# PJLab-ADG/DetZero

Measured on AMD Instinct MI355X. Metric: LiDAR frames/sec (160k pts, 0.1m voxels), higher is better.
Workload: dtype f32 as f16 pairs (hi+lo, 22-bit significand; 3 f16 MFMA per product, f32 accumulate)

## Files before the change

### detzero_amd/csrc/common.h

```cpp
#pragma once
#include <hip/hip_runtime.h>
#include <stdint.h>
#include <stdio.h>

#include "../../include/detzero_hip.h"

namespace dz {

void set_error(const char *fmt, ...);

#define DZ_CHECK_ARG(cond, ...)                 \
    do {                                        \
        if (!(cond)) {                          \
            dz::set_error(__VA_ARGS__);         \
            return DZ_ERR_INVALID;              \
        }                                       \
    } while (0)

#define DZ_HIP(expr)                                                                     \
    do {                                                                                 \
        hipError_t _e = (expr);                                                          \
        if (_e != hipSuccess) {                                                          \
            dz::set_error("%s failed: %s (%s:%d)", #expr, hipGetErrorString(_e), __FILE__, __LINE__); \
            return DZ_ERR_HIP;                                                           \
        }                                                                                \
    } while (0)

#define DZ_LAUNCH_CHECK()                                                                \
    do {                                                                                 \
        hipError_t _e = hipGetLastError();                                               \
        if (_e != hipSuccess) {                                                          \
            dz::set_error("kernel launch failed: %s (%s:%d)", hipGetErrorString(_e), __FILE__, __LINE__); \
            return DZ_ERR_HIP;                                                           \
        }                                                                                \
    } while (0)

static inline int ceil_div(long a, long b) { return (int)((a + b - 1) / b); }

static inline int tile_masks_words(int cap) { return (cap / 32 + 1 + 3) & ~3; }
static inline size_t align_up(size_t x, size_t a) { return (x + a - 1) / a * a; }

static inline int stream_grid(long work_items, int block) {
    long g = (work_items + block - 1) / block;
    if (g < 1) g = 1;
    if (g > 2048) g = 2048;
    return (int)g;
}

constexpr int DZ_MAX_DEVICES = 32;
struct PerDeviceFlags { bool v[DZ_MAX_DEVICES] = {}; };
static inline int reserve_lds(const void *kernel, int bytes, PerDeviceFlags &done, const char *who) {
    int dev = 0;
    if (hipGetDevice(&dev) != hipSuccess) { set_error("%s: hipGetDevice failed", who); return DZ_ERR_HIP; }
    if (dev >= 0 && dev < DZ_MAX_DEVICES && done.v[dev]) return DZ_OK;
    if (hipFuncSetAttribute(kernel, hipFuncAttributeMaxDynamicSharedMemorySize, bytes) != hipSuccess) {
        set_error("%s: cannot reserve %d bytes of LDS on device %d", who, bytes, dev);
        return DZ_ERR_HIP;
    }
    if (dev >= 0 && dev < DZ_MAX_DEVICES) done.v[dev] = true;
    return DZ_OK;
}
static inline int device_cus() {
    static int cus[DZ_MAX_DEVICES] = {};
    int dev = 0;
    if (hipGetDevice(&dev) != hipSuccess) return 256;
    if (dev >= 0 && dev < DZ_MAX_DEVICES && cus[dev]) return cus[dev];
    int n = 0;
    if (hipDeviceGetAttribute(&n, hipDeviceAttributeMultiprocessorCount, dev) != hipSuccess || n <= 0) n = 256;
    if (dev >= 0 && dev < DZ_MAX_DEVICES) cus[dev] = n;
    return n;
}

constexpr uint32_t KEY_INVALID = 0xFFFFFFFFu;

__device__ __forceinline__ int bitmap_rank(const uint32_t *__restrict__ bitmap,
                                           const uint32_t *__restrict__ prefix, uint32_t key) {
    const uint32_t w = key >> 5, bit = key & 31u;
    const uint32_t word = bitmap[w];
    return (int)(prefix[w] + __popc(word & ((1u << bit) - 1u)));
}
__device__ __forceinline__ int bitmap_find(const uint32_t *__restrict__ bitmap,
                                           const uint32_t *__restrict__ prefix, uint32_t key) {
    const uint32_t w = key >> 5, bit = key & 31u;
    const uint32_t word = bitmap[w];
    if (!((word >> bit) & 1u)) return -1;
    return (int)(prefix[w] + __popc(word & ((1u << bit) - 1u)));
}

struct LevelGeom {
    int b, d, h, w, layout, nby, nbx;
    __host__ __device__ __forceinline__ uint32_t key(int bi, int z, int y, int x) const {
        if (layout == 0) return (uint32_t)(((bi * d + z) * h + y) * w + x);
        const uint32_t brick = (uint32_t)((bi * nby + (y >> 3)) * nbx + (x >> 3));
        return ((brick * (uint32_t)d + (uint32_t)z) << 6) | (uint32_t)(((y & 7) << 3) | (x & 7));
    }
    __host__ __device__ __forceinline__ bool inside(int bi, int z, int y, int x) const {
        return (unsigned)bi < (unsigned)b && (unsigned)z < (unsigned)d && (unsigned)y < (unsigned)h && (unsigned)x < (unsigned)w;
    }
    __host__ __device__ __forceinline__ size_t cells() const {
        return layout == 0 ? (size_t)b * d * h * w : (size_t)b * nby * nbx * d * 64;
    }
    __host__ __device__ __forceinline__ uint32_t batch_key(int bi) const {
        return layout == 0 ? (uint32_t)bi * (uint32_t)(d * h * w) : (uint32_t)bi * (uint32_t)(nby * nbx * d * 64);
    }
};
static inline LevelGeom make_level(int b, int d, int h, int w, int layout) {
    LevelGeom g;
    g.b = b; g.d = d; g.h = h; g.w = w; g.layout = layout ? 1 : 0;
    g.nby = (h + 7) / 8; g.nbx = (w + 7) / 8;
    return g;
}

__device__ __forceinline__ uint32_t block_excl_scan_256(uint32_t v, uint32_t *lds, uint32_t &total) {
    const int lane = threadIdx.x & 63, wid = threadIdx.x >> 6;
    uint32_t incl = v;
#pragma unroll
    for (int off = 1; off < 64; off <<= 1) {
        uint32_t t = __shfl_up(incl, off, 64);
        if (lane >= off) incl += t;
    }
    if (lane == 63) lds[wid] = incl;
    __syncthreads();
    uint32_t woff = 0, tot = 0;
#pragma unroll
    for (int w = 0; w < 4; ++w) {
        uint32_t s = lds[w];
        if (w < wid) woff += s;
        tot += s;
    }
    __syncthreads();
    total = tot;
    return woff + incl - v;
}

struct ScanDims { int d0, d1, d2; };
int fill_u32(void *ptr, uint32_t value, size_t nwords, hipStream_t stream);
int nms_sweep(const unsigned long long *mask, const int *d_n, int batch, int n_cap, int col_blocks, int post_max, int *keep,
              int *d_num_keep, hipStream_t stream);
size_t bitmap_scan_workspace_bytes(size_t nwords);
int bitmap_scan(const uint32_t *bitmap, size_t nwords, uint32_t *prefix, int *d_total, int mode,
                ScanDims dims, int *coords_out, int cap_out, void *ws, size_t ws_bytes,
                hipStream_t stream, bool nonzero_only = false,
                const unsigned char *line_flags = nullptr);
int level_scan(const uint32_t *bitmap, const LevelGeom &lg, uint32_t *prefix, int *d_total, int *coords_out, int cap_out, void *ws,
               size_t ws_bytes, hipStream_t stream, bool nonzero_only, const unsigned char *line_flags = nullptr);

}
```

### detzero_amd/csrc/sparse_conv_h.hip

```cpp
#include "hgemm.h"
#include "sparse_conv_w.h"

namespace dz {

constexpr int KVOL_MAX_H = 27;

template <class T, class M, int NS, bool GN, int OCC>
__global__ __launch_bounds__(T::THREADS) __attribute__((amdgpu_waves_per_eu(OCC))) void k_spconv_h(SpConvHArgs a) {
    extern __shared__ __attribute__((aligned(16))) unsigned char smem_raw[];
    v4u *const smem = reinterpret_cast<v4u *>(smem_raw);
    int *const nbr_s = reinterpret_cast<int *>(smem + T::LDS_U4);
    __shared__ unsigned int mask_s;
    __shared__ __attribute__((aligned(16))) float sc_s[T::BC], sh_s[T::BC];
    constexpr int P = T::P_PER_THREAD;
    constexpr int NST = T::P_PER_THREAD + T::C_PER_THREAD;

    const int tid = threadIdx.x, lane = tid & 63, wid = tid >> 6;
    const int wp = wid / T::WC, wc = wid % T::WC;
    const int m = min(*a.d_m_out, a.cap);
    const int ntiles = (m + T::BP - 1) / T::BP;
    const int kchunks = a.cin / T::KC;
    const int n0 = blockIdx.y * T::BC;
    const srsrc_t prsrc = make_srsrc(a.in, a.in_bytes);
    const srsrc_t crsrc = make_srsrc(a.w, a.w_bytes);
    const srsrc_t nrsrc = make_srsrc(a.nbr, a.nbr_bytes);
    unsigned int cvoff[T::C_PER_THREAD];
#pragma unroll
    for (int i = 0; i < T::C_PER_THREAD; ++i) {
        const int idx = tid + i * T::THREADS;
        cvoff[i] = OOB_OFFSET;
        if (T::C_PIECES % T::THREADS == 0 || idx < T::C_PIECES) {
            const int n = idx / (T::KC / 4), q = idx % (T::KC / 4);
            cvoff[i] = (unsigned int)(((n0 + n) * a.cin + q * 4) * 4);
        }
    }
    const unsigned int tap_bytes = (unsigned int)(a.cout_pad * a.cin * 4);
    const unsigned int nbr_tap_bytes = (unsigned int)a.cap * 4u;
    for (int c = tid; c < T::BC; c += T::THREADS) {
        const bool in = n0 + c < a.cout;
        sc_s[c] = (in && a.scale) ? a.scale[n0 + c] : 1.f;
        sh_s[c] = (in && a.shift) ? a.shift[n0 + c] : 0.f;
    }
    __syncthreads();

    constexpr int XRUN = 16;
    const int xcd = blockIdx.x & 7;
    for (int t = blockIdx.x >> 3;; t += gridDim.x >> 3) {
        const int tile = ((t / XRUN) * 8 + xcd) * XRUN + t % XRUN;
        if ((t / XRUN) * 8 * XRUN >= ntiles) break;
        if (tile >= ntiles) continue;
        const int row0 = tile * T::BP;
        unsigned int taps;
        if constexpr (GN) {
            taps = 0u;
#pragma unroll
            for (int i = 0; i < T::BP / 32; ++i) taps |= a.tile_masks[tile * (T::BP / 32) + i];
            taps = __builtin_amdgcn_readfirstlane(taps);
        } else {
            if (tid == 0) mask_s = 0u;
            __syncthreads();
            unsigned int local = 0u;
            for (int idx = tid; idx < a.kvol * T::BP; idx += T::THREADS) {
                const int k = idx / T::BP, r = idx % T::BP;
                const int row = row0 + r;
                const int v = (row < m) ? a.nbr[(size_t)k * a.cap + row] : -1;
                nbr_s[idx] = v;
                if (v >= 0) local |= 1u << k;
            }
            if (local) atomicOr(&mask_s, local);
            __syncthreads();
            taps = mask_s;
        }

        f32x16 acc[T::CT][T::PT];
#pragma unroll
        for (int i = 0; i < T::CT; ++i)
#pragma unroll
            for (int j = 0; j < T::PT; ++j)
#pragma unroll
                for (int e = 0; e < 16; ++e) acc[i][j][e] = 0.f;

        const int nchunks = __popc(taps) * kchunks;
        if (nchunks > 0) {
            unsigned int rem = taps;
            int tap = __ffs((int)rem) - 1, kc = 0;
            auto advance = [&]() {
                rem &= rem - 1;
                if (rem == 0u) { rem = taps; ++kc; }
                tap = __ffs((int)rem) - 1;
            };
            if constexpr (GN) {
                int nb[NS][P];
                unsigned int nvoff[P];
#pragma unroll
                for (int i = 0; i < P; ++i) {
                    const int idx = tid + i * T::THREADS;
                    const int row = row0 + idx / (T::KC / 4);
                    nvoff[i] = ((T::P_PIECES % T::THREADS == 0 || idx < T::P_PIECES) && row < m) ? (unsigned int)row * 4u : OOB_OFFSET;
                }
                unsigned int rem_a = taps;
                int tap_a = __ffs((int)rem_a) - 1;
                auto fetch_nbr = [&](int (&dst)[P]) {
                    const unsigned int toff = (unsigned int)tap_a * nbr_tap_bytes;
#pragma unroll
                    for (int i = 0; i < P; ++i)
                        asm volatile("buffer_load_dword %0, %1, %2, 0 offen" : "=v"(dst[i]) : "v"(nvoff[i] == OOB_OFFSET ? OOB_OFFSET : nvoff[i] + toff), "s"(nrsrc));
                    rem_a &= rem_a - 1;
                    if (rem_a == 0u) rem_a = taps;
                    tap_a = __ffs((int)rem_a) - 1;
                };
#pragma unroll
                for (int s = 0; s < NS; ++s) fetch_nbr(nb[s]);
                asm volatile("s_waitcnt vmcnt(0)");
#pragma unroll
                for (int s = 0; s < NS; ++s)
#pragma unroll
                    for (int i = 0; i < P; ++i) asm volatile("" : "+v"(nb[s][i]));
                auto issue = [&](HStage<T> &st, auto s_t) {
                    constexpr int S = decltype(s_t)::value;
                    asm volatile("s_waitcnt vmcnt(%0)" ::"n"((NS - 1) * (NST + P)));
                    unsigned int pvoff[P];
#pragma unroll
                    for (int i = 0; i < P; ++i) {
                        asm volatile("" : "+v"(nb[S][i]));
                        const int q = (tid + i * T::THREADS) % (T::KC / 4);
                        const int rb = nb[S][i];
                        pvoff[i] = (nvoff[i] != OOB_OFFSET && rb >= 0) ? (unsigned int)rb * (unsigned int)(a.cin * 4) + (unsigned int)(q * 16) : OOB_OFFSET;
                    }
                    load_hstage<T>(st, prsrc, pvoff, (unsigned int)(kc * T::KC * 4), crsrc, cvoff,
                                   (unsigned int)tap * tap_bytes + (unsigned int)(kc * T::KC * 4));
                    fetch_nbr(nb[S]);
                };
                hgemm_pipeline<T, M, NS, P, (T::THREADS == 512)>(nchunks, smem, issue, advance, acc, wp, wc, lane, tid);
            } else {
                auto issue = [&](HStage<T> &st, auto) {
                    unsigned int pvoff[P];
#pragma unroll
                    for (int i = 0; i < P; ++i) {
                        const int idx = tid + i * T::THREADS;
                        pvoff[i] = OOB_OFFSET;
                        if (T::P_PIECES % T::THREADS == 0 || idx < T::P_PIECES) {
                            const int rr = idx / (T::KC / 4), q = idx % (T::KC / 4);
                            const int rb = nbr_s[tap * T::BP + rr];
                            pvoff[i] = rb >= 0 ? (unsigned int)rb * (unsigned int)(a.cin * 4) + (unsigned int)(q * 16) : OOB_OFFSET;
                        }
                    }
                    load_hstage<T>(st, prsrc, pvoff, (unsigned int)(kc * T::KC * 4), crsrc, cvoff,
                                   (unsigned int)tap * tap_bytes + (unsigned int)(kc * T::KC * 4));
                };
                hgemm_pipeline<T, M, NS>(nchunks, smem, issue, advance, acc, wp, wc, lane, tid);
            }
        }

        store_tile_pair16<T, M>(acc, smem_raw, sc_s, sh_s, n0, a.cout, a.relu != 0, reinterpret_cast<const unsigned char *>(a.residual),
                                reinterpret_cast<unsigned char *>(a.out), wp, wc, lane, wid, [&](int lr) {
                                    const int row = row0 + lr;
                                    return row < m ? (size_t)row * a.cout * 4 : ~size_t(0);
                                });
        __syncthreads();
    }
}


template <class M, class T, int NS, bool GN, int OCC>
static int launch_spconv_h(const SpConvHArgs &a, hipStream_t stream) {
    constexpr int LDS = T::LDS_BYTES + (GN ? 0 : KVOL_MAX_H * T::BP * 4);
    static PerDeviceFlags lds_done;
    if (int rc_ = reserve_lds(reinterpret_cast<const void *>(&k_spconv_h<T, M, NS, GN, OCC>), LDS, lds_done, "dz_spconv_forward_split")) return rc_;
    int grid = ceil_div(a.cap, T::BP);
    if (grid > 2048) grid = 2048;
    grid = (grid + 7) & ~7;
    if (grid < 8) grid = 8;
    hipLaunchKernelGGL((k_spconv_h<T, M, NS, GN, OCC>), dim3(grid, a.cout_pad / T::BC), dim3(T::THREADS), LDS, stream, a);
    DZ_LAUNCH_CHECK();
    return DZ_OK;
}

enum SpHVariant { SH_NONE = 0, SH_W_16_16, SH_W_16_32, SH_W_32_32, SH_WP_16_16, SH_WP_16_32, SH_WP_32_32, SH_128_32_16_LDS, SH_128_32_32_LDS,
                  SH_256_64_RING, SH_256_64_LDS, SH_256_128_RING, SH_256_128_LDS };

using SpHLaunch = int (*)(const SpConvHArgs &, hipStream_t);
struct SpHEntry { const char *name, *arm; SpHLaunch launch[3]; };
#define DZ_BY_MATH(fn, ...) {fn<MathF16, __VA_ARGS__>, fn<MathBF16, __VA_ARGS__>, fn<MathF16H, __VA_ARGS__>}
static const SpHEntry kSpH[] = {
    {"none", "none", {nullptr, nullptr, nullptr}},
    {"k_spconv_w<16x16>", "k_spconv_w<16x16>", DZ_BY_MATH(launch_spconv_w, 16, 16, 4, 4, 3, false)},
    {"k_spconv_w<16x32>", "k_spconv_w<16x32>", DZ_BY_MATH(launch_spconv_w, 16, 32, 3, 6, 3, false)},
    {"k_spconv_w<32x32>", "k_spconv_w<32x32>", DZ_BY_MATH(launch_spconv_w, 32, 32, 2, 12, 3, false)},
    {"k_spconv_w<16x16>", "k_spconv_w<16x16>", DZ_BY_MATH(launch_spconv_w, 16, 16, 4, 6, 3, true)},
    {"k_spconv_w<16x32>", "k_spconv_w<16x32>", DZ_BY_MATH(launch_spconv_w, 16, 32, 3, 6, 3, true)},
    {"k_spconv_w<32x32>", "k_spconv_w<32x32>", DZ_BY_MATH(launch_spconv_w, 32, 32, 2, 12, 3, true)},
    {"k_spconv_h<128x32x16>", "k_spconv_h<128x32x16> lds", DZ_BY_MATH(launch_spconv_h, HTile<128, 32, 16, 4, 1>, 4, false, 4)},
    {"k_spconv_h<128x32x32>", "k_spconv_h<128x32x32> lds", DZ_BY_MATH(launch_spconv_h, HTile<128, 32, 32, 4, 1>, 3, false, 1)},
    {"k_spconv_h<256x64x32>", "k_spconv_h<256x64x32> ring", DZ_BY_MATH(launch_spconv_h, HTile<256, 64, 32, 4, 2>, 3, true, 2)},
    {"k_spconv_h<256x64x32>", "k_spconv_h<256x64x32> lds", DZ_BY_MATH(launch_spconv_h, HTile<256, 64, 32, 4, 2>, 3, false, 2)},
    {"k_spconv_h<256x128x32>", "k_spconv_h<256x128x32> ring", DZ_BY_MATH(launch_spconv_h, HTile<256, 128, 32, 4, 2>, 2, true, 2)},
    {"k_spconv_h<256x128x32>", "k_spconv_h<256x128x32> lds", DZ_BY_MATH(launch_spconv_h, HTile<256, 128, 32, 4, 2>, 2, false, 2)},
};
#undef DZ_BY_MATH
static_assert(sizeof(kSpH) / sizeof(kSpH[0]) == SH_256_128_LDS + 1, "one entry per variant");

static SpHVariant spconv_h_select(int cin, int cout, bool packed, bool masks) {
    if (packed || (masks && cout <= 32)) {
        if (cin == 16 && cout == 16) return packed ? SH_WP_16_16 : SH_W_16_16;
        if (cin == 16 && cout == 32) return packed ? SH_WP_16_32 : SH_W_16_32;
        if (cin == 32 && cout == 32) return packed ? SH_WP_32_32 : SH_W_32_32;
        if (packed) return SH_NONE;
    }
    if (cin == 16 && cout <= 32) return SH_128_32_16_LDS;
    if (cin == 32 && cout <= 32) return SH_128_32_32_LDS;
    if ((cin == 32 || cin == 64) && cout == 64) return masks ? SH_256_64_RING : SH_256_64_LDS;
    if ((cin == 64 || cin == 128) && cout == 128) return masks ? SH_256_128_RING : SH_256_128_LDS;
    return SH_NONE;
}

}

using namespace dz;

extern "C" {

int dz_spconv_forward_split(const float *in, int in_rows, int cin, const int *nbr, const uint32_t *tile_masks, int kvol, int cap_out,
                            const int *d_m_out, const float *w, const float *scale, const float *shift, const float *residual,
                            int relu, float *out, int cout, int math, void *stream_) {
    hipStream_t stream = (hipStream_t)stream_;
    DZ_CHECK_ARG(in && nbr && d_m_out && w && out, "dz_spconv_forward_split: null pointer");
    DZ_CHECK_ARG(kvol >= 1 && kvol <= KVOL_MAX_H, "dz_spconv_forward_split: kvol %d not in [1,27]", kvol);
    DZ_CHECK_ARG(math == DZ_MATH_F16X2 || math == DZ_MATH_BF16X2 || math == DZ_MATH_F16, "dz_spconv_forward_split: math %d is not a split mode", math);
    DZ_CHECK_ARG(cout % 8 == 0 && cin % 8 == 0, "dz_spconv_forward_split: channels must be multiples of the 8-channel pair16 group");
    if (cap_out == 0) return DZ_OK;
    const int cout_pad = cout < 32 ? 32 : cout;
    const size_t in_bytes = (size_t)in_rows * cin * sizeof(float);
    const size_t w_bytes = (size_t)kvol * cout_pad * cin * sizeof(float);
    if (in_rows < 0 || in_bytes >= 0x80000000ull) {
        set_error("dz_spconv_forward_split: input of %zu bytes exceeds the 2 GiB buffer-addressing limit", in_bytes);
        return DZ_ERR_UNSUPPORTED;
    }
    const size_t nbr_bytes = (size_t)kvol * cap_out * sizeof(int);
    SpConvHArgs a{in, nbr, tile_masks, d_m_out, w, scale, shift, residual, out, cin, cout, cout_pad, kvol, cap_out, relu,
                  (unsigned int)in_bytes, (unsigned int)w_bytes, nbr_bytes < 0x80000000ull ? (unsigned int)nbr_bytes : 0u,
                  tile_masks ? (unsigned int)tile_masks_words(cap_out) * 4u : 0u};
    const SpHVariant v = spconv_h_select(cin, cout, false, a.tile_masks && a.nbr_bytes);
    if (v == SH_NONE) {
        set_error("dz_spconv_forward_split: unsupported channels cin=%d cout=%d", cin, cout);
        return DZ_ERR_UNSUPPORTED;
    }
    return kSpH[v].launch[math - 1](a, stream);
}

int dz_spconv_forward_split_packed(const float *in, int in_rows, int cin, const int *nbr_packed, const uint32_t *tile_masks, int cap_out,
                                   const int *d_m_out, const float *w, const float *scale, const float *shift, const float *residual,
                                   int relu, float *out, int cout, int math, void *stream_) {
    hipStream_t stream = (hipStream_t)stream_;
    DZ_CHECK_ARG(in && nbr_packed && tile_masks && d_m_out && w && out, "dz_spconv_forward_split_packed: null pointer");
    DZ_CHECK_ARG(math == DZ_MATH_F16X2 || math == DZ_MATH_BF16X2 || math == DZ_MATH_F16, "dz_spconv_forward_split_packed: math %d is not a split mode", math);
    if (cap_out == 0) return DZ_OK;
    const int kvol = 27, cout_pad = 32;
    const size_t in_bytes = (size_t)in_rows * cin * sizeof(float);
    const size_t w_bytes = (size_t)kvol * cout_pad * cin * sizeof(float);
    const size_t nbr_bytes = (size_t)9 * cap_out * sizeof(int);
    if (in_rows < 0 || in_bytes >= 0x80000000ull || nbr_bytes >= 0x80000000ull) {
        set_error("dz_spconv_forward_split_packed: input of %zu / table of %zu bytes exceeds the 2 GiB buffer-addressing limit", in_bytes, nbr_bytes);
        return DZ_ERR_UNSUPPORTED;
    }
    SpConvHArgs a{in, nbr_packed, tile_masks, d_m_out, w, scale, shift, residual, out, cin, cout, cout_pad, kvol, cap_out, relu,
                  (unsigned int)in_bytes, (unsigned int)w_bytes, (unsigned int)nbr_bytes, (unsigned int)tile_masks_words(cap_out) * 4u};
    const SpHVariant v = spconv_h_select(cin, cout, true, true);
    if (v == SH_NONE) {
        set_error("dz_spconv_forward_split_packed: %d -> %d channels (the packed table feeds the 16 -> 16, 16 -> 32 and 32 -> 32 kernels)", cin, cout);
        return DZ_ERR_UNSUPPORTED;
    }
    return kSpH[v].launch[math - 1](a, stream);
}

const char *dz_spconv_variant_split(int cin, int cout) {
    return kSpH[spconv_h_select(cin, cout, false, true)].name;
}

const char *dz_spconv_variant_split_packed(int cin, int cout) {
    return kSpH[spconv_h_select(cin, cout, true, true)].name;
}

const char *dz_spconv_variant_split_arm(int cin, int cout, int kvol, int has_tile_masks, size_t nbr_bytes) {
    (void)kvol;
    return kSpH[spconv_h_select(cin, cout, false, has_tile_masks && nbr_bytes > 0 && nbr_bytes < 0x80000000ull)].arm;
}

}
```

### detzero_amd/csrc/sparse_index.hip

```cpp
#include <algorithm>
#include <stdarg.h>
#include <string.h>

#include "common.h"

namespace dz {

static thread_local char g_err[512] = "";
void set_error(const char *fmt, ...) {
    va_list ap;
    va_start(ap, fmt);
    vsnprintf(g_err, sizeof(g_err), fmt, ap);
    va_end(ap);
}
const char *last_error() { return g_err; }

__global__ void k_fill_u32(uint32_t *__restrict__ p, uint32_t v, size_t n) {
    const size_t n4 = n / 4;
    uint4 *p4 = reinterpret_cast<uint4 *>(p);
    const uint4 v4 = make_uint4(v, v, v, v);
    for (size_t i = (size_t)blockIdx.x * blockDim.x + threadIdx.x; i < n4; i += (size_t)gridDim.x * blockDim.x) p4[i] = v4;
    for (size_t i = n4 * 4 + (size_t)blockIdx.x * blockDim.x + threadIdx.x; i < n; i += (size_t)gridDim.x * blockDim.x) p[i] = v;
}

int fill_u32(void *ptr, uint32_t value, size_t nwords, hipStream_t stream) {
    if (nwords == 0) return DZ_OK;
    if (((uintptr_t)ptr & 15u) != 0) { set_error("fill_u32: pointer not 16-byte aligned"); return DZ_ERR_INVALID; }
    hipLaunchKernelGGL(k_fill_u32, dim3(stream_grid((long)(nwords / 4 + 1), 256)), dim3(256), 0, stream,
                       reinterpret_cast<uint32_t *>(ptr), value, nwords);
    DZ_LAUNCH_CHECK();
    return DZ_OK;
}

template <int WPT>
__global__ __launch_bounds__(256) void k_scan_reduce(const uint32_t *__restrict__ bitmap, size_t nwords,
                                                     uint32_t *__restrict__ partial, const unsigned char *__restrict__ line_flags) {
    __shared__ uint32_t lds[4];
    const size_t base = (size_t)blockIdx.x * (256 * WPT) + (size_t)threadIdx.x * WPT;
    uint32_t s = 0;
    if (!line_flags || (base < nwords && line_flags[base >> 5])) {
#pragma unroll
        for (int j = 0; j < WPT; ++j)
            if (base + j < nwords) s += __popc(bitmap[base + j]);
    }
    uint32_t total;
    block_excl_scan_256(s, lds, total);
    if (threadIdx.x == 0) partial[blockIdx.x] = total;
}

__global__ __launch_bounds__(1024) void k_scan_partials(uint32_t *__restrict__ partial, int nblocks, int *__restrict__ d_total) {
    constexpr int PPT = 8, TRIP = 1024 * PPT;
    __shared__ uint32_t buf[TRIP + TRIP / 32];
    __shared__ uint32_t wsum[16];
    const int t = threadIdx.x, lane = t & 63, wid = t >> 6;
    auto slot = [](int i) { return i + (i >> 5); };
    uint32_t carry = 0, nxt[PPT];
#pragma unroll
    for (int j = 0; j < PPT; ++j) nxt[j] = (j * 1024 + t < nblocks) ? partial[j * 1024 + t] : 0u;
    for (int base = 0; base < nblocks; base += TRIP) {
#pragma unroll
        for (int j = 0; j < PPT; ++j) buf[slot(j * 1024 + t)] = nxt[j];
        if (base + TRIP < nblocks) {
#pragma unroll
            for (int j = 0; j < PPT; ++j) { const int i = base + TRIP + j * 1024 + t; nxt[j] = i < nblocks ? partial[i] : 0u; }
        }
        __syncthreads();
        uint32_t v[PPT], s = 0;
#pragma unroll
        for (int j = 0; j < PPT; ++j) { v[j] = buf[slot(t * PPT + j)]; s += v[j]; }
        uint32_t incl = s;
#pragma unroll
        for (int off = 1; off < 64; off <<= 1) {
            const uint32_t u = __shfl_up(incl, off, 64);
            if (lane >= off) incl += u;
        }
        if (lane == 63) wsum[wid] = incl;
        __syncthreads();
        uint32_t woff = 0, tot = 0;
#pragma unroll
        for (int w = 0; w < 16; ++w) { const uint32_t x = wsum[w]; if (w < wid) woff += x; tot += x; }
        uint32_t run = carry + woff + incl - s;
#pragma unroll
        for (int j = 0; j < PPT; ++j) { buf[slot(t * PPT + j)] = run; run += v[j]; }
        carry += tot;
        __syncthreads();
#pragma unroll
        for (int j = 0; j < PPT; ++j) { const int i = base + j * 1024 + t; if (i < nblocks) partial[i] = buf[slot(j * 1024 + t)]; }
        __syncthreads();
    }
    if (t == 0) *d_total = (int)carry;
}

struct FastDiv { uint32_t d; double inv; };
__device__ __forceinline__ uint32_t fast_divmod(uint32_t n, const FastDiv f, uint32_t &rem) {
    uint32_t q = (uint32_t)__double2uint_rz((double)n * f.inv);
    uint32_t r = n - q * f.d;
    if ((int32_t)r < 0) { --q; r += f.d; }
    else if (r >= f.d) { ++q; r -= f.d; }
    rem = r;
    return q;
}
struct ScanDecode { FastDiv d0, d1, d2; };

template <int MODE, int WPT, bool NZ = false>
__global__ __launch_bounds__(256) void k_scan_down(const uint32_t *__restrict__ bitmap, size_t nwords,
                                                   const uint32_t *__restrict__ partial,
                                                   uint32_t *__restrict__ prefix, ScanDecode dec,
                                                   int *__restrict__ coords_out, int cap_out,
                                                   const unsigned char *__restrict__ line_flags, const int *__restrict__ d_total) {
    constexpr int CHUNK = 256 * WPT;
    if (NZ) {
        const uint32_t p0 = partial[blockIdx.x], p1 = blockIdx.x + 1 < gridDim.x ? partial[blockIdx.x + 1] : (uint32_t)*d_total;
        if (p0 == p1) return;
    }
    __shared__ uint32_t lds[4];
    __shared__ __attribute__((aligned(16))) uint32_t w_s[CHUNK];
    __shared__ __attribute__((aligned(16))) uint32_t p_s[CHUNK];
    const size_t base = (size_t)blockIdx.x * CHUNK + (size_t)threadIdx.x * WPT;
    uint32_t wv[WPT];
    const bool live = !line_flags || (base < nwords && line_flags[base >> 5]);
#pragma unroll
    for (int j = 0; j < WPT; ++j) wv[j] = (live && base + j < nwords) ? bitmap[base + j] : 0u;
    uint32_t s = 0;
#pragma unroll
    for (int j = 0; j < WPT; ++j) s += __popc(wv[j]);
    uint32_t total;
    uint32_t run = block_excl_scan_256(s, lds, total) + partial[blockIdx.x];
    uint32_t pv[WPT];
#pragma unroll
    for (int j = 0; j < WPT; ++j) { pv[j] = run; run += __popc(wv[j]); }
#pragma unroll
    for (int j = 0; j < WPT; ++j)
        if (base + j < nwords && (!NZ || wv[j])) prefix[base + j] = pv[j];
    if (MODE < 0 || total == 0) return;
#pragma unroll
    for (int j = 0; j < WPT; ++j) { w_s[threadIdx.x * WPT + j] = wv[j]; p_s[threadIdx.x * WPT + j] = pv[j]; }
    __syncthreads();
#pragma unroll 1
    for (int j = 0; j < WPT; ++j) {
        const int idx = threadIdx.x + 256 * j;
        uint32_t word = w_s[idx];
        if (!word) continue;
        uint32_t r = p_s[idx];
        const uint32_t key0 = (uint32_t)(((size_t)blockIdx.x * CHUNK + idx) << 5);
        if (MODE == 2) {
            uint32_t z, by, bx;
            const uint32_t brick = fast_divmod(key0 >> 6, dec.d0, z);
            const uint32_t t = fast_divmod(brick, dec.d2, bx);
            const uint32_t bb = fast_divmod(t, dec.d1, by);
            const int y0 = (int)(by * 8u + ((key0 >> 3) & 7u)), x0 = (int)(bx * 8u);
            while (word) {
                const int bit = __ffs((int)word) - 1;
                word &= word - 1;
                if ((int)r < cap_out) reinterpret_cast<int4 *>(coords_out)[r] = make_int4((int)bb, (int)z, y0 + (bit >> 3), x0 + (bit & 7));
                ++r;
            }
            continue;
        }
        uint32_t c2, c1, c0;
        const uint32_t t1 = fast_divmod(key0, dec.d2, c2);
        const uint32_t t0 = fast_divmod(t1, dec.d1, c1);
        uint32_t bb = fast_divmod(t0, dec.d0, c0);
        int last = 0;
        while (word) {
            const int bit = __ffs((int)word) - 1;
            word &= word - 1;
            c2 += (uint32_t)(bit - last);
            last = bit;
            while (c2 >= dec.d2.d) {
                c2 -= dec.d2.d;
                if (++c1 == dec.d1.d) { c1 = 0; if (++c0 == dec.d0.d) { c0 = 0; ++bb; } }
            }
            if ((int)r < cap_out) {
                int4 o;
                if (MODE == 0) o = make_int4((int)bb, (int)c0, (int)c1, (int)c2);
                else o = make_int4((int)bb, (int)c2, (int)c1, (int)c0);
                reinterpret_cast<int4 *>(coords_out)[r] = o;
            }
            ++r;
        }
    }
}

size_t bitmap_scan_workspace_bytes(size_t nwords) {
    const size_t nblocks = (nwords + 255) / 256;
    return align_up(nblocks * sizeof(uint32_t), 256);
}

template <int WPT>
static void launch_scan(const uint32_t *bitmap, size_t nwords, uint32_t *prefix, int *d_total, int mode, const ScanDecode &dec,
                        int *coords_out, int cap_out, uint32_t *partial, hipStream_t stream, bool nonzero_only,
                        const unsigned char *lf) {
    const int nblocks = (int)((nwords + 256 * WPT - 1) / (256 * WPT));
    hipLaunchKernelGGL(k_scan_reduce<WPT>, dim3(nblocks), dim3(256), 0, stream, bitmap, nwords, partial, lf);
    hipLaunchKernelGGL(k_scan_partials, dim3(1), dim3(1024), 0, stream, partial, nblocks, d_total);
    if (mode == 0 && nonzero_only)
        hipLaunchKernelGGL((k_scan_down<0, WPT, true>), dim3(nblocks), dim3(256), 0, stream, bitmap, nwords, partial, prefix, dec,
                           coords_out, cap_out, lf, d_total);
    else if (mode == 0)
        hipLaunchKernelGGL((k_scan_down<0, WPT>), dim3(nblocks), dim3(256), 0, stream, bitmap, nwords, partial, prefix, dec,
                           coords_out, cap_out, lf, d_total);
    else if (mode == 1)
        hipLaunchKernelGGL((k_scan_down<1, WPT>), dim3(nblocks), dim3(256), 0, stream, bitmap, nwords, partial, prefix, dec,
                           coords_out, cap_out, lf, d_total);
    else if (mode == 2 && nonzero_only)
        hipLaunchKernelGGL((k_scan_down<2, WPT, true>), dim3(nblocks), dim3(256), 0, stream, bitmap, nwords, partial, prefix, dec,
                           coords_out, cap_out, lf, d_total);
    else if (mode == 2)
        hipLaunchKernelGGL((k_scan_down<2, WPT>), dim3(nblocks), dim3(256), 0, stream, bitmap, nwords, partial, prefix, dec,
                           coords_out, cap_out, lf, d_total);
    else
        hipLaunchKernelGGL((k_scan_down<-1, WPT>), dim3(nblocks), dim3(256), 0, stream, bitmap, nwords, partial, prefix, dec,
                           coords_out, cap_out, lf, d_total);
}

int bitmap_scan(const uint32_t *bitmap, size_t nwords, uint32_t *prefix, int *d_total, int mode,
                ScanDims dims, int *coords_out, int cap_out, void *ws, size_t ws_bytes,
                hipStream_t stream, bool nonzero_only, const unsigned char *line_flags) {
    if (ws_bytes < bitmap_scan_workspace_bytes(nwords)) {
        set_error("bitmap_scan: workspace %zu < %zu", ws_bytes, bitmap_scan_workspace_bytes(nwords));
        return DZ_ERR_WORKSPACE;
    }
    uint32_t *partial = reinterpret_cast<uint32_t *>(ws);
    ScanDecode dec;
    dec.d0 = FastDiv{(uint32_t)(dims.d0 > 0 ? dims.d0 : 1), 1.0 / (double)(dims.d0 > 0 ? dims.d0 : 1)};
    dec.d1 = FastDiv{(uint32_t)(dims.d1 > 0 ? dims.d1 : 1), 1.0 / (double)(dims.d1 > 0 ? dims.d1 : 1)};
    dec.d2 = FastDiv{(uint32_t)(dims.d2 > 0 ? dims.d2 : 1), 1.0 / (double)(dims.d2 > 0 ? dims.d2 : 1)};
    if (nwords <= ((size_t)1 << 21))
        launch_scan<1>(bitmap, nwords, prefix, d_total, mode, dec, coords_out, cap_out, partial, stream, nonzero_only, line_flags);
    else
        launch_scan<4>(bitmap, nwords, prefix, d_total, mode, dec, coords_out, cap_out, partial, stream, nonzero_only, line_flags);
    DZ_LAUNCH_CHECK();
    return DZ_OK;
}

__global__ void k_set_bits_from_coords(const int *__restrict__ coords, const int *__restrict__ d_n, int n_cap,
                                       LevelGeom lg, uint32_t *__restrict__ bitmap) {
    const int n = d_n ? min(*d_n, n_cap) : n_cap;
    for (int i = blockIdx.x * blockDim.x + threadIdx.x; i < n; i += gridDim.x * blockDim.x) {
        const int4 c = reinterpret_cast<const int4 *>(coords)[i];
        if (!lg.inside(c.x, c.y, c.z, c.w)) continue;
        const uint32_t key = lg.key(c.x, c.y, c.z, c.w);
        atomicOr(&bitmap[key >> 5], 1u << (key & 31u));
    }
}

__global__ void k_rank_of_coords(const int *__restrict__ coords, const int *__restrict__ d_n, int n_cap, LevelGeom lg,
                                 const uint32_t *__restrict__ bitmap, const uint32_t *__restrict__ prefix, int *__restrict__ rank) {
    const int n = d_n ? min(*d_n, n_cap) : n_cap;
    for (int i = blockIdx.x * blockDim.x + threadIdx.x; i < n_cap; i += gridDim.x * blockDim.x) {
        int r = -1;
        if (i < n) {
            const int4 c = reinterpret_cast<const int4 *>(coords)[i];
            if (lg.inside(c.x, c.y, c.z, c.w)) r = bitmap_rank(bitmap, prefix, lg.key(c.x, c.y, c.z, c.w));
        }
        rank[i] = r;
    }
}

struct ConvGeom {
    int k[3], s[3], p[3];
    int od, oh, ow;
};

__device__ __forceinline__ int outs_of(int c, int k, int s, int p, int od, int (&w)[3]) {
    int n = 0;
    const int cp = c + p;
    for (int t = cp % s; t < k && t <= cp; t += s) {
        const int o = (cp - t) / s;
        if (o < od && n < 3) w[n++] = o;
    }
    return n;
}

__global__ void k_mark_outputs(const int *__restrict__ coords_in, const int *__restrict__ d_m_in, int cap_in,
                               ConvGeom g, LevelGeom lo, uint32_t *__restrict__ bitmap_out) {
    const int m = min(*d_m_in, cap_in);
    for (int i = blockIdx.x * blockDim.x + threadIdx.x; i < m; i += gridDim.x * blockDim.x) {
        const int4 c = reinterpret_cast<const int4 *>(coords_in)[i];
        int wz[3], wy[3], wx[3];
        const int nz = outs_of(c.y, g.k[0], g.s[0], g.p[0], g.od, wz);
        const int ny = outs_of(c.z, g.k[1], g.s[1], g.p[1], g.oh, wy);
        const int nx = outs_of(c.w, g.k[2], g.s[2], g.p[2], g.ow, wx);
        for (int a = 0; a < nz; ++a)
            for (int b = 0; b < ny; ++b) {
                uint32_t word_idx = 0xFFFFFFFFu, bits = 0u;
                for (int e = 0; e < nx; ++e) {
                    const uint32_t key = lo.key(c.x, wz[a], wy[b], wx[e]);
                    if ((key >> 5) != word_idx) {
                        if (bits && (__builtin_nontemporal_load(&bitmap_out[word_idx]) & bits) != bits) atomicOr(&bitmap_out[word_idx], bits);
                        word_idx = key >> 5;
                        bits = 0u;
                    }
                    bits |= 1u << (key & 31u);
                }
                if (bits && (__builtin_nontemporal_load(&bitmap_out[word_idx]) & bits) != bits) atomicOr(&bitmap_out[word_idx], bits);
            }
    }
}

__global__ __launch_bounds__(256) void k_mark_outputs_w(const int *__restrict__ coords_in, const int *__restrict__ d_m_in, int cap_in,
                                                        ConvGeom g, LevelGeom lo, uint32_t *__restrict__ bitmap_out) {
    const int m = min(*d_m_in, cap_in);
    const int m_pad = (m + 63) & ~63;
    const int lane = threadIdx.x & 63;
    for (int i = blockIdx.x * blockDim.x + threadIdx.x; i < m_pad; i += gridDim.x * blockDim.x) {
        uint32_t widx[4] = {0xFFFFFFFFu, 0xFFFFFFFFu, 0xFFFFFFFFu, 0xFFFFFFFFu}, wbits[4] = {0u, 0u, 0u, 0u};
        if (i < m) {
            const int4 c = reinterpret_cast<const int4 *>(coords_in)[i];
            int wz[3], wy[3], wx[3];
            const int nz = outs_of(c.y, g.k[0], g.s[0], g.p[0], g.od, wz);
            const int ny = outs_of(c.z, g.k[1], g.s[1], g.p[1], g.oh, wy);
            const int nx = outs_of(c.w, g.k[2], g.s[2], g.p[2], g.ow, wx);
#pragma unroll
            for (int a = 0; a < 2; ++a)
#pragma unroll
                for (int b = 0; b < 2; ++b) {
                    if (a >= nz || b >= ny || nx < 1) continue;
                    const uint32_t k0 = lo.key(c.x, wz[a], wy[b], wx[0]);
                    uint32_t w = k0 >> 5, bits = 1u << (k0 & 31u);
                    if (nx > 1) {
                        const uint32_t k1 = lo.key(c.x, wz[a], wy[b], wx[1]);
                        if ((k1 >> 5) == w) bits |= 1u << (k1 & 31u);
                        else atomicOr(&bitmap_out[k1 >> 5], 1u << (k1 & 31u));
                    }
                    widx[a * 2 + b] = w;
                    wbits[a * 2 + b] = bits;
                }
        }
        bool last[4];
#pragma unroll
        for (int sl = 0; sl < 4; ++sl) {
            const uint32_t w = widx[sl];
            uint32_t bits = wbits[sl];
#pragma unroll
            for (int d = 1; d < 64; d <<= 1) {
                const uint32_t wp = (uint32_t)__shfl_up((int)w, d, 64), bp = (uint32_t)__shfl_up((int)bits, d, 64);
                if (lane >= d && wp == w) bits |= bp;
            }
            const uint32_t wn = (uint32_t)__shfl_down((int)w, 1, 64);
            last[sl] = bits && (lane == 63 || wn != w);
            wbits[sl] = bits;
        }
        uint32_t seen[4];
#pragma unroll
        for (int sl = 0; sl < 4; ++sl) seen[sl] = last[sl] ? __builtin_nontemporal_load(&bitmap_out[widx[sl]]) : 0xFFFFFFFFu;
#pragma unroll
        for (int sl = 0; sl < 4; ++sl)
            if (last[sl] && (seen[sl] & wbits[sl]) != wbits[sl]) atomicOr(&bitmap_out[widx[sl]], wbits[sl]);
    }
}

#ifndef DZ_NBR_DIAG
#define DZ_NBR_DIAG 0
#endif
typedef unsigned int nbr_u3 __attribute__((ext_vector_type(3)));

template <bool EDGE>
__device__ __forceinline__ void nbr_row3(nbr_u3 w, nbr_u3 p, int ci, uint32_t bc, bool ok, bool lv, bool rv, int &vl, int &vc, int &vr) {
    uint32_t wc_ = w.y, pc_ = p.y, lw = w.x, lp = p.x, rw = w.z, rp = p.z;
    if (EDGE) {
        wc_ = ci == 1 ? w.y : (ci == 0 ? w.x : w.z);
        pc_ = ci == 1 ? p.y : (ci == 0 ? p.x : p.z);
        lw = ci == 1 ? w.x : (ci == 2 ? w.y : 0u); lp = ci == 1 ? p.x : p.y;
        rw = ci == 1 ? w.z : (ci == 0 ? w.y : 0u); rp = ci == 1 ? p.z : p.y;
    }
    if (!ok) wc_ = lw = rw = 0u;
    const int rank = (int)(pc_ + __popc(wc_ & ((1u << bc) - 1u)));
    const uint32_t cbit = (wc_ >> bc) & 1u;
    vc = cbit ? rank : -1;
    const bool lbit = bc != 0u ? ((wc_ >> (bc - 1u)) & 1u) != 0u : (lw >> 31) != 0u;
    const bool rbit = bc != 31u ? ((wc_ >> (bc + 1u)) & 1u) != 0u : (rw & 1u) != 0u;
    const int lrank = bc != 0u ? rank - 1 : (int)(lp + __popc(lw)) - 1;
    const int rrank = bc != 31u ? rank + (int)cbit : (int)rp;
    vl = lbit && lv ? lrank : -1;
    vr = rbit && rv ? rrank : -1;
}

template <int K0, int K1, int KW, bool XCD, bool PACK = false>
__global__ __launch_bounds__(256) void k_build_neighbors_rows(const int *__restrict__ coords_out, const int *__restrict__ d_m_out,
                                                              int cap_out, const uint32_t *__restrict__ bitmap_in,
                                                              const uint32_t *__restrict__ prefix_in, LevelGeom li, ConvGeom g,
                                                              int *__restrict__ nbr, uint32_t *__restrict__ tile_masks, int mask_rows,
                                                              uint32_t last_base, uint32_t index_bytes, uint32_t nbr_bytes) {
// ... 149 lines not shown
            if (tz + 1 < 3) fetch(tz + 1, sl[tz + 1]);
            const Slab &q = sl[tz];
            const bool any_edge = __any(q.edge);
#pragma unroll
            for (int ty = 0; ty < 3; ++ty) {
                const int r = tz * 3 + ty;
                const uint32_t bc = q.kc[ty] & 31u;
                int vl, vc, vr;
                if (any_edge) nbr_row3<true>(q.word[ty], q.pref[ty], (int)((q.kc[ty] >> 5) - q.base[ty]), bc, q.ok[ty], lv, rv, vl, vc, vr);
                else nbr_row3<false>(q.word[ty], q.pref[ty], 1, bc, q.ok[ty], lv, rv, vl, vc, vr);
                const uint32_t rr = vl >= 0 ? (uint32_t)vl + 1u : (vc >= 0 ? (uint32_t)vc : (vr >= 0 ? (uint32_t)vr : 0u));
                const uint32_t e = rr | (vl >= 0 ? 1u << 29 : 0u) | (vc >= 0 ? 1u << 30 : 0u) | (vr >= 0 ? 1u << 31 : 0u);
                words[r] = mine ? e : 0u;
                if (mine) __builtin_amdgcn_raw_buffer_store_b32((int)e, tab, voff, (uint32_t)r * row_bytes, 0);
                bits |= ((vl >= 0 ? 1u : 0u) | (vc >= 0 ? 2u : 0u) | (vr >= 0 ? 4u : 0u)) << (r * 3);
            }
        }
        {
            uint32_t gb = bits;
#pragma unroll
            for (int d = 16; d >= 1; d >>= 1) gb |= (uint32_t)__shfl_xor((int)gb, d, 64);
            if ((tid & 31) == 0 && o < mask_rows) tile_masks[o >> 5] = gb;
        }
        __syncthreads();
#pragma unroll
        for (int tz = 0; tz < 3; ++tz) {
            int lo = 0x7FFFFFFF, hi = -1;
#pragma unroll
            for (int ty = 0; ty < 3; ++ty) {
                const uint32_t e = words[tz * 3 + ty];
                if (!(e >> 29)) continue;
                const int r = (int)(e & 0x1FFFFFFFu), l = (int)((e >> 29) & 1u), cc = (int)((e >> 30) & 1u), rt = (int)(e >> 31);
                lo = min(lo, r - l);
                hi = max(hi, rt ? r + cc : (cc ? r : r - 1));
            }
#pragma unroll
            for (int d = 32; d >= 1; d >>= 1) {
                lo = min(lo, __shfl_xor(lo, d, 64));
                hi = max(hi, __shfl_xor(hi, d, 64));
            }
            if ((tid & 63) == 0 && hi >= 0) { atomicMin(&lo_s[su][tz], lo); atomicMax(&hi_s[su][tz], hi); }
        }
        const int unit = blk * upb + su, row0 = unit * tile_rows;
        unsigned int key = 0x8000000u;
        if (perm) {
            const unsigned int k27 = (unit & 1) ? (0x7FFFFFFu - (bits & 0x7FFFFFFu)) : (bits & 0x7FFFFFFu);
            key = mine ? k27 : 0x8000000u;
            key_s[tid] = key;
        }
        __syncthreads();
        if (ui < 3 && unit < nunits) {
            const int tz = ui;
            int lo = lo_s[su][tz], n = hi_s[su][tz] >= 0 ? hi_s[su][tz] - lo + 1 : 0;
            if (n == 0) lo = 0;
            if (tz == 1 && n == 0 && row0 < m) n = 1;
            win[(size_t)unit * 6 + 2 * tz] = lo;
            win[(size_t)unit * 6 + 2 * tz + 1] = n;
        }
        if (perm) {
            int rank = 0;
            const unsigned int *ks = key_s + su * tile_rows;
            for (int j = 0; j < tile_rows; j += 4) {
                const uint4 v = *reinterpret_cast<const uint4 *>(&ks[j]);
                rank += (v.x < key || (v.x == key && j < ui)) + (v.y < key || (v.y == key && j + 1 < ui)) + (v.z < key || (v.z == key && j + 2 < ui)) +
                        (v.w < key || (v.w == key && j + 3 < ui));
            }
            const int pos = row0 + rank;
            if (pos < cap_out) {
                perm[pos] = o;
#pragma unroll
                for (int g = 0; g < 9; ++g) nbr_sorted[(size_t)g * cap_out + pos] = (int)words[g];
            }
        }
        __syncthreads();
    }
}

__global__ __launch_bounds__(256) void k_build_neighbors(const int *__restrict__ coords_out,
                                                         const int *__restrict__ d_m_out, int cap_out,
                                                         const uint32_t *__restrict__ bitmap_in,
                                                         const uint32_t *__restrict__ prefix_in, LevelGeom li,
                                                         ConvGeom g, int *__restrict__ nbr,
                                                         uint32_t *__restrict__ tile_masks) {
    const int m = min(*d_m_out, cap_out);
    const int rows = g.k[0] * g.k[1];
    const int m_pad = (m + 63) & ~63;
    const long total = (long)m_pad * rows;
    for (long idx = (long)blockIdx.x * blockDim.x + threadIdx.x; idx < total;
         idx += (long)gridDim.x * blockDim.x) {
        const int o = (int)(idx % m_pad);
        const int zy = (int)(idx / m_pad);
        const int tz = zy / g.k[1], ty = zy % g.k[1];
        uint32_t bits = 0u;
        if (o < m) {
            const int4 c = reinterpret_cast<const int4 *>(coords_out)[o];
            const int uz = c.y * g.s[0] - g.p[0] + tz;
            const int uy = c.z * g.s[1] - g.p[1] + ty;
            const bool row_ok = (unsigned)uz < (unsigned)li.d && (unsigned)uy < (unsigned)li.h;
            const int base_x = c.w * g.s[2] - g.p[2];
            for (int tx = 0; tx < g.k[2]; ++tx) {
                const int ux = base_x + tx;
                int v = -1;
                if (row_ok && (unsigned)ux < (unsigned)li.w) v = bitmap_find(bitmap_in, prefix_in, li.key(c.x, uz, uy, ux));
                const int tap = (tz * g.k[1] + ty) * g.k[2] + tx;
                nbr[(size_t)tap * cap_out + o] = v;
                if (v >= 0) bits |= 1u << tap;
            }
        }
        if (tile_masks) {
#pragma unroll
            for (int d = 16; d >= 1; d >>= 1) bits |= (uint32_t)__shfl_xor((int)bits, d, 64);
            if ((threadIdx.x & 31) == 0 && bits) atomicOr(&tile_masks[o >> 5], bits);
        }
    }
}

__global__ void k_scatter_rows(const float *__restrict__ src, const int *__restrict__ rank,
                               const int *__restrict__ d_n, int n_cap, int c_src, float *__restrict__ dst,
                               int c_dst) {
    const int n = d_n ? min(*d_n, n_cap) : n_cap;
    const long total = (long)n * c_dst;
    for (long idx = (long)blockIdx.x * blockDim.x + threadIdx.x; idx < total;
         idx += (long)gridDim.x * blockDim.x) {
        const int i = (int)(idx / c_dst), ch = (int)(idx % c_dst);
        const int r = rank[i];
        if (r < 0) continue;
        dst[(size_t)r * c_dst + ch] = (ch < c_src) ? src[(size_t)i * c_src + ch] : 0.f;
    }
}

__global__ void k_gather_rows(const float *__restrict__ src, const int *__restrict__ idx_,
                              const int *__restrict__ d_n, int n_cap, int c, float *__restrict__ out) {
    const int n = d_n ? min(*d_n, n_cap) : n_cap;
    const long total = (long)n * c;
    for (long idx = (long)blockIdx.x * blockDim.x + threadIdx.x; idx < total;
         idx += (long)gridDim.x * blockDim.x) {
        const int i = (int)(idx / c), ch = (int)(idx % c);
        out[idx] = src[(size_t)idx_[i] * c + ch];
    }
}

static bool geom_from(const int *k3, const int *s3, const int *p3, int d, int h, int w, ConvGeom &g) {
    for (int i = 0; i < 3; ++i) {
        g.k[i] = k3[i]; g.s[i] = s3[i]; g.p[i] = p3[i];
        if (g.k[i] < 1 || g.s[i] < 1 || g.p[i] < 0) return false;
    }
    g.od = (d + 2 * g.p[0] - g.k[0]) / g.s[0] + 1;
    g.oh = (h + 2 * g.p[1] - g.k[1]) / g.s[1] + 1;
    g.ow = (w + 2 * g.p[2] - g.k[2]) / g.s[2] + 1;
    return g.od > 0 && g.oh > 0 && g.ow > 0;
}

int level_scan(const uint32_t *bitmap, const LevelGeom &lg, uint32_t *prefix, int *d_total, int *coords_out, int cap_out, void *ws,
               size_t ws_bytes, hipStream_t stream, bool nonzero_only, const unsigned char *line_flags) {
    const size_t nwords = align_up((lg.cells() + 31) / 32, 8);
    if (lg.layout == 0)
        return bitmap_scan(bitmap, nwords, prefix, d_total, 0, ScanDims{lg.d, lg.h, lg.w}, coords_out, cap_out, ws, ws_bytes, stream,
                           nonzero_only, line_flags);
    return bitmap_scan(bitmap, nwords, prefix, d_total, 2, ScanDims{lg.d, lg.nby, lg.nbx}, coords_out, cap_out, ws, ws_bytes, stream,
                       nonzero_only, line_flags);
}

}

using namespace dz;

extern "C" {

const char *dz_version(void) { return "detzero_hip 0.1 (gfx950)"; }
const char *dz_last_error(void) { return dz::last_error(); }

int dz_device_cu_count(void) {
    int dev = 0, n = 0;
    if (hipGetDevice(&dev) != hipSuccess) return -1;
    if (hipDeviceGetAttribute(&n, hipDeviceAttributeMultiprocessorCount, dev) != hipSuccess) return -1;
    return n;
}

size_t dz_index_words(int b, int d, int h, int w, int layout) {
    const size_t cells = make_level(b, d, h, w, layout).cells();
    return align_up((cells + 31) / 32, 8);
}

size_t dz_index_workspace_bytes(int b, int d, int h, int w, int layout) {
    return bitmap_scan_workspace_bytes(dz_index_words(b, d, h, w, layout));
}

static int check_cells(int b, int d, int h, int w, int layout) {
    if (b < 1 || d < 1 || h < 1 || w < 1 || (layout != DZ_LAYOUT_LINEAR && layout != DZ_LAYOUT_BRICK) ||
        make_level(b, d, h, w, layout).cells() >= 0xFFFFFFFFull) {
        set_error("grid %d x %d x %d x %d (layout %d) does not fit 32-bit cell keys", b, d, h, w, layout);
        return DZ_ERR_UNSUPPORTED;
    }
    return DZ_OK;
}


int dz_index_from_coords(const int *coords, const int *d_n, int n_cap, int b, int d, int h, int w, int layout,
                         uint32_t *bitmap, uint32_t *prefix, int *coords_out, int *d_m, int cap_out,
                         int *rank_of_input, void *ws, size_t ws_bytes, void *stream_) {
    hipStream_t stream = (hipStream_t)stream_;
    DZ_CHECK_ARG((coords || n_cap == 0) && bitmap && prefix && coords_out && d_m && n_cap >= 0 && cap_out >= 0,
                 "dz_index_from_coords: null/negative argument");
    int rc = check_cells(b, d, h, w, layout);
    if (rc) return rc;
    const LevelGeom lg = make_level(b, d, h, w, layout);
    const size_t nwords = dz_index_words(b, d, h, w, layout);
    rc = fill_u32(bitmap, 0u, nwords, stream);
    if (rc) return rc;
    if (n_cap > 0)
        hipLaunchKernelGGL(k_set_bits_from_coords, dim3(stream_grid(n_cap, 256)), dim3(256), 0, stream, coords,
                           d_n, n_cap, lg, bitmap);
    rc = level_scan(bitmap, lg, prefix, d_m, coords_out, cap_out, ws, ws_bytes, stream, false);
    if (rc) return rc;
    if (rank_of_input && n_cap > 0)
        hipLaunchKernelGGL(k_rank_of_coords, dim3(stream_grid(n_cap, 256)), dim3(256), 0, stream, coords, d_n,
                           n_cap, lg, bitmap, prefix, rank_of_input);
    DZ_LAUNCH_CHECK();
    return DZ_OK;
}

int dz_index_downsample(const int *coords_in, const int *d_m_in, int cap_in, int b, int d, int h, int w, int layout,
                        const int *h_k3, const int *h_s3, const int *h_p3, uint32_t *bitmap_out,
                        uint32_t *prefix_out, int *coords_out, int *d_m_out, int cap_out, void *ws,
                        size_t ws_bytes, void *stream_) {
    hipStream_t stream = (hipStream_t)stream_;
    DZ_CHECK_ARG(coords_in && d_m_in && bitmap_out && prefix_out && coords_out && d_m_out,
                 "dz_index_downsample: null argument");
    ConvGeom g;
    DZ_CHECK_ARG(geom_from(h_k3, h_s3, h_p3, d, h, w, g), "dz_index_downsample: bad kernel/stride/padding");
    int rc = check_cells(b, g.od, g.oh, g.ow, layout);
    if (rc) return rc;
    const LevelGeom lo = make_level(b, g.od, g.oh, g.ow, layout);
    const size_t nwords = dz_index_words(b, g.od, g.oh, g.ow, layout);
    rc = fill_u32(bitmap_out, 0u, nwords, stream);
    if (rc) return rc;
    static const int plain = getenv("DZ_TUNE_MARK_PLAIN") ? atoi(getenv("DZ_TUNE_MARK_PLAIN")) : 0;
    const bool two = (g.k[0] + g.s[0] - 1) / g.s[0] <= 2 && (g.k[1] + g.s[1] - 1) / g.s[1] <= 2 && (g.k[2] + g.s[2] - 1) / g.s[2] <= 2;
    if (cap_in > 0 && two && !plain)
        hipLaunchKernelGGL(k_mark_outputs_w, dim3(stream_grid(cap_in, 256)), dim3(256), 0, stream, coords_in, d_m_in,
                           cap_in, g, lo, bitmap_out);
    else if (cap_in > 0)
        hipLaunchKernelGGL(k_mark_outputs, dim3(stream_grid(cap_in, 256)), dim3(256), 0, stream, coords_in, d_m_in,
                           cap_in, g, lo, bitmap_out);
    rc = level_scan(bitmap_out, lo, prefix_out, d_m_out, coords_out, cap_out, ws, ws_bytes, stream, false);
    if (rc) return rc;
    DZ_LAUNCH_CHECK();
    return DZ_OK;
}

int dz_tile_masks_words(int cap_out) { return cap_out < 0 ? 0 : tile_masks_words(cap_out); }

int dz_build_neighbors(const int *coords_out, const int *d_m_out, int cap_out, const uint32_t *bitmap_in,
                       const uint32_t *prefix_in, int b, int d, int h, int w, int layout, const int *h_k3, const int *h_s3,
                       const int *h_p3, int *nbr, uint32_t *tile_masks, void *stream_) {
    hipStream_t stream = (hipStream_t)stream_;
    DZ_CHECK_ARG(coords_out && d_m_out && bitmap_in && prefix_in && nbr, "dz_build_neighbors: null argument");
    ConvGeom g;
    DZ_CHECK_ARG(geom_from(h_k3, h_s3, h_p3, d, h, w, g), "dz_build_neighbors: bad kernel/stride/padding");
    DZ_CHECK_ARG(layout == DZ_LAYOUT_LINEAR || layout == DZ_LAYOUT_BRICK, "dz_build_neighbors: bad layout %d", layout);
    if (cap_out == 0) return DZ_OK;
    const LevelGeom li = make_level(b, d, h, w, layout);
    static const int generic = getenv("DZ_TUNE_NBR_GENERIC") ? atoi(getenv("DZ_TUNE_NBR_GENERIC")) : 0;
    const bool kw3 = g.k[2] == 3 && g.p[2] == 1 && (long)(g.ow - 1) * g.s[2] <= w - 1;
    const bool kw1 = g.k[2] == 1 && g.p[2] == 0 && (long)(g.ow - 1) * g.s[2] <= w - 1;
    const size_t table_bytes = (size_t)g.k[0] * g.k[1] * g.k[2] * cap_out * sizeof(int);
    if (!generic && layout == DZ_LAYOUT_LINEAR && g.k[0] == 3 && ((g.k[1] == 3 && kw3) || (g.k[1] == 1 && kw1)) &&
        table_bytes < 0xFFFFFFFFull) {
        const int mask_rows = tile_masks_words(cap_out) * 32;
        const size_t index_words = dz_index_words(b, d, h, w, layout);
        const uint32_t last_base = (uint32_t)(index_words - 3);
        static const int gmax = getenv("DZ_TUNE_NBR_GRID") ? atoi(getenv("DZ_TUNE_NBR_GRID")) : 2048;
        const dim3 grid((std::min(stream_grid(tile_masks ? mask_rows : cap_out, 256), gmax) + 7) & ~7);
        static const int flat = getenv("DZ_TUNE_NBR_FLAT") ? atoi(getenv("DZ_TUNE_NBR_FLAT")) : 0;
#define DZ_NBR_ROWS(K1_, KW_, X_)                                                                                                   \
    hipLaunchKernelGGL((k_build_neighbors_rows<3, K1_, KW_, X_>), grid, dim3(256), 0, stream, coords_out, d_m_out, cap_out, bitmap_in, \
                       prefix_in, li, g, nbr, tile_masks, mask_rows, last_base, (uint32_t)(index_words * 4), (uint32_t)table_bytes)
        if (g.k[1] == 3) { if (flat) DZ_NBR_ROWS(3, 3, false); else DZ_NBR_ROWS(3, 3, true); }
        else { if (flat) DZ_NBR_ROWS(1, 1, false); else DZ_NBR_ROWS(1, 1, true); }
#undef DZ_NBR_ROWS
        DZ_LAUNCH_CHECK();
        return DZ_OK;
    }
    if (tile_masks) {
        const int rc = fill_u32(tile_masks, 0u, (size_t)tile_masks_words(cap_out), stream);
        if (rc) return rc;
    }
    const long work = (long)cap_out * g.k[0] * g.k[1];
    hipLaunchKernelGGL(k_build_neighbors, dim3(stream_grid(work, 256)), dim3(256), 0, stream, coords_out, d_m_out,
                       cap_out, bitmap_in, prefix_in, li, g, nbr, tile_masks);
    DZ_LAUNCH_CHECK();
    return DZ_OK;
}

int dz_build_neighbors_packed(const int *coords_out, const int *d_m_out, int cap_out, const uint32_t *bitmap_in,
                              const uint32_t *prefix_in, int b, int d, int h, int w, int layout, const int *h_k3, const int *h_s3,
                              const int *h_p3, int *nbr, uint32_t *tile_masks, void *stream_) {
    hipStream_t stream = (hipStream_t)stream_;
    DZ_CHECK_ARG(coords_out && d_m_out && bitmap_in && prefix_in && nbr && tile_masks, "dz_build_neighbors_packed: null argument");
    ConvGeom g;
    DZ_CHECK_ARG(geom_from(h_k3, h_s3, h_p3, d, h, w, g), "dz_build_neighbors_packed: bad kernel/stride/padding");
    const bool kw3 = g.k[2] == 3 && g.p[2] == 1 && (long)(g.ow - 1) * g.s[2] <= w - 1;
    const size_t table_bytes = (size_t)9 * cap_out * sizeof(int);
    if (layout != DZ_LAYOUT_LINEAR || g.k[0] != 3 || g.k[1] != 3 || !kw3 || table_bytes >= 0xFFFFFFFFull || cap_out >= (1 << 29)) {
        set_error("dz_build_neighbors_packed: needs linear keys, a 3 x 3 x 3 window with x padding 1 and fewer than 2^29 rows");
        return DZ_ERR_UNSUPPORTED;
    }
    if (cap_out == 0) return DZ_OK;
    const LevelGeom li = make_level(b, d, h, w, layout);
    const int mask_rows = tile_masks_words(cap_out) * 32;
    const size_t index_words = dz_index_words(b, d, h, w, layout);
    const dim3 grid((stream_grid(mask_rows, 256) + 7) & ~7);
    hipLaunchKernelGGL((k_build_neighbors_rows<3, 3, 3, true, true>), grid, dim3(256), 0, stream, coords_out, d_m_out, cap_out, bitmap_in,
                       prefix_in, li, g, nbr, tile_masks, mask_rows, (uint32_t)(index_words - 3), (uint32_t)(index_words * 4),
                       (uint32_t)table_bytes);
    DZ_LAUNCH_CHECK();
    return DZ_OK;
}

int dz_build_neighbors_packed_x(const int *coords, const int *d_m, int cap, const uint32_t *bitmap, const uint32_t *prefix, int b, int d, int h,
                                int w, int *nbr, uint32_t *tile_masks, int tile_rows, int *windows, int *nbr_sorted, int *perm, void *stream_) {
    hipStream_t stream = (hipStream_t)stream_;
    DZ_CHECK_ARG(coords && d_m && bitmap && prefix && nbr && tile_masks && windows, "dz_build_neighbors_packed_x: null argument");
    DZ_CHECK_ARG(b >= 1 && d >= 1 && h >= 1 && w >= 1 && cap >= 0, "dz_build_neighbors_packed_x: bad grid");
    DZ_CHECK_ARG(tile_rows == 128 || tile_rows == 256, "dz_build_neighbors_packed_x: tile_rows %d (128 or 256: dz_spconv_x_tile_rows)", tile_rows);
    DZ_CHECK_ARG((nbr_sorted == nullptr) == (perm == nullptr), "dz_build_neighbors_packed_x: nbr_sorted and perm come together");
    const size_t table_bytes = (size_t)9 * cap * sizeof(int);
    if (table_bytes >= 0xFFFFFFFFull || cap >= (1 << 29)) {
        set_error("dz_build_neighbors_packed_x: needs fewer than 2^29 rows");
        return DZ_ERR_UNSUPPORTED;
    }
    if (cap == 0) return DZ_OK;
    const LevelGeom li = make_level(b, d, h, w, DZ_LAYOUT_LINEAR);
    const int mask_rows = tile_masks_words(cap) * 32;
    const size_t index_words = dz_index_words(b, d, h, w, DZ_LAYOUT_LINEAR);
    const dim3 grid((std::min(ceil_div(cap, 256), 2048) + 7) & ~7);
    hipLaunchKernelGGL(k_build_neighbors_xwin, grid, dim3(256), 0, stream, coords, d_m, cap, bitmap, prefix, li, nbr, tile_masks, mask_rows,
                       (uint32_t)(index_words - 3), (uint32_t)(index_words * 4), (uint32_t)table_bytes, tile_rows, windows, nbr_sorted, perm);
    DZ_LAUNCH_CHECK();
    return DZ_OK;
}

int dz_scatter_rows(const float *src, const int *rank, const int *d_n, int n_cap, int c_src, float *dst, int c_dst,
                    void *stream_) {
    hipStream_t stream = (hipStream_t)stream_;
    DZ_CHECK_ARG(src && rank && dst && c_src > 0 && c_dst >= c_src, "dz_scatter_rows: bad argument");
    if (n_cap == 0) return DZ_OK;
    hipLaunchKernelGGL(k_scatter_rows, dim3(stream_grid((long)n_cap * c_dst, 256)), dim3(256), 0, stream, src, rank,
                       d_n, n_cap, c_src, dst, c_dst);
    DZ_LAUNCH_CHECK();
    return DZ_OK;
}

int dz_gather_rows(const float *src, const int *idx, const int *d_n, int n_cap, int c, float *out, void *stream_) {
    hipStream_t stream = (hipStream_t)stream_;
    DZ_CHECK_ARG(src && idx && out && c > 0, "dz_gather_rows: bad argument");
    if (n_cap == 0) return DZ_OK;
    hipLaunchKernelGGL(k_gather_rows, dim3(stream_grid((long)n_cap * c, 256)), dim3(256), 0, stream, src, idx, d_n,
                       n_cap, c, out);
    DZ_LAUNCH_CHECK();
    return DZ_OK;
}

}
```

### detzero_amd/csrc/voxelize.hip

```cpp
#include "hgemm.h"

namespace dz {

struct VoxGeom {
    float lo[3], vs[3], hi[3];
    int g[3];
    int xy_mask;
};

__device__ __forceinline__ bool voxel_coord(const float *p, const VoxGeom &g, int &cx, int &cy, int &cz) {
    if (g.xy_mask && !(p[0] >= g.lo[0] && p[0] <= g.hi[0] && p[1] >= g.lo[1] && p[1] <= g.hi[1])) return false;
    const float fx = floorf(__fdiv_rn(__fsub_rn(p[0], g.lo[0]), g.vs[0]));
    const float fy = floorf(__fdiv_rn(__fsub_rn(p[1], g.lo[1]), g.vs[1]));
    const float fz = floorf(__fdiv_rn(__fsub_rn(p[2], g.lo[2]), g.vs[2]));
    if (!(fx >= 0.f && fx < (float)g.g[0] && fy >= 0.f && fy < (float)g.g[1] && fz >= 0.f && fz < (float)g.g[2]))
        return false;
    cx = (int)fx; cy = (int)fy; cz = (int)fz;
    return true;
}

__global__ void k_hard_keys(const float *__restrict__ pts, int n, int c, VoxGeom g, int n_per, uint32_t cells,
                            uint32_t *__restrict__ keys, uint32_t *__restrict__ bitmap) {
    for (int i = blockIdx.x * blockDim.x + threadIdx.x; i < n; i += gridDim.x * blockDim.x) {
        const float *p = pts + (size_t)i * c;
// ... 180 lines not shown
                           const int *__restrict__ d_m, int cap, int max_points, int c, float *__restrict__ out,
                           int c_out) {
    const int m = d_m ? min(*d_m, cap) : cap;
    const long total = (long)m * c_out;
    for (long idx = (long)blockIdx.x * blockDim.x + threadIdx.x; idx < total;
         idx += (long)gridDim.x * blockDim.x) {
        const int v = (int)(idx / c_out), ch = (int)(idx % c_out);
        float r = 0.f;
        if (ch < c) {
            float s = 0.f;
            for (int q = 0; q < max_points; ++q) s = __fadd_rn(s, voxels[((size_t)v * max_points + q) * c + ch]);
            const float nrm = fmaxf((float)num_points[v], 1.0f);
            r = __fdiv_rn(s, nrm);
        }
        out[idx] = r;
    }
}

__global__ void k_dyn_keys(const float *__restrict__ pts, int n, int stride, VoxGeom g, int batch,
                           uint32_t *__restrict__ keys, uint32_t *__restrict__ bitmap) {
    const int lane = threadIdx.x & 63;
    const int n_pad = (n + 63) & ~63;
    for (int i = blockIdx.x * blockDim.x + threadIdx.x; i < n_pad; i += gridDim.x * blockDim.x) {
        uint32_t key = KEY_INVALID;
        if (i < n) {
            const float *p = pts + (size_t)i * stride;
            const float xyz[3] = {p[1], p[2], p[3]};
            int cx, cy, cz;
            const int b = (int)p[0];
            if ((unsigned)b < (unsigned)batch && voxel_coord(xyz, g, cx, cy, cz))
                key = (uint32_t)(((b * g.g[0] + cx) * g.g[1] + cy) * g.g[2] + cz);
            keys[i] = key;
        }
        const uint32_t w = key == KEY_INVALID ? KEY_INVALID : key >> 5;
        uint32_t bits = key == KEY_INVALID ? 0u : 1u << (key & 31u);
#pragma unroll
        for (int d = 1; d < 64; d <<= 1) {
            const uint32_t wp = (uint32_t)__shfl_up((int)w, d, 64), bp = (uint32_t)__shfl_up((int)bits, d, 64);
            if (lane >= d && wp == w) bits |= bp;
        }
        const uint32_t wn = (uint32_t)__shfl_down((int)w, 1, 64);
        if (bits && (lane == 63 || wn != w)) atomicOr(&bitmap[w], bits);
    }
}

constexpr float DYN_FIX = 268435456.f;

__global__ void k_dyn_accumulate(const float *__restrict__ pts, int n, int c, const uint32_t *__restrict__ keys,
                                 const uint32_t *__restrict__ bitmap, const uint32_t *__restrict__ prefix, int cap,
                                 unsigned long long *__restrict__ acc, int *__restrict__ counts) {
    const int lane = threadIdx.x & 63;
    const int n_pad = (n + 63) & ~63;
    for (int i = blockIdx.x * blockDim.x + threadIdx.x; i < n_pad; i += gridDim.x * blockDim.x) {
        const uint32_t key = i < n ? keys[i] : KEY_INVALID;
        const uint32_t prev = (uint32_t)__shfl_up((int)key, 1, 64), next = (uint32_t)__shfl_down((int)key, 1, 64);
        const unsigned long long heads = __ballot(lane == 0 || prev != key);
        const int first = 63 - __clzll(heads & (~0ull >> (63 - lane)));
        const int run = lane - first + 1;
        const bool last = key != KEY_INVALID && (lane == 63 || next != key);
        int v = cap;
        if (last) v = bitmap_rank(bitmap, prefix, key);
        int steps = 0;
        while (steps < 6 && __ballot(lane - (1 << steps) >= first) != 0ull) ++steps;
        for (int ch = 0; ch < c; ++ch) {
            long long q = key != KEY_INVALID ? __float2ll_rn(pts[(size_t)i * (c + 1) + 1 + ch] * DYN_FIX) : 0ll;
#pragma unroll
            for (int j = 0; j < 6; ++j) {
                if (j >= steps) break;
                const int lo = __shfl_up((int)(unsigned int)q, 1 << j, 64), hi = __shfl_up((int)(q >> 32), 1 << j, 64);
                if (lane - (1 << j) >= first) q += (long long)(((unsigned long long)(unsigned int)hi << 32) | (unsigned int)lo);
            }
            if (v < cap) atomicAdd(&acc[(size_t)v * c + ch], (unsigned long long)q);
        }
        if (v < cap) atomicAdd(&counts[v], run);
    }
}

__global__ void k_dyn_divide(const unsigned long long *__restrict__ acc, float *__restrict__ feats, const int *__restrict__ counts,
                             const int *__restrict__ d_m, int cap, int c) {
    const int m = min(*d_m, cap);
    const long total = (long)m * c;
    for (long idx = (long)blockIdx.x * blockDim.x + threadIdx.x; idx < total;
         idx += (long)gridDim.x * blockDim.x) {
        const int v = (int)(idx / c);
        const double sum = (double)(long long)acc[idx] * (1.0 / (double)DYN_FIX);
        feats[idx] = __fdiv_rn((float)sum, (float)counts[v]);
    }
}

static bool make_geom(const float *r6, const float *vs3, const int *g3, int xy_mask, VoxGeom &g) {
    g.xy_mask = xy_mask;
    for (int i = 0; i < 3; ++i) {
        g.lo[i] = r6[i]; g.hi[i] = r6[3 + i]; g.vs[i] = vs3[i]; g.g[i] = g3[i];
        if (!(g.vs[i] > 0.f) || g.g[i] < 1) return false;
    }
    return true;
}

struct HardWs {
    uint32_t *keys, *bitmap, *prefix, *pt_bitmap, *pt_prefix;
    int *mins, *canon_coords, *d_m;
    void *scan_ws;
    size_t scan_ws_bytes, total;
};
static HardWs carve_hard(void *ws, int n, size_t nwords, int max_points) {
    HardWs w{};
    size_t off = 0;
    auto take = [&](size_t bytes) { size_t o = off; off += align_up(bytes, 256); return o; };
    char *base = (char *)ws;
    const size_t pt_words = align_up(((size_t)n + 31) / 32, 8);
    size_t o_keys = take((size_t)n * 4), o_bm = take(nwords * 4), o_pf = take(nwords * 4);
    size_t o_pb = take(pt_words * 4), o_pp = take(pt_words * 4);
    size_t o_min = take((size_t)max_points * n * 4), o_cc = take((size_t)n * 16), o_dm = take(256);
    w.scan_ws_bytes = bitmap_scan_workspace_bytes(nwords > pt_words ? nwords : pt_words);
    size_t o_sw = take(w.scan_ws_bytes);
    w.total = off;
    if (base) {
        w.keys = (uint32_t *)(base + o_keys); w.bitmap = (uint32_t *)(base + o_bm); w.prefix = (uint32_t *)(base + o_pf);
        w.pt_bitmap = (uint32_t *)(base + o_pb); w.pt_prefix = (uint32_t *)(base + o_pp);
        w.mins = (int *)(base + o_min); w.canon_coords = (int *)(base + o_cc); w.d_m = (int *)(base + o_dm);
        w.scan_ws = base + o_sw;
    }
    return w;
}

}

using namespace dz;

extern "C" {

size_t dz_voxelize_hard_workspace_bytes(int n, int gx, int gy, int gz, int max_points) {
    if (n < 1) n = 1;
    return carve_hard(nullptr, n, dz_index_words(1, gz, gy, gx, DZ_LAYOUT_LINEAR), max_points).total;
}

static int voxelize_hard_impl(const float *points, int n, int c, const float *h_range6, const float *h_vsize3,
                              const int *h_grid3, int xy_range_mask, int max_points, int max_voxels, float *voxels,
                              int *coords_zyx, int *num_points, int batch_index, int batch, int cap_frame, float *feats,
                              int c_stride, int *coords_bzyx, int *d_num_voxels, void *ws, size_t ws_bytes, hipStream_t stream) {
    VoxGeom g;
    DZ_CHECK_ARG(make_geom(h_range6, h_vsize3, h_grid3, xy_range_mask, g), "dz_voxelize_hard: bad geometry");
    const size_t cells = (size_t)g.g[0] * g.g[1] * g.g[2];
    if (cells * (size_t)batch >= 0xFFFFFFFFull) { set_error("dz_voxelize_hard: grid x batch too large for 32-bit keys"); return DZ_ERR_UNSUPPORTED; }
    if (n == 0) return fill_u32(d_num_voxels, 0u, (size_t)batch, stream);
    DZ_CHECK_ARG(points, "dz_voxelize_hard: null points");
    const int n_per = n / batch;
    const size_t nwords = dz_index_words(batch, g.g[2], g.g[1], g.g[0], DZ_LAYOUT_LINEAR);
    HardWs w = carve_hard(ws, n, nwords, max_points);
    if (ws_bytes < w.total) { set_error("dz_voxelize_hard: workspace %zu < %zu", ws_bytes, w.total); return DZ_ERR_WORKSPACE; }
    const size_t pt_words = align_up(((size_t)n + 31) / 32, 8);
    const int cap = n;

    int rc = fill_u32(w.bitmap, 0u, nwords, stream);
    if (!rc) rc = fill_u32(w.pt_bitmap, 0u, pt_words, stream);
    if (!rc) rc = fill_u32(w.mins, 0x7f7f7f7fu, (size_t)max_points * cap, stream);
    if (rc) return rc;
    const int grid_n = stream_grid(n, 256);
    hipLaunchKernelGGL(k_hard_keys, dim3(grid_n), dim3(256), 0, stream, points, n, c, g, n_per, (uint32_t)cells, w.keys, w.bitmap);
    rc = bitmap_scan(w.bitmap, nwords, w.prefix, w.d_m, 0, ScanDims{g.g[2], g.g[1], g.g[0]}, w.canon_coords, cap,
                         w.scan_ws, w.scan_ws_bytes, stream);
    if (rc) return rc;
    hipLaunchKernelGGL(k_hard_insert, dim3(grid_n), dim3(256), 0, stream, w.keys, n, w.bitmap, w.prefix, w.mins, cap, max_points);
    hipLaunchKernelGGL(k_hard_mark_first, dim3(grid_n), dim3(256), 0, stream, w.mins, w.d_m, cap, w.pt_bitmap);
    rc = bitmap_scan(w.pt_bitmap, pt_words, w.pt_prefix, d_num_voxels, -1, ScanDims{1, 1, 1}, nullptr, 0, w.scan_ws,
                     w.scan_ws_bytes, stream);
    if (rc) return rc;
    if (feats)
        hipLaunchKernelGGL(k_hard_emit_mean, dim3(stream_grid((long)cap * c_stride, 256)), dim3(256), 0, stream, points, c, w.mins,
                           cap, max_points, max_voxels, w.d_m, w.canon_coords, w.pt_bitmap, w.pt_prefix, batch_index, batch, n_per,
                           cap_frame, feats, c_stride, coords_bzyx, d_num_voxels);
    else
        hipLaunchKernelGGL(k_hard_emit, dim3(stream_grid((long)cap * max_points, 256)), dim3(256), 0, stream, points, c,
                           w.mins, cap, max_points, max_voxels, w.d_m, w.canon_coords, w.pt_bitmap, w.pt_prefix, voxels,
                           coords_zyx, num_points, d_num_voxels);
    DZ_LAUNCH_CHECK();
    return DZ_OK;
}

int dz_voxelize_hard(const float *points, int n, int c, const float *h_range6, const float *h_vsize3,
                     const int *h_grid3, int xy_range_mask, int max_points, int max_voxels, float *voxels, int *coords_zyx,
                     int *num_points, int *d_num_voxels, void *ws, size_t ws_bytes, void *stream_) {
    DZ_CHECK_ARG(n >= 0 && c >= 3 && max_points >= 1 && max_voxels >= 1, "dz_voxelize_hard: bad sizes");
    DZ_CHECK_ARG(voxels && coords_zyx && num_points && d_num_voxels && ws, "dz_voxelize_hard: null pointer");
    return voxelize_hard_impl(points, n, c, h_range6, h_vsize3, h_grid3, xy_range_mask, max_points, max_voxels, voxels, coords_zyx,
                              num_points, 0, 1, 0, nullptr, 0, nullptr, d_num_voxels, ws, ws_bytes, (hipStream_t)stream_);
}

int dz_voxelize_hard_mean(const float *points, int n, int c, const float *h_range6, const float *h_vsize3,
                          const int *h_grid3, int xy_range_mask, int max_points, int max_voxels, int batch_index, float *feats,
                          int c_stride, int *coords_bzyx, int *d_num_voxels, void *ws, size_t ws_bytes, void *stream_) {
    DZ_CHECK_ARG(n >= 0 && c >= 3 && max_points >= 1 && max_voxels >= 1 && c_stride >= c, "dz_voxelize_hard_mean: bad sizes");
    DZ_CHECK_ARG(feats && coords_bzyx && d_num_voxels && ws, "dz_voxelize_hard_mean: null pointer");
    return voxelize_hard_impl(points, n, c, h_range6, h_vsize3, h_grid3, xy_range_mask, max_points, max_voxels, nullptr, nullptr,
                              nullptr, batch_index, 1, 0, feats, c_stride, coords_bzyx, d_num_voxels, ws, ws_bytes, (hipStream_t)stream_);
}

size_t dz_voxelize_hard_batched_workspace_bytes(int n_per_frame, int batch, int gx, int gy, int gz, int max_points) {
    const long n = (long)(n_per_frame < 1 ? 1 : n_per_frame) * (batch < 1 ? 1 : batch);
    return carve_hard(nullptr, (int)n, dz_index_words(batch < 1 ? 1 : batch, gz, gy, gx, DZ_LAYOUT_LINEAR), max_points).total;
}

int dz_voxelize_hard_mean_batched(const float *points, int n_per_frame, int batch, int c, const float *h_range6,
                                  const float *h_vsize3, const int *h_grid3, int xy_range_mask, int max_points, int max_voxels,
                                  float *feats, int c_stride, int *coords_bzyx, int cap_per_frame, int *d_num_voxels, void *ws,
                                  size_t ws_bytes, void *stream_) {
    DZ_CHECK_ARG(n_per_frame >= 0 && batch >= 1 && batch <= 256 && c >= 3 && max_points >= 1 && max_voxels >= 1 && c_stride >= c,
                 "dz_voxelize_hard_mean_batched: bad sizes");
    DZ_CHECK_ARG((long)n_per_frame * batch < 0x7FFFFFFFl, "dz_voxelize_hard_mean_batched: too many points");
    DZ_CHECK_ARG(cap_per_frame >= (max_voxels < n_per_frame ? max_voxels : n_per_frame),
                 "dz_voxelize_hard_mean_batched: cap_per_frame below min(max_voxels, points per frame)");
    DZ_CHECK_ARG(feats && coords_bzyx && d_num_voxels && ws, "dz_voxelize_hard_mean_batched: null pointer");
    return voxelize_hard_impl(points, n_per_frame * batch, c, h_range6, h_vsize3, h_grid3, xy_range_mask, max_points, max_voxels,
                              nullptr, nullptr, nullptr, 0, batch, cap_per_frame, feats, c_stride, coords_bzyx, d_num_voxels, ws,
                              ws_bytes, (hipStream_t)stream_);
}

static size_t level_ws_layout(long n, int max_points, int cap, size_t nwords, size_t *o_min, size_t *o_sw, size_t *sw_bytes, size_t *o_lf,
                              size_t *lf_words) {
    size_t off = align_up((size_t)(n < 1 ? 1 : n) * 4, 256);
    *o_min = off;
    off += align_up((size_t)max_points * (cap < 1 ? 1 : cap) * 4, 256);
    *sw_bytes = bitmap_scan_workspace_bytes(nwords);
    *o_sw = off;
    off += align_up(*sw_bytes, 256);
    *lf_words = align_up((nwords + 31) / 32, 16) / 4;
    *o_lf = off;
    off += align_up(*lf_words * 4, 256);
    return off;
}

size_t dz_voxelize_to_level_workspace_bytes(int n_per_frame, int batch, int max_points, int cap, int d, int h, int w, int layout) {
    size_t a, b, c, e, f;
    return level_ws_layout((long)n_per_frame * batch, max_points, cap, dz_index_words(batch, d, h, w, layout), &a, &b, &c, &e, &f);
}

int dz_voxelize_to_level(const float *points, int n_per_frame, int batch, int c, const float *h_range6, const float *h_vsize3,
                         const int *h_grid3, int xy_range_mask, int max_points, int max_voxels, int level_d, int layout, uint32_t *bitmap,
                         uint32_t *prefix, int *coords_out, int *d_m, int cap, float *feats, int c_dst, int math, void *ws,
                         size_t ws_bytes, void *stream_) {
    hipStream_t stream = (hipStream_t)stream_;
    DZ_CHECK_ARG(n_per_frame >= 0 && batch >= 1 && c >= 3 && max_points >= 1 && c_dst >= c && c_dst % 8 == 0,
                 "dz_voxelize_to_level: bad sizes");
    DZ_CHECK_ARG(math >= 0 && math <= 2, "dz_voxelize_to_level: bad math mode %d", math);
    DZ_CHECK_ARG(bitmap && prefix && coords_out && d_m && feats && ws, "dz_voxelize_to_level: null pointer");
    VoxGeom g;
    DZ_CHECK_ARG(make_geom(h_range6, h_vsize3, h_grid3, xy_range_mask, g), "dz_voxelize_to_level: bad geometry");
    DZ_CHECK_ARG(level_d >= g.g[2], "dz_voxelize_to_level: level depth %d below the voxel grid's %d", level_d, g.g[2]);
    if (n_per_frame > max_voxels) {
        set_error("dz_voxelize_to_level: %d points per frame could exceed max_voxels %d - use dz_voxelize_hard_mean_batched",
                  n_per_frame, max_voxels);
        return DZ_ERR_UNSUPPORTED;
    }
    const long n = (long)n_per_frame * batch;
    DZ_CHECK_ARG(n < 0x7FFFFFFFl && cap >= (n < 1 ? 1 : 0), "dz_voxelize_to_level: too many points");
    DZ_CHECK_ARG(layout == DZ_LAYOUT_LINEAR || layout == DZ_LAYOUT_BRICK, "dz_voxelize_to_level: bad layout %d", layout);
    const LevelGeom lg = make_level(batch, level_d, g.g[1], g.g[0], layout);
    if (lg.cells() >= 0xFFFFFFFFull) { set_error("dz_voxelize_to_level: grid x batch too large for 32-bit keys"); return DZ_ERR_UNSUPPORTED; }
    const size_t nwords = dz_index_words(batch, level_d, g.g[1], g.g[0], layout);
    size_t o_min, o_sw, sw_bytes, o_lf, lf_words;
    const size_t need = level_ws_layout(n, max_points, cap, nwords, &o_min, &o_sw, &sw_bytes, &o_lf, &lf_words);
    if (ws_bytes < need) { set_error("dz_voxelize_to_level: workspace %zu < %zu", ws_bytes, need); return DZ_ERR_WORKSPACE; }
    uint32_t *keys = (uint32_t *)ws;
    int *mins = (int *)((char *)ws + o_min);
    static const int use_flags = getenv("DZ_TUNE_LINE_FLAGS") ? atoi(getenv("DZ_TUNE_LINE_FLAGS")) : 1;
    unsigned char *line_flags = use_flags ? (unsigned char *)ws + o_lf : nullptr;
    int rc = fill_u32(bitmap, 0u, nwords, stream);
    if (!rc) rc = fill_u32(mins, 0x7f7f7f7fu, (size_t)max_points * cap, stream);
    if (!rc && line_flags) rc = fill_u32(line_flags, 0u, lf_words, stream);
    if (rc) return rc;
    if (n == 0) return level_scan(bitmap, lg, prefix, d_m, coords_out, cap, (char *)ws + o_sw, sw_bytes, stream, true, line_flags);
    DZ_CHECK_ARG(points, "dz_voxelize_to_level: null points");
    const int grid_n = stream_grid(n, 256);
    hipLaunchKernelGGL(k_level_keys, dim3(grid_n), dim3(256), 0, stream, points, (int)n, c, g, n_per_frame, lg, keys, bitmap,
                       line_flags);
    rc = level_scan(bitmap, lg, prefix, d_m, coords_out, cap, (char *)ws + o_sw, sw_bytes, stream, true, line_flags);
    if (rc) return rc;
    hipLaunchKernelGGL(k_hard_insert, dim3(grid_n), dim3(256), 0, stream, keys, (int)n, bitmap, prefix, mins, cap, max_points);
    const dim3 ge(stream_grid((long)cap * (c_dst / 8), 256));
    if (math == 0)
        hipLaunchKernelGGL(k_level_emit_mean<0>, ge, dim3(256), 0, stream, points, c, mins, cap, max_points, d_m, feats, c_dst);
    else if (math == 1)
        hipLaunchKernelGGL(k_level_emit_mean<1>, ge, dim3(256), 0, stream, points, c, mins, cap, max_points, d_m, feats, c_dst);
    else
        hipLaunchKernelGGL(k_level_emit_mean<2>, ge, dim3(256), 0, stream, points, c, mins, cap, max_points, d_m, feats, c_dst);
    DZ_LAUNCH_CHECK();
    return DZ_OK;
}

int dz_mean_vfe(const float *voxels, const int *num_points, const int *d_m, int cap, int max_points, int c, float *out,
                int c_out_stride, void *stream_) {
    hipStream_t stream = (hipStream_t)stream_;
    DZ_CHECK_ARG(voxels && num_points && out && c >= 1 && c_out_stride >= c && max_points >= 1, "dz_mean_vfe: bad argument");
    if (cap == 0) return DZ_OK;
    hipLaunchKernelGGL(k_mean_vfe, dim3(stream_grid((long)cap * c_out_stride, 256)), dim3(256), 0, stream, voxels,
                       num_points, d_m, cap, max_points, c, out, c_out_stride);
    DZ_LAUNCH_CHECK();
    return DZ_OK;
}

static size_t dyn_layout(int n, size_t nwords, int cap, int c, size_t *o_keys, size_t *o_bm, size_t *o_pf, size_t *o_cnt,
                         size_t *o_acc, size_t *o_sw, size_t *sw_bytes) {
    size_t off = 0;
    auto take = [&](size_t bytes) { size_t o = off; off += align_up(bytes, 256); return o; };
    *o_keys = take((size_t)(n < 1 ? 1 : n) * 4);
    *o_bm = take(nwords * 4);
    *o_pf = take(nwords * 4);
    *o_cnt = take((size_t)(cap < 1 ? 1 : cap) * 4);
    *o_acc = take((size_t)(cap < 1 ? 1 : cap) * (c < 1 ? 1 : c) * 8);
    *sw_bytes = bitmap_scan_workspace_bytes(nwords);
    *o_sw = take(*sw_bytes);
    return off;
}

size_t dz_voxelize_dynamic_workspace_bytes(int n, int batch, int gx, int gy, int gz, int c, int cap) {
    size_t a, b, d, e, f, g, h;
    return dyn_layout(n, dz_index_words(batch, gx, gy, gz, DZ_LAYOUT_LINEAR), cap, c, &a, &b, &d, &e, &h, &f, &g);
}

int dz_voxelize_dynamic_mean(const float *points_b, int n, int c, const float *h_range6, const float *h_vsize3,
                             const int *h_grid3, int xy_range_mask, int batch, float *feats, int *coords_bzyx,
                             int *d_num_voxels, int cap,
                             void *ws, size_t ws_bytes, void *stream_) {
    hipStream_t stream = (hipStream_t)stream_;
    DZ_CHECK_ARG(n >= 0 && c >= 3 && batch >= 1 && cap >= 0, "dz_voxelize_dynamic_mean: bad sizes");
    DZ_CHECK_ARG(feats && coords_bzyx && d_num_voxels && ws, "dz_voxelize_dynamic_mean: null pointer");
    VoxGeom g;
    DZ_CHECK_ARG(make_geom(h_range6, h_vsize3, h_grid3, xy_range_mask, g), "dz_voxelize_dynamic_mean: bad geometry");
    const size_t cells = (size_t)batch * g.g[0] * g.g[1] * g.g[2];
    if (cells >= 0x7FFFFFFFull) { set_error("dz_voxelize_dynamic_mean: batch*grid exceeds int32 merge keys"); return DZ_ERR_UNSUPPORTED; }
    const size_t nwords = dz_index_words(batch, g.g[0], g.g[1], g.g[2], DZ_LAYOUT_LINEAR);
    size_t o_keys, o_bm, o_pf, o_cnt, o_acc, o_sw, sw_bytes;
    const size_t need = dyn_layout(n, nwords, cap, c, &o_keys, &o_bm, &o_pf, &o_cnt, &o_acc, &o_sw, &sw_bytes);
    if (ws_bytes < need) { set_error("dz_voxelize_dynamic_mean: workspace %zu < %zu", ws_bytes, need); return DZ_ERR_WORKSPACE; }
    char *base = (char *)ws;
    uint32_t *keys = (uint32_t *)(base + o_keys), *bitmap = (uint32_t *)(base + o_bm), *prefix = (uint32_t *)(base + o_pf);
    int *counts = (int *)(base + o_cnt);
    unsigned long long *acc = (unsigned long long *)(base + o_acc);

    int rc = fill_u32(bitmap, 0u, nwords, stream);
    if (!rc && cap > 0) rc = fill_u32(feats, 0u, (size_t)cap * c, stream);
    if (!rc && cap > 0) rc = fill_u32(acc, 0u, (size_t)cap * c * 2, stream);
    if (!rc && cap > 0) rc = fill_u32(counts, 0u, (size_t)cap, stream);
    if (rc) return rc;
    if (n > 0) {
        DZ_CHECK_ARG(points_b, "dz_voxelize_dynamic_mean: null points");
        hipLaunchKernelGGL(k_dyn_keys, dim3(stream_grid(n, 256)), dim3(256), 0, stream, points_b, n, c + 1, g, batch, keys,
                           bitmap);
    }
    rc = bitmap_scan(bitmap, nwords, prefix, d_num_voxels, 1, ScanDims{g.g[0], g.g[1], g.g[2]}, coords_bzyx, cap,
                         base + o_sw, sw_bytes, stream);
    if (rc) return rc;
    if (n > 0 && cap > 0) {
        hipLaunchKernelGGL(k_dyn_accumulate, dim3(stream_grid((long)n, 256)), dim3(256), 0, stream, points_b, n, c,
                           keys, bitmap, prefix, cap, acc, counts);
        hipLaunchKernelGGL(k_dyn_divide, dim3(stream_grid((long)cap * c, 256)), dim3(256), 0, stream, acc, feats, counts,
                           d_num_voxels, cap, c);
    }
    DZ_LAUNCH_CHECK();
    return DZ_OK;
}

}
```

### detzero_amd/det_modules.py

```python
import contextlib
import os
from functools import partial

import numpy as np
import torch
import torch.nn as nn

from . import ops, range_audit
from .lib import DetZeroHipError
from .range_audit import RangeAudit

PACKED_TABLES = bool(os.environ.get('DZ_TUNE_PACKED_TABLES'))

K3, S1, P1 = (3, 3, 3), (1, 1, 1), (1, 1, 1)


def _inference_only(module):
    if module.training:
        raise DetZeroHipError('%s: only the inference path is implemented on the HIP backend '
                              '(call .eval()); training is out of scope' % type(module).__name__)


def fold_bn(bn, conv_bias=None):
    w = bn.weight.detach().double()
    b = bn.bias.detach().double()
    mean = bn.running_mean.detach().double()
    var = bn.running_var.detach().double()
    scale = w / torch.sqrt(var + bn.eps)
    shift = b - mean * scale
    if conv_bias is not None:
        shift = shift + conv_bias.detach().double() * scale
    return scale.float().contiguous(), shift.float().contiguous()


_FROM_ENTRY = object()
CACHE_GEN = [0]


class _Cached(nn.Module):

    def __init__(self):
        super().__init__()
        self._plan = None
        self.act_exp = None
        self.math = 0
        self.register_load_state_dict_post_hook(lambda module, incompatible: module.invalidate())

    def invalidate(self):
        self._plan = None
        CACHE_GEN[0] += 1

    def set_math(self, mode):
        if ops.math_id(mode) != self.math:
            CACHE_GEN[0] += 1
        self.math = ops.math_id(mode)
        return self

    def set_prescale(self, exps):
        self.act_exp = {k: int(v) for k, v in exps.items()} if exps else None
        CACHE_GEN[0] += 1
        return self

    def _e(self, name):
        if getattr(self, 'act_exp', None) is None or ops.storage_math(self.math) != 1:
            return 0
        return int(self.act_exp.get(name, 0))

    def _p(self, entry, e_in=0, e_out=0, key='w', scale=_FROM_ENTRY, shift=_FROM_ENTRY):
        scale = entry.get('scale') if scale is _FROM_ENTRY else scale
        shift = entry.get('shift') if shift is _FROM_ENTRY else shift
        if not self.math:
            return entry[key], scale, shift
        sm = ops.storage_math(self.math)
        if sm != 1:
            return self._w(entry, key), scale, shift
        cache = entry.setdefault('_pre', {})
        ck = (key, int(e_in), int(e_out), None if scale is None else scale.data_ptr(), None if shift is None else shift.data_ptr())
        if ck not in cache:
            wk = (key, 'w')
            if wk not in cache:
                ws, inv = ops.weight_prescale(entry[key])
                cache[wk] = (ops.pack_weight_split(ws, sm), inv)
            wp, inv = cache[wk]
            k = inv * (2.0 ** (int(e_out) - int(e_in)))
            ref = scale if scale is not None else shift
            if ref is not None and k.numel() != ref.numel():
                g = k.shape[0] if k.dim() > 1 else 1
                kk = k.reshape(g, -1)
                pad = ref.numel() // g - kk.shape[1]
                if pad < 0:
                    raise DetZeroHipError('_p: %d weight columns per group but %d scale / shift entries' % (kk.shape[1], ref.numel() // g))
                k = torch.cat([kk, kk.new_ones(g, pad)], dim=1)
            k = k.reshape(-1).contiguous()
            sc = (scale * k if scale is not None else k).contiguous()
            sh = None if shift is None else ((shift * (2.0 ** int(e_out))).contiguous() if e_out else shift)
            cache[ck] = (wp, sc, sh)
        return cache[ck]

    def _w(self, entry, key='w'):
        if not self.math:
            return entry[key]
        ck = '%s_split%d' % (key, ops.storage_math(self.math))
        if ck not in entry:
            entry[ck] = ops.pack_weight_split(entry[key], ops.storage_math(self.math))
        return entry[ck]

    def _apply(self, fn, *a, **kw):
        self._plan = None
        CACHE_GEN[0] += 1
        return super()._apply(fn, *a, **kw)


class SparseConvTensor:

    def __init__(self, features, indices, spatial_shape, batch_size, level=None, padded=None, math=0):
        self._features = features
        self.indices = indices
        self.spatial_shape = list(spatial_shape)
        self.batch_size = batch_size
        self._level = level
        self._padded = padded
        self._math = math

    @property
    def features(self):
        if self._features is None:
            rows = self._padded[0][:self.indices.shape[0]]
            self._features = ops.level_rows_f32(rows, self._padded[1], self._math)
        return self._features

    @features.setter
    def features(self, value):
        self._features = value

    def feature_rows(self, rows):
        if self._features is not None or self._padded is None or not self._math:
            return self.features[rows]
        return ops.level_rows_f32(self._padded[0][rows].contiguous(), self._padded[1], self._math)

    def replace_feature(self, new_features):
        return SparseConvTensor(new_features, self.indices, self.spatial_shape, self.batch_size, self._level)

    def dense(self):
        c = self.features.shape[1]
        d, h, w = self.spatial_shape
        bev = ops.sparse_to_bev(self.features, self._level, c, pad=0)
        return bev.view(self.batch_size, h, w, c, d).permute(0, 3, 4, 1, 2)


class _SparseConvBase(nn.Module):
    def __init__(self, in_channels, out_channels, kernel_size, stride=1, padding=0, bias=True, indice_key=None,
                 subm=False):
        super().__init__()
        k = (kernel_size,) * 3 if isinstance(kernel_size, int) else tuple(kernel_size)
        s = (stride,) * 3 if isinstance(stride, int) else tuple(stride)
        p = (padding,) * 3 if isinstance(padding, int) else tuple(padding)
        self.in_channels, self.out_channels = in_channels, out_channels
        self.kernel_size, self.stride, self.padding = k, s, p
        self.indice_key, self.subm = indice_key, subm
        self.weight = nn.Parameter(torch.empty(out_channels, *k, in_channels))
        nn.init.kaiming_uniform_(self.weight, a=5 ** 0.5)
        if bias:
            self.bias = nn.Parameter(torch.zeros(out_channels))
        else:
            self.register_parameter('bias', None)
# ... 42 lines not shown
    elif conv_type == 'spconv':
        conv = SparseConv3d(in_channels, out_channels, kernel_size, stride=stride, padding=padding, bias=False,
                            indice_key=indice_key)
    else:
        raise NotImplementedError(conv_type)
    return SparseSequential(conv, norm_fn(out_channels), nn.ReLU())


class MeanVFE(nn.Module):

    def __init__(self, model_cfg, num_point_features, **kwargs):
        super().__init__()
        self.num_point_features = num_point_features

    def get_output_feature_dim(self):
        return self.num_point_features

    def forward(self, batch_dict, **kwargs):
        voxels, num_points = batch_dict['voxels'], batch_dict['voxel_num_points']
        batch_dict['voxel_features'] = ops.mean_vfe(voxels.float().contiguous(), num_points.int().contiguous())
        return batch_dict


class DynamicMeanVFE(nn.Module):

    def __init__(self, model_cfg, num_point_features, voxel_size, grid_size, point_cloud_range, **kwargs):
        super().__init__()
        self.num_point_features = num_point_features
        self.voxel_size = [float(v) for v in voxel_size]
        self.point_cloud_range = [float(v) for v in point_cloud_range]
        self.grid_size = [int(g) for g in grid_size]

    def get_output_feature_dim(self):
        return self.num_point_features

    @torch.no_grad()
    def forward(self, batch_dict, **kwargs):
        points = batch_dict['points'].float().contiguous()
        feats, coords = ops.voxelize_dynamic(points, self.point_cloud_range, self.voxel_size,
                                             batch_dict['batch_size'])
        batch_dict['voxel_features'] = feats
        batch_dict['voxel_coords'] = coords
        return batch_dict


class VoxelResBackBone8x(_Cached):

    CIN_PAD = 16

    def __init__(self, model_cfg, input_channels, grid_size, **kwargs):
        super().__init__()
        self.model_cfg = model_cfg
        channels = list(model_cfg.get('CHANNELS', [16, 32, 64, 128])) if hasattr(model_cfg, 'get') else [16, 32, 64, 128]
        norm_fn = partial(nn.BatchNorm1d, eps=1e-3, momentum=0.01)
        grid_size = [int(g) for g in grid_size]
        self.sparse_shape = [grid_size[2] + 1, grid_size[1], grid_size[0]]
        self.input_channels = input_channels

        self.conv_input = SparseSequential(
            SubMConv3d(input_channels, channels[0], 3, padding=1, bias=False, indice_key='subm1'),
            norm_fn(channels[0]), nn.ReLU())
        block = post_act_block
        self.conv1 = SparseSequential(
            SparseBasicBlock(channels[0], channels[0], norm_fn=norm_fn, indice_key='res1'),
            SparseBasicBlock(channels[0], channels[0], norm_fn=norm_fn, indice_key='res1'))
        self.conv2 = SparseSequential(
            block(channels[0], channels[1], 3, norm_fn=norm_fn, stride=2, padding=1, indice_key='spconv2', conv_type='spconv'),
            SparseBasicBlock(channels[1], channels[1], norm_fn=norm_fn, indice_key='res2'),
            SparseBasicBlock(channels[1], channels[1], norm_fn=norm_fn, indice_key='res2'))
        self.conv3 = SparseSequential(
            block(channels[1], channels[2], 3, norm_fn=norm_fn, stride=2, padding=1, indice_key='spconv3', conv_type='spconv'),
            SparseBasicBlock(channels[2], channels[2], norm_fn=norm_fn, indice_key='res3'),
            SparseBasicBlock(channels[2], channels[2], norm_fn=norm_fn, indice_key='res3'))
        self.conv4 = SparseSequential(
            block(channels[2], channels[3], 3, norm_fn=norm_fn, stride=2, padding=(0, 1, 1), indice_key='spconv4', conv_type='spconv'),
            SparseBasicBlock(channels[3], channels[3], norm_fn=norm_fn, indice_key='res4'),
            SparseBasicBlock(channels[3], channels[3], norm_fn=norm_fn, indice_key='res4'))
        last_pad = model_cfg.get('last_pad', 0) if hasattr(model_cfg, 'get') else 0
        self.conv_out = SparseSequential(
            SparseConv3d(channels[3], channels[3], (3, 1, 1), stride=(2, 1, 1), padding=last_pad, bias=False,
                         indice_key='spconv_down2'),
            norm_fn(channels[3]), nn.ReLU())
        self.num_point_features = channels[3]
        self.layout = int(os.environ.get('DZ_TUNE_LAYOUT', ops.LAYOUT_LINEAR))
        self.engine = os.environ.get('DZ_TUNE_SPCONV_ENGINE', 'xrun')
        self.f32_engine = os.environ.get('DZ_TUNE_SPCONV_F32_ENGINE', 'gather')
        self.tile_couts = tuple(int(c) for c in os.environ.get('DZ_TUNE_SPCONV_TILE_COUTS', '16,32,64,128').split(',') if c)
        self.backbone_channels = {'x_conv1': channels[0], 'x_conv2': channels[1], 'x_conv3': channels[2],
                                  'x_conv4': channels[3]}
        self.channels = channels

    def set_engine(self, engine, f32_engine=None):
        if engine not in ('gather', 'tiles', 'xrun'):
            raise DetZeroHipError('unknown sparse engine %r (gather | xrun | tiles)' % (engine,))
        if f32_engine is not None and f32_engine not in ('gather', 'xrun'):
            raise DetZeroHipError('unknown fp32 sparse engine %r (gather | xrun)' % (f32_engine,))
        if engine == 'tiles' and ops.L.load().dz_spconv_tile_rows() == 0:
            raise DetZeroHipError("sparse engine 'tiles' is an experimental build option (measured slower, DESIGN.md 2d): rebuild the library "
                                  'with DZ_BUILD_EXPERIMENTAL=1 (python -m detzero_amd.build --force)')
        self.engine = engine
        if f32_engine is not None:
            self.f32_engine = f32_engine
        self.layout = ops.LAYOUT_BRICK if engine == 'tiles' else ops.LAYOUT_LINEAR

    def plan(self):
        if self._plan is not None:
            return self._plan

        def conv_bn(conv, bn, cin_pad=None):
            scale, shift = fold_bn(bn, conv.bias)
            return {'w': conv.taps(cin_pad), 'scale': scale, 'shift': shift, 'k': conv.kernel_size,
                    's': conv.stride, 'p': conv.padding}

        def blk(b):
            return (conv_bn(b.conv1, b.bn1), conv_bn(b.conv2, b.bn2))

        p = {'conv_input': conv_bn(self.conv_input[0], self.conv_input[1], self.CIN_PAD)}
        p['conv1'] = [blk(self.conv1[0]), blk(self.conv1[1])]
        for name in ('conv2', 'conv3', 'conv4'):
            seq = getattr(self, name)
            p[name] = {'down': conv_bn(seq[0][0], seq[0][1]), 'blocks': [blk(seq[1]), blk(seq[2])]}
        p['conv_out'] = conv_bn(self.conv_out[0], self.conv_out[1])
        self._plan = p
        return p

    def _audit(self, name, stage, y, level, e):
        audit = range_audit.active()
        if audit is not None:
            audit.probe('backbone3d.' + name, y, math=self.math, stage=stage, exp=e, d_rows=level.d_m)
        return y

    def _res_block(self, x, nbr, level, params, e=0, name=None, stage=None):
        c1, c2 = params
        y = self._audit('%s.conv1' % name, stage, ops.spconv_forward(x, nbr, level, *self._p(c1, e, e), None, True, math=self.math), level, e)
        return self._audit('%s.conv2' % name, stage, ops.spconv_forward(y, nbr, level, *self._p(c2, e, e), x, True, math=self.math), level, e)

    def build_pyramid(self, voxel_features, voxel_coords, batch_size, d_n=None, overlap=True, side_key=0, caps=None, level1=None,
                      staggered=False, exact=False):
        p = self.plan()
        dev = voxel_features.device
        if level1 is None:
            n = voxel_features.shape[0]
            lvl1 = ops.SparseLevel(batch_size, self.sparse_shape, max(n, 1), dev, layout=self.layout)
            rank = lvl1.build_from_coords(voxel_coords, d_n)
        else:
            lvl1, rank = level1, None
        main = torch.cuda.current_stream(dev)
        side = self._side_stream(dev, side_key) if overlap else main
        if overlap:
            side.wait_stream(main)
        steps = []
        tiled = self.engine == 'tiles' and self.math != 0

        pack = PACKED_TABLES and self.math != 0 and not tiled and self.layout == 0

        xrun = (self.engine if self.math != 0 else self.f32_engine) == 'xrun' and self.layout == 0
        xrun_couts = tuple(int(c) for c in os.environ.get('DZ_TUNE_XRUN_COUTS', '32,64,128').split(',') if c)

        def table(src, dst, k, s, p, cout):
            if (xrun and src is dst and cout in xrun_couts and tuple(k) == (3, 3, 3) and dst.cap < (1 << 29)
                    and ops.L.load().dz_spconv_x_tile_rows(int(cout), int(cout)) != 0
                    and (self.math != 0 or ops.L.load().dz_spconv_x_f32_window_rows(int(cout), int(cout)) != 0)):
                nbr = ops.neighbors_xrun(dst, cout)
                if getattr(nbr, 'xwin', None) is not None:
                    return nbr
            nbr = src.neighbors_to(dst, k, s, p, packed=pack and cout <= 32)
            return ops.build_tiles(nbr, dst) if tiled and cout in self.tile_couts and k[0] * k[1] * k[2] >= 3 else nbr

        def hand_over(step):
            nbr_d, nbr_s, lvl, _ = step
            for t in (nbr_d, nbr_s, lvl.coords, lvl.d_m, lvl.bitmap, lvl.prefix, lvl.ws):
                if t is not None:
                    t.record_stream(main)
                    if getattr(t, 'tile_masks', None) is not None:
                        t.tile_masks.record_stream(main)
                    for tt in getattr(t, 'tiles', None) or ():
                        tt.record_stream(main)
                    if getattr(t, 'xwin', None) is not None:
                        for tt in t.xwin:
                            if torch.is_tensor(tt):
                                tt.record_stream(main)
        ch = self.channels
        with torch.cuda.stream(side):
            nbr1 = table(lvl1, lvl1, K3, S1, P1, ch[0])
            steps.append((None, nbr1, lvl1, side.record_event() if overlap else None))
        x = voxel_features if level1 is not None else ops.scatter_rows(voxel_features, rank, self.CIN_PAD, lvl1.cap, d_n, math=self.math)
        pyr = {'x': x, 'steps': steps}
        names = ('conv2', 'conv3', 'conv4', 'conv_out')

        def build_stage(li, gate=None):
            name = names[li]
            level = steps[li][2]
            with torch.cuda.stream(side):
                if gate is not None:
                    side.wait_event(gate)
                dp = p[name]['down'] if name != 'conv_out' else p[name]
                nxt = level.downsample(dp['k'], dp['s'], dp['p'], cap=None if caps is None else int(caps[li]))
                if exact and caps is None:
                    m = nxt.num_active()
                    nxt.cap = max(int(m), 1)
                    nxt.coords = nxt.coords[:nxt.cap]
                co = ch[min(li + 1, 3)]
                nbr_d = table(level, nxt, dp['k'], dp['s'], dp['p'], co)
                nbr_s = table(nxt, nxt, K3, S1, P1, co) if name != 'conv_out' else None
                if name == 'conv_out' and caps is not None:
                    lv = [st[2] for st in steps[1:]] + [nxt]
                    key = (tuple(l.cap for l in lv), str(dev))
                    cache = self.__dict__.setdefault('_cap_limits', {})
                    if key not in cache:
                        cache[key] = torch.tensor(key[0], dtype=torch.int32, device=dev)
                    pyr['overflow'] = (torch.cat([l.d_m for l in lv]) > cache[key]).any()
                steps.append((nbr_d, nbr_s, nxt, side.record_event() if overlap else None))
            if overlap:
                hand_over(steps[-1])
                if 'overflow' in pyr and name == 'conv_out':
                    pyr['overflow'].record_stream(main)
        if overlap:
            hand_over(steps[0])
        if staggered and overlap:
            pyr['build_stage'] = build_stage
        else:
            for li in range(4):
                build_stage(li)
        return pyr

    def run_pyramid(self, pyr):
        p = self.plan()
        mm = self.math
        steps = pyr['steps']
        x = pyr['x']
        main = torch.cuda.current_stream(x.device)
        build_stage = pyr.pop('build_stage', None)

        def ready(ev):
            if ev is not None:
                main.wait_event(ev)
        if build_stage is not None:
            build_stage(0)
        _, nbr, lvl1, ev = steps[0]
        ready(ev)
        ci = p['conv_input']
        e = self._e('x_conv1')
        x = self._audit('conv_input', 'x_conv1', ops.spconv_forward(x, nbr, lvl1, *self._p(ci, 0, e), None, True, math=mm), lvl1, e)
        for bi, bp in enumerate(p['conv1']):
            x = self._res_block(x, nbr, lvl1, bp, e, 'conv1.%d' % bi, 'x_conv1')
        lvl1.act_exp = e
        out = {'x_conv1': (x, lvl1)}
        level = lvl1
        for i, name in enumerate(('conv2', 'conv3', 'conv4')):
            if build_stage is not None:
                build_stage(i + 1, gate=main.record_event())
            dp = p[name]['down']
            nbr_d, nbr, nxt, ev = steps[i + 1]
            ready(ev)
            e_prev, e = e, self._e('x_conv%d' % (i + 2))
            stage = 'x_conv%d' % (i + 2)
            x = self._audit('%s.0' % name, stage, ops.spconv_forward(x, nbr_d, nxt, *self._p(dp, e_prev, e), None, True, in_level=level, math=mm), nxt, e)
            for bi, bp in enumerate(p[name]['blocks']):
                x = self._res_block(x, nbr, nxt, bp, e, '%s.%d' % (name, bi + 1), stage)
            nxt.act_exp = e
            out['x_conv%d' % (i + 2)] = (x, nxt)
            level = nxt
        dp = p['conv_out']
        nbr_d, _, nxt, ev = steps[4]
        ready(ev)
        e_prev, e = e, self._e('encoded')
        x = self._audit('conv_out', 'encoded', ops.spconv_forward(x, nbr_d, nxt, *self._p(dp, e_prev, e), None, True, in_level=level, math=mm), nxt, e)
        nxt.act_exp = e
        out['encoded'] = (x, nxt)
        return out

    def run(self, voxel_features, voxel_coords, batch_size, d_n=None, side_key=0, exact=False):
        return self.run_pyramid(self.build_pyramid(voxel_features, voxel_coords, batch_size, d_n, True, side_key, exact=exact))

    def _side_stream(self, dev, key=0):
        pool = self.__dict__.setdefault('_side_streams', {})
        k = (str(dev), key)
        if k not in pool:
            pool[k] = torch.cuda.Stream(device=dev, priority=int(os.environ.get('DZ_TUNE_SIDE_PRIORITY', '0')))
        return pool[k]

    def forward(self, batch_dict):
        _inference_only(self)
        vf = batch_dict['voxel_features'].float().contiguous()
        vc = batch_dict['voxel_coords'].int().contiguous()
        batch_size = batch_dict['batch_size']
        with torch.no_grad():
            res = self.run(vf, vc, batch_size, exact=True)

        def as_tensor(item):
            feats, level = item
            m = level.num_active()
            return SparseConvTensor(None, level.coords[:m], level.shape, batch_size, level=level, padded=(feats, level), math=self.math)
        batch_dict.update({'encoded_spconv_tensor': as_tensor(res['encoded']), 'encoded_spconv_tensor_stride': 8})
        batch_dict.update({'multi_scale_3d_features': {k: as_tensor(res[k]) for k in ('x_conv1', 'x_conv2', 'x_conv3', 'x_conv4')}})
        batch_dict.update({'multi_scale_3d_strides': {'x_conv1': 1, 'x_conv2': 2, 'x_conv3': 4, 'x_conv4': 8}})
        return batch_dict


class HeightCompression(nn.Module):

    def __init__(self, model_cfg, **kwargs):
        super().__init__()
        self.model_cfg = model_cfg
        self.num_bev_features = self.model_cfg.NUM_BEV_FEATURES

    def forward(self, batch_dict):
        t = batch_dict['encoded_spconv_tensor']
        feats, level = t._padded if t._padded is not None else (t.features, t._level)
        math = t._math if t._padded is not None else 0
        c = feats.shape[1]
        bev = ops.sparse_to_bev(feats, level, c, pad=1, math=math)
        e = int(getattr(level, 'act_exp', 0) or 0) if t._padded is not None else 0
        batch_dict['_nhwc_spatial_features'] = bev
        batch_dict['_nhwc_math'] = math
        batch_dict['_nhwc_exp'] = e
        plain = ops.pair16_to_f32(bev, math) if math else bev
        if e:
            plain = plain * (2.0 ** -e)
# ... 653 lines not shown
```

### detzero_amd/lib.py

```python
import ctypes
import os

import torch

_HERE = os.path.dirname(os.path.abspath(__file__))
LIB_PATH = os.path.join(_HERE, 'libdetzero_hip.so')


ERR_INVALID, ERR_WORKSPACE, ERR_HIP, ERR_UNSUPPORTED = -1, -2, -3, -4


class DetZeroHipError(RuntimeError):
    pass


c_int, c_float, c_size_t, c_void_p, c_double = ctypes.c_int, ctypes.c_float, ctypes.c_size_t, ctypes.c_void_p, ctypes.c_double
_I3 = c_int * 3
_F3 = c_float * 3
_F6 = c_float * 6
_I8 = c_int * 8


class Conv2dDesc(ctypes.Structure):
    _fields_ = [
        ('inp', c_void_p), ('out', c_void_p), ('w', c_void_p), ('scale', c_void_p), ('shift', c_void_p),
        ('batch', c_int), ('ho', c_int), ('wo', c_int),
        ('in_hp', c_int), ('in_wp', c_int), ('in_cstride', c_int), ('in_coff', c_int), ('cin', c_int),
        ('kh', c_int), ('kw', c_int), ('stride', c_int), ('in_off', c_int),
        ('out_hp', c_int), ('out_wp', c_int), ('out_cstride', c_int), ('out_coff', c_int),
        ('out_sy', c_int), ('out_sx', c_int), ('out_dy', c_int), ('out_dx', c_int),
        ('groups', c_int), ('cout_pad', c_int),
        ('g_cout', _I8), ('g_ooff', _I8),
        ('relu', c_int),
        ('group_shift', c_void_p), ('group_rows', c_int), ('group_max', c_int), ('phase_groups', c_int),
        ('in_rowidx', c_void_p), ('in_row_channels', c_int), ('in_rows', c_int), ('in_tiles', c_void_p),
    ]


_SIGS = {
    'dz_version': (ctypes.c_char_p, []),
    'dz_last_error': (ctypes.c_char_p, []),
    'dz_device_cu_count': (c_int, []),
    'dz_voxelize_hard_workspace_bytes': (c_size_t, [c_int] * 5),
    'dz_voxelize_hard': (c_int, [c_void_p, c_int, c_int, c_void_p, c_void_p, c_void_p, c_int, c_int, c_int, c_void_p,
                                 c_void_p, c_void_p, c_void_p, c_void_p, c_size_t, c_void_p]),
    'dz_voxelize_hard_mean': (c_int, [c_void_p, c_int, c_int, c_void_p, c_void_p, c_void_p, c_int, c_int, c_int, c_int, c_void_p,
                                      c_int, c_void_p, c_void_p, c_void_p, c_size_t, c_void_p]),
    'dz_voxelize_hard_batched_workspace_bytes': (c_size_t, [c_int] * 6),
    'dz_voxelize_hard_mean_batched': (c_int, [c_void_p, c_int, c_int, c_int, c_void_p, c_void_p, c_void_p, c_int, c_int, c_int, c_void_p,
                                              c_int, c_void_p, c_int, c_void_p, c_void_p, c_size_t, c_void_p]),
    'dz_voxelize_to_level_workspace_bytes': (c_size_t, [c_int] * 8),
    'dz_voxelize_to_level': (c_int, [c_void_p, c_int, c_int, c_int, c_void_p, c_void_p, c_void_p, c_int, c_int, c_int, c_int, c_int, c_void_p,
                                     c_void_p, c_void_p, c_void_p, c_int, c_void_p, c_int, c_int, c_void_p, c_size_t, c_void_p]),
    'dz_mean_vfe': (c_int, [c_void_p, c_void_p, c_void_p, c_int, c_int, c_int, c_void_p, c_int, c_void_p]),
    'dz_voxelize_dynamic_workspace_bytes': (c_size_t, [c_int] * 7),
    'dz_voxelize_dynamic_mean': (c_int, [c_void_p, c_int, c_int, c_void_p, c_void_p, c_void_p, c_int, c_int, c_void_p,
                                         c_void_p, c_void_p, c_int, c_void_p, c_size_t, c_void_p]),
    'dz_index_words': (c_size_t, [c_int] * 5),
    'dz_index_workspace_bytes': (c_size_t, [c_int] * 5),
    'dz_index_from_coords': (c_int, [c_void_p, c_void_p, c_int, c_int, c_int, c_int, c_int, c_int, c_void_p, c_void_p,
                                     c_void_p, c_void_p, c_int, c_void_p, c_void_p, c_size_t, c_void_p]),
    'dz_index_downsample': (c_int, [c_void_p, c_void_p, c_int, c_int, c_int, c_int, c_int, c_int, c_void_p, c_void_p,
                                    c_void_p, c_void_p, c_void_p, c_void_p, c_void_p, c_int, c_void_p, c_size_t,
                                    c_void_p]),
    'dz_draw_subsets': (c_int, [c_void_p, c_int, c_int, ctypes.c_ulonglong, c_int, c_void_p, c_void_p]),
    'dz_grm_feature_channels': (c_int, [c_int]),
    'dz_grm_encode_points': (c_int, [c_void_p, c_void_p, c_void_p, c_void_p, c_void_p, c_void_p, c_int, c_void_p, c_void_p,
                                     c_int, c_int, c_int, c_int, c_void_p, c_void_p, c_void_p]),
    'dz_prm_feature_channels': (c_int, [c_void_p, c_int]),
    'dz_prm_encode_points': (c_int, [c_void_p, c_void_p, c_void_p, c_void_p, c_void_p, c_void_p, c_void_p, c_void_p, c_int, c_int,
                                     c_int, c_int, c_void_p, c_int, c_void_p, c_void_p, c_void_p, c_void_p, c_void_p, c_void_p,
                                     c_void_p]),
    'dz_tta_augment_points': (c_int, [c_void_p, c_int, c_int, c_void_p, c_void_p, c_int, c_void_p, c_void_p]),
    'dz_tta_restore_boxes': (c_int, [c_void_p, c_int, c_int, c_int, c_int, c_void_p, c_void_p, c_void_p]),
    'dz_wbf_workspace_bytes': (c_size_t, [c_int, c_int]),
    'dz_wbf_fuse_3d': (c_int, [c_void_p, c_void_p, c_void_p, c_void_p, c_int, c_int, c_int, c_void_p, c_int, c_void_p, c_void_p, c_double,
                               c_int, c_int, c_void_p, c_void_p, c_void_p, c_void_p, c_void_p, c_void_p, c_size_t, c_void_p]),
    'dz_merge_sweeps_workspace_bytes': (c_size_t, [c_int]),
    'dz_merge_sweeps': (c_int, [c_void_p, c_int, c_void_p, c_void_p, c_void_p, c_int, c_void_p, c_void_p, c_void_p, c_size_t, c_void_p]),
    'dz_linear_forward_split': (c_int, [c_void_p, ctypes.c_long, c_int, c_int, c_void_p, c_int, c_int, c_void_p, c_void_p, c_void_p, c_int,
                                        c_int, c_void_p, c_int, c_int, c_int, c_int, c_void_p]),
    'dz_tile_masks_words': (c_int, [c_int]),
    'dz_build_neighbors': (c_int, [c_void_p, c_void_p, c_int, c_void_p, c_void_p, c_int, c_int, c_int, c_int, c_int,
                                   c_void_p, c_void_p, c_void_p, c_void_p, c_void_p, c_void_p]),
    'dz_build_neighbors_packed': (c_int, [c_void_p, c_void_p, c_int, c_void_p, c_void_p, c_int, c_int, c_int, c_int, c_int,
                                          c_void_p, c_void_p, c_void_p, c_void_p, c_void_p, c_void_p]),
    'dz_scatter_rows': (c_int, [c_void_p, c_void_p, c_void_p, c_int, c_int, c_void_p, c_int, c_void_p]),
    'dz_spconv_forward': (c_int, [c_void_p, c_int, c_int, c_void_p, c_int, c_int, c_void_p, c_void_p, c_void_p, c_void_p,
                                  c_void_p, c_int, c_void_p, c_int, c_void_p]),
    'dz_sparse_to_bev': (c_int, [c_void_p, c_void_p, c_void_p, c_int, c_int, c_int, c_int, c_int, c_int, c_void_p,
                                 c_void_p]),
    'dz_conv2d_forward': (c_int, [ctypes.POINTER(Conv2dDesc), c_void_p]),
    'dz_conv2d_variant': (ctypes.c_char_p, [ctypes.POINTER(Conv2dDesc)]),
    'dz_spconv_variant': (ctypes.c_char_p, [c_int, c_int]),
    'dz_pair16_from_f32': (c_int, [c_void_p, ctypes.c_long, c_int, c_int, c_int, c_void_p, c_void_p]),
    'dz_pair16_to_f32': (c_int, [c_void_p, ctypes.c_long, c_int, c_int, c_void_p, c_void_p]),
    'dz_range_probe': (c_int, [c_void_p, ctypes.c_long, c_void_p, c_int, c_int, c_int, c_int, c_void_p, c_void_p]),
    'dz_range_reset': (c_int, [c_void_p, c_int, c_void_p]),
    'dz_scatter_rows_split': (c_int, [c_void_p, c_void_p, c_void_p, c_int, c_int, c_void_p, c_int, c_int, c_void_p]),
    'dz_spconv_forward_split': (c_int, [c_void_p, c_int, c_int, c_void_p, c_void_p, c_int, c_int, c_void_p, c_void_p, c_void_p,
                                        c_void_p, c_void_p, c_int, c_void_p, c_int, c_int, c_void_p]),
    'dz_spconv_forward_split_packed': (c_int, [c_void_p, c_int, c_int, c_void_p, c_void_p, c_int, c_void_p, c_void_p, c_void_p,
                                               c_void_p, c_void_p, c_int, c_void_p, c_int, c_int, c_void_p]),
    'dz_spconv_tile_rows': (c_int, []),
    'dz_spconv_tile_info_words': (c_int, []),
    'dz_spconv_tile_table_entries': (c_int, []),
    'dz_build_tiles_halo_stride': (c_size_t, [c_int]),
    'dz_build_tiles': (c_int, [c_void_p, c_int, c_int, c_void_p, c_void_p, c_void_p, c_void_p, c_void_p, c_void_p]),
    'dz_spconv_tiles_forward': (c_int, [c_void_p, c_int, c_int, c_void_p, c_void_p, c_void_p, c_void_p, c_int, c_int, c_void_p, c_void_p,
                                        c_void_p, c_void_p, c_void_p, c_int, c_void_p, c_int, c_int, c_void_p]),
    'dz_spconv_tiles_variant': (ctypes.c_char_p, [c_int, c_int]),
    'dz_spconv_x_tile_rows': (c_int, [c_int, c_int]),
    'dz_spconv_x_window_rows': (c_int, [c_int, c_int]),
    'dz_spconv_x_windows_words': (c_size_t, [c_int, c_int]),
    'dz_spconv_x_windows': (c_int, [c_void_p, c_int, c_void_p, c_int, c_void_p, c_void_p, c_void_p, c_void_p]),
    'dz_build_neighbors_packed_x': (c_int, [c_void_p, c_void_p, c_int, c_void_p, c_void_p, c_int, c_int, c_int, c_int, c_void_p, c_void_p, c_int,
                                            c_void_p, c_void_p, c_void_p, c_void_p]),
    'dz_spconv_forward_split_x': (c_int, [c_void_p, c_int, c_int, c_void_p, c_void_p, c_void_p, c_int, c_int, c_void_p, c_void_p, c_void_p, c_void_p,
                                          c_void_p, c_int, c_void_p, c_int, c_int, c_void_p]),
    'dz_spconv_x_variant': (ctypes.c_char_p, [c_int, c_int]),
    'dz_spconv_forward_x_f32': (c_int, [c_void_p, c_int, c_int, c_void_p, c_void_p, c_void_p, c_int, c_int, c_void_p, c_void_p, c_void_p, c_void_p,
                                        c_void_p, c_int, c_void_p, c_int, c_void_p]),
    'dz_spconv_x_f32_window_rows': (c_int, [c_int, c_int]),
    'dz_spconv_x_f32_variant': (ctypes.c_char_p, [c_int, c_int]),
    'dz_bev_tile_list_words': (c_size_t, [c_int, c_int, c_int]),
    'dz_bev_tile_list': (c_int, [c_void_p, c_int, c_int, c_int, c_int, c_int, c_int, c_void_p, c_void_p, c_void_p]),
    'dz_bev_fill_empty_tiles': (c_int, [c_void_p, c_int, c_int, c_int, c_void_p, c_int, c_int, c_void_p, c_int, c_int, c_int, c_int, c_void_p, c_int, c_void_p]),
    'dz_bev_row_index': (c_int, [c_void_p, c_void_p, c_int, c_int, c_int, c_int, c_int, c_int, c_int, c_void_p, c_void_p]),
    'dz_sparse_to_bev_split': (c_int, [c_void_p, c_void_p, c_void_p, c_int, c_int, c_int, c_int, c_int, c_int, c_void_p,
                                       c_void_p]),
    'dz_sparse_to_bev_split_dense': (c_int, [c_void_p, c_int, c_void_p, c_void_p, c_int, c_int, c_int, c_int, c_int, c_int, c_int, c_void_p,
                                             c_void_p]),
    'dz_conv2d_forward_split': (c_int, [ctypes.POINTER(Conv2dDesc), c_int, c_int, c_void_p]),
    'dz_conv2d_variant_split': (ctypes.c_char_p, [ctypes.POINTER(Conv2dDesc), c_int]),
    'dz_spconv_variant_split': (ctypes.c_char_p, [c_int, c_int]),
    'dz_spconv_variant_split_arm': (ctypes.c_char_p, [c_int, c_int, c_int, c_int, c_size_t]),
    'dz_spconv_variant_split_packed': (ctypes.c_char_p, [c_int, c_int]),
    'dz_xattn_folded_supported': (c_int, [c_int, c_int, c_int]),
    'dz_xattn_folded_workspace_bytes': (ctypes.c_size_t, [c_int, c_int]),
    'dz_xattn_folded': (c_int, [c_void_p] * 6 + [c_int] * 5 + [ctypes.c_float, c_void_p, ctypes.c_size_t, c_void_p, c_void_p]),
    'dz_roi_bev_features': (c_int, [c_void_p, c_int, c_void_p, ctypes.c_long, ctypes.c_long, c_int, c_int, c_int] + [ctypes.c_float] * 4 + [c_int, c_void_p, c_void_p]),
    'dz_linear_splitk_workspace_bytes': (ctypes.c_size_t, [c_int, c_int, c_int]),
    'dz_linear_forward_splitk': (c_int, [c_void_p, c_int, c_int, c_int, c_void_p, c_int, c_int, c_void_p, c_void_p, c_int, c_void_p, c_int, c_int, c_void_p,
                                         ctypes.c_size_t, c_void_p]),
    'dz_mha_core_split': (c_int, [c_void_p, c_void_p, c_void_p, c_void_p, c_int, c_int, c_int, c_int, ctypes.c_float, c_void_p, c_int, c_void_p]),
    'dz_pdv_sa_pool_supported': (c_int, [c_int] * 7),
    'dz_pdv_sa_pool': (c_int, [c_void_p, c_int, c_int, c_void_p, c_void_p, c_int, c_void_p, c_void_p, c_int, c_void_p, c_void_p, c_int,
                               c_void_p, c_int, c_void_p, c_void_p, c_int, c_void_p, c_int, c_void_p, c_void_p, c_int, c_int, c_void_p, c_void_p]),
    'dz_pdv_encoder_front': (c_int, [c_void_p, c_int, c_void_p, c_void_p, ctypes.c_long] + [c_void_p] * 9 + [c_int, c_void_p]),
    'dz_pdv_encoder_back': (c_int, [c_void_p, c_void_p, c_void_p, c_void_p, ctypes.c_long, c_void_p, c_void_p, c_void_p, c_void_p, c_float, c_void_p, c_void_p,
                                    c_void_p, c_void_p, c_void_p, c_void_p, c_float, c_void_p, c_int, c_int, c_void_p]),
    'dz_self_attention_split_supported': (c_int, [c_int, c_int]),
    'dz_self_attention_split': (c_int, [c_void_p, c_void_p, c_void_p, c_int, c_int, c_int, c_void_p, c_int, c_void_p]),
    'dz_pdv_sa_pool_split_supported': (c_int, [c_int] * 7),
    'dz_pdv_sa_pool_split': (c_int, [c_void_p, c_int, c_int, c_void_p, c_void_p, ctypes.c_long, c_int, c_void_p, c_void_p, c_int, c_void_p, c_void_p, c_int,
                                     c_void_p, c_int, c_void_p, c_void_p, c_int, c_void_p, c_int, c_void_p, c_void_p, c_int, c_int, c_int, c_void_p, c_int, c_void_p]),
    'dz_mlp_chain_forward': (c_int, [c_void_p, ctypes.c_long, c_void_p, c_void_p, c_void_p, c_void_p, c_int, c_int] + [c_void_p] * 10 + [c_int, c_void_p]),
    'dz_pointnet3_forward': (c_int, [c_void_p, ctypes.c_long] + [c_void_p] * 9 + [c_int, c_int, c_void_p, c_void_p, c_int, c_int, c_void_p]),
    'dz_centerhead_decode_workspace_bytes': (c_size_t, [c_int] * 4),
    'dz_centerhead_decode': (c_int, [c_void_p, c_int, c_int, c_int, c_int, c_int, c_float, c_void_p, c_void_p,
                                     c_void_p, c_int, c_int, c_void_p, c_void_p, c_void_p, c_void_p, c_void_p,
                                     c_size_t, c_void_p]),
    'dz_centerhead_candidates_offset': (c_size_t, [c_int] * 5),
    'dz_centerhead_select': (c_int, [c_void_p, c_int, c_int, c_int, c_int, c_int, c_int, c_void_p, c_size_t, c_void_p]),
    'dz_centerhead_decode_selected': (c_int, [c_void_p, c_int, c_int, c_int, c_int, c_int, c_float, c_void_p, c_void_p,
                                              c_void_p, c_int, c_void_p, c_void_p, c_void_p, c_void_p, c_void_p,
                                              c_size_t, c_void_p]),
    'dz_head_at_candidates_supported': (c_int, [c_int, c_int]),
    'dz_head_at_candidates': (c_int, [c_void_p, c_int, c_int, c_int, c_void_p, c_void_p, c_int, c_int, c_void_p, c_int, c_void_p, c_void_p,
                                      c_void_p, c_void_p, c_void_p, c_int, c_void_p, c_void_p, c_void_p, c_int, c_void_p]),
    'dz_nms_workspace_bytes': (c_size_t, [c_int]),
    'dz_nms_rotated': (c_int, [c_void_p, c_void_p, c_int, c_float, c_int, c_void_p, c_void_p, c_void_p, c_size_t,
                               c_void_p]),
    'dz_nms_rotated_batched': (c_int, [c_void_p, c_void_p, c_int, c_int, c_float, c_int, c_void_p, c_void_p, c_void_p, c_size_t,
                                       c_void_p]),
    'dz_pack_detections': (c_int, [c_void_p, c_void_p, c_void_p, c_void_p, c_void_p, c_int, c_int, c_int, c_void_p, c_void_p]),
    'dz_boxes_overlap_bev': (c_int, [c_void_p, c_int, c_void_p, c_int, c_void_p, c_void_p]),
    'dz_boxes_iou_bev': (c_int, [c_void_p, c_int, c_void_p, c_int, c_void_p, c_void_p]),
    'dz_boxes_pairwise_metric': (c_int, [c_void_p, c_int, c_void_p, c_int, c_int, c_void_p, c_void_p]),
    'dz_nms_normal': (c_int, [c_void_p, c_void_p, c_int, c_float, c_int, c_void_p, c_void_p, c_void_p, c_size_t,
                              c_void_p]),
    'dz_nms_normal_batched': (c_int, [c_void_p, c_void_p, c_int, c_int, c_float, c_int, c_void_p, c_void_p, c_void_p, c_size_t,
                                      c_void_p]),
    'dz_gather_rows': (c_int, [c_void_p, c_void_p, c_void_p, c_int, c_int, c_void_p, c_void_p]),
    'dz_pdv_centroids_workspace_bytes': (c_size_t, [c_int] * 7),
    'dz_pdv_voxel_centroids': (c_int, [c_void_p, c_int, c_int, c_void_p, c_void_p, c_void_p, c_int, c_int, c_void_p, c_void_p, c_void_p, c_void_p,
                                       c_int, c_void_p, c_void_p, c_void_p, c_void_p, c_int, c_void_p, c_size_t, c_void_p]),
    'dz_index_lookup': (c_int, [c_void_p, c_void_p, c_int, c_void_p, c_void_p, c_int, c_int, c_int, c_int, c_int, c_void_p, c_void_p]),
    'dz_pdv_ball_query': (c_int, [c_void_p, c_int, c_int, c_void_p, c_void_p, c_void_p, c_int, c_int, c_int, c_int, c_void_p, c_void_p, c_float,
                                  c_int, c_void_p, c_void_p, c_void_p]),
    'dz_pdv_group_features': (c_int, [c_void_p, c_int, c_int, c_void_p, c_void_p, c_int, c_void_p, c_void_p, c_int, c_void_p, c_void_p, c_int,
                                      c_void_p, c_int, c_void_p]),
    'dz_pdv_part_counts': (c_int, [c_void_p, c_int, c_int, c_void_p, c_int, c_int, c_int, c_int, c_void_p, c_void_p]),
    'dz_pdv_part_counts_ws_bytes': (ctypes.c_size_t, [c_int, c_int]),
    'dz_pdv_part_counts_binned': (c_int, [c_void_p, c_int, c_int, c_void_p, c_int, c_int, c_int, c_int, c_void_p, c_void_p, ctypes.c_size_t, c_void_p]),
    'dz_attention_single_head': (c_int, [c_void_p, c_void_p, c_void_p, c_void_p, c_int, c_int, c_int, c_float, c_void_p, c_void_p]),
    'dz_points_in_boxes_count': (c_int, [c_void_p, c_void_p, c_int, c_int, c_void_p, c_void_p]),
    'dz_points_in_boxes_v2': (c_int, [c_void_p, c_void_p, c_int, c_int, c_int, c_void_p, c_void_p]),
    'dz_crop_points_workspace_bytes': (c_size_t, [c_int] * 3),
    'dz_crop_points_in_boxes': (c_int, [c_void_p, c_int, c_void_p, c_int, c_void_p, c_int, c_void_p, c_void_p, c_void_p, c_void_p,
                                        c_int, c_void_p, c_size_t, c_void_p]),
    'dz_mha_core': (c_int, [c_void_p, c_void_p, c_void_p, c_void_p, c_int, c_int, c_int, c_int, c_float, c_void_p,
                            c_void_p]),
    'dz_linear_forward': (c_int, [c_void_p, c_int, c_int, c_int, c_void_p, c_int, c_int, c_void_p, c_void_p, c_void_p,
                                  c_int, c_int, c_void_p, c_int, c_void_p]),
    'dz_group_max': (c_int, [c_void_p, c_int, c_int, c_int, c_void_p, c_void_p]),
    'dz_rows_all_zero': (c_int, [c_void_p, c_void_p, c_int, c_int, c_void_p, c_void_p]),
    'dz_add_layernorm_combine': (c_int, [c_void_p, c_void_p, c_void_p, c_void_p, c_int, c_int, c_float, c_void_p, c_void_p, c_int, c_void_p, c_void_p]),
    'dz_add_layernorm': (c_int, [c_void_p, c_void_p, c_void_p, c_void_p, c_int, c_int, c_float, c_int, c_void_p, c_void_p]),
}

_lib = None


def load():
    global _lib
    if _lib is not None:
        return _lib
    if not os.path.exists(LIB_PATH):
        raise DetZeroHipError(
            'libdetzero_hip.so not found at %s - build it with `python -m detzero_amd.build` '
            '(hipcc --offload-arch=gfx950); there is no CPU fallback' % LIB_PATH)
    lib = ctypes.CDLL(LIB_PATH)
    for name, (res, args) in _SIGS.items():
        fn = getattr(lib, name)
        fn.restype = res
        fn.argtypes = args
    variant_split = lib.dz_conv2d_variant_split
    lib.dz_conv2d_variant_split = lambda desc, out_f32=0: variant_split(desc, out_f32)
    _lib = lib
    return lib


def exported_symbols():
    return sorted(_SIGS)
# ... 37 lines not shown
```

### include/detzero_hip.h

```cpp
#ifndef DETZERO_HIP_H
#define DETZERO_HIP_H

#include <stddef.h>
#include <stdint.h>

#ifdef __cplusplus
extern "C" {
#endif

#define DZ_OK 0
#define DZ_ERR_INVALID (-1)
#define DZ_ERR_WORKSPACE (-2)
#define DZ_ERR_HIP (-3)
#define DZ_ERR_UNSUPPORTED (-4)

const char *dz_version(void);
const char *dz_last_error(void);
int dz_device_cu_count(void);


size_t dz_voxelize_hard_workspace_bytes(int n, int gx, int gy, int gz, int max_points);
int dz_voxelize_hard(const float *points, int n, int c, const float *h_range6, const float *h_vsize3,
                     const int *h_grid3, int xy_range_mask, int max_points, int max_voxels, float *voxels,
                     int *coords_zyx, int *num_points, int *d_num_voxels, void *ws, size_t ws_bytes,
                     void *stream);
int dz_voxelize_hard_mean(const float *points, int n, int c, const float *h_range6, const float *h_vsize3,
                          const int *h_grid3, int xy_range_mask, int max_points, int max_voxels, int batch_index,
                          float *feats, int c_stride, int *coords_bzyx, int *d_num_voxels, void *ws, size_t ws_bytes,
                          void *stream);
size_t dz_voxelize_hard_batched_workspace_bytes(int n_per_frame, int batch, int gx, int gy, int gz, int max_points);
int dz_voxelize_hard_mean_batched(const float *points, int n_per_frame, int batch, int c, const float *h_range6,
                                  const float *h_vsize3, const int *h_grid3, int xy_range_mask, int max_points,
                                  int max_voxels, float *feats, int c_stride, int *coords_bzyx, int cap_per_frame,
                                  int *d_num_voxels, void *ws, size_t ws_bytes, void *stream);
size_t dz_voxelize_to_level_workspace_bytes(int n_per_frame, int batch, int max_points, int cap, int d, int h, int w, int layout);
int dz_voxelize_to_level(const float *points, int n_per_frame, int batch, int c, const float *h_range6,
                         const float *h_vsize3, const int *h_grid3, int xy_range_mask, int max_points, int max_voxels,
                         int level_d, int layout, uint32_t *bitmap, uint32_t *prefix, int *coords_out, int *d_m, int cap,
                         float *feats, int c_dst, int math, void *ws, size_t ws_bytes, void *stream);

int dz_mean_vfe(const float *voxels, const int *num_points, const int *d_m, int cap, int max_points,
                int c, float *out, int c_out_stride, void *stream);

size_t dz_voxelize_dynamic_workspace_bytes(int n, int batch, int gx, int gy, int gz, int c, int cap);
int dz_voxelize_dynamic_mean(const float *points_b, int n, int c, const float *h_range6,
                             const float *h_vsize3, const int *h_grid3, int xy_range_mask, int batch, float *feats,
                             int *coords_bzyx, int *d_num_voxels, int cap, void *ws, size_t ws_bytes,
                             void *stream);

#define DZ_LAYOUT_LINEAR 0
#define DZ_LAYOUT_BRICK 1
size_t dz_index_words(int b, int d, int h, int w, int layout);
size_t dz_index_workspace_bytes(int b, int d, int h, int w, int layout);

int dz_index_from_coords(const int *coords, const int *d_n, int n_cap, int b, int d, int h, int w, int layout,
                         uint32_t *bitmap, uint32_t *prefix, int *coords_out, int *d_m, int cap_out,
                         int *rank_of_input, void *ws, size_t ws_bytes, void *stream);

int dz_index_downsample(const int *coords_in, const int *d_m_in, int cap_in, int b, int d, int h,
                        int w, int layout, const int *h_k3, const int *h_s3, const int *h_p3, uint32_t *bitmap_out,
                        uint32_t *prefix_out, int *coords_out, int *d_m_out, int cap_out, void *ws,
                        size_t ws_bytes, void *stream);

int dz_build_neighbors(const int *coords_out, const int *d_m_out, int cap_out, const uint32_t *bitmap_in,
                       const uint32_t *prefix_in, int b, int d, int h, int w, int layout, const int *h_k3,
                       const int *h_s3, const int *h_p3, int *nbr, uint32_t *tile_masks, void *stream);
int dz_tile_masks_words(int cap_out);
int dz_build_neighbors_packed(const int *coords_out, const int *d_m_out, int cap_out, const uint32_t *bitmap_in,
                              const uint32_t *prefix_in, int b, int d, int h, int w, int layout, const int *h_k3,
                              const int *h_s3, const int *h_p3, int *nbr, uint32_t *tile_masks, void *stream);

int dz_scatter_rows(const float *src, const int *rank, const int *d_n, int n_cap, int c_src, float *dst,
                    int c_dst, void *stream);

int dz_spconv_forward(const float *in, int in_rows, int cin, const int *nbr, int kvol, int cap_out, const int *d_m_out,
                      const float *w, const float *scale, const float *shift, const float *residual,
                      int relu, float *out, int cout, void *stream);

int dz_sparse_to_bev(const float *feats, const int *coords, const int *d_m, int cap, int c, int d, int h,
                     int w, int pad, float *bev, void *stream);

typedef struct dz_conv2d_desc {
    const float *in;
    float *out;
    const float *w;
    const float *scale;
    const float *shift;
    int batch, ho, wo;
    int in_hp, in_wp, in_cstride, in_coff, cin;
    int kh, kw, stride, in_off;
    int out_hp, out_wp, out_cstride, out_coff;
    int out_sy, out_sx, out_dy, out_dx;
    int groups, cout_pad;
    int g_cout[8];
    int g_ooff[8];
    int relu;
    const float *group_shift;
    int group_rows;
    int group_max;
    int phase_groups;
    const int *in_rowidx;
    int in_row_channels, in_rows;
    const int *in_tiles;
} dz_conv2d_desc;
int dz_conv2d_forward(const dz_conv2d_desc *h_desc, void *stream);
const char *dz_conv2d_variant(const dz_conv2d_desc *h_desc);
const char *dz_spconv_variant(int cin, int cout);

#define DZ_MATH_F32 0
#define DZ_MATH_F16X2 1
#define DZ_MATH_BF16X2 2
#define DZ_MATH_F16 3
int dz_pair16_from_f32(const float *src, long rows, int c_src, int c_dst, int math, float *dst, void *stream);
int dz_pair16_to_f32(const float *src, long rows, int c, int math, float *dst, void *stream);
int dz_range_probe(const float *x, long rows, const int *d_rows, int row_stride_words, int c_off, int c, int math, unsigned long long *slot,
                   void *stream);
int dz_range_reset(unsigned long long *table, int n_slots, void *stream);
int dz_scatter_rows_split(const float *src, const int *rank, const int *d_n, int n_cap, int c_src, float *dst,
                          int c_dst, int math, void *stream);
int dz_spconv_forward_split(const float *in, int in_rows, int cin, const int *nbr, const uint32_t *tile_masks, int kvol,
                            int cap_out, const int *d_m_out, const float *w, const float *scale, const float *shift,
                            const float *residual, int relu, float *out, int cout, int math, void *stream);
int dz_spconv_tile_rows(void);
int dz_spconv_tile_info_words(void);
int dz_spconv_tile_table_entries(void);
size_t dz_build_tiles_halo_stride(int kvol);
int dz_build_tiles(const int *nbr, int kvol, int cap_out, const int *d_m_out, int *halo, int *tinfo, unsigned short *ltab,
                   unsigned short *rowmap, void *stream);
int dz_spconv_tiles_forward(const float *in, int in_rows, int cin, const int *halo, const int *tinfo, const unsigned short *ltab,
                            const unsigned short *rowmap, int kvol, int cap_out, const int *d_m_out, const float *w,
                            const float *scale, const float *shift, const float *residual, int relu, float *out, int cout,
                            int math, void *stream);
const char *dz_spconv_tiles_variant(int cin, int cout);
int dz_spconv_forward_split_packed(const float *in, int in_rows, int cin, const int *nbr_packed, const uint32_t *tile_masks,
                                   int cap_out, const int *d_m_out, const float *w, const float *scale, const float *shift,
                                   const float *residual, int relu, float *out, int cout, int math, void *stream);
int dz_spconv_x_tile_rows(int cin, int cout);
int dz_spconv_x_window_rows(int cin, int cout);
size_t dz_spconv_x_windows_words(int cap_out, int tile_rows);
int dz_spconv_x_windows(const int *nbr_packed, int cap_out, const int *d_m_out, int tile_rows, int *windows, int *nbr_sorted, int *perm,
                        void *stream);
int dz_build_neighbors_packed_x(const int *coords, const int *d_m, int cap, const uint32_t *bitmap, const uint32_t *prefix, int b, int d,
                                int h, int w, int *nbr_packed, uint32_t *tile_masks, int tile_rows, int *windows, int *nbr_sorted,
                                int *perm, void *stream);
int dz_spconv_forward_split_x(const float *in, int in_rows, int cin, const int *nbr_packed, const int *perm, int *windows, int tile_rows,
                              int cap_out, const int *d_m_out, const float *w, const float *scale, const float *shift,
                              const float *residual, int relu, float *out, int cout, int math, void *stream);
const char *dz_spconv_x_variant(int cin, int cout);
int dz_spconv_forward_x_f32(const float *in, int in_rows, int cin, const int *nbr_packed, const int *perm, int *windows, int tile_rows,
                            int cap_out, const int *d_m_out, const float *w, const float *scale, const float *shift,
                            const float *residual, int relu, float *out, int cout, void *stream);
int dz_spconv_x_f32_window_rows(int cin, int cout);
const char *dz_spconv_x_f32_variant(int cin, int cout);
int dz_bev_row_index(const uint32_t *bitmap, const uint32_t *prefix, int batch, int d, int h, int w, int layout, int pad, int feat_rows,
                     int *idx, void *stream);
size_t dz_bev_tile_list_words(int batch, int ho, int wo);
int dz_bev_tile_list(const int *idx, int batch, int hp, int wp, int ho, int wo, int nlists, int *lists, unsigned char *mind_ws, void *stream);
int dz_bev_fill_empty_tiles(const int *list, int batch, int ho, int wo, const float *shift, int relu, int cout, float *out, int out_hp, int out_wp,
                            int out_cstride, int out_coff, const float *zero_resp, int math, void *stream);
int dz_sparse_to_bev_split(const float *feats, const int *coords, const int *d_m, int cap, int c, int d, int h,
                           int w, int pad, float *bev, void *stream);
int dz_sparse_to_bev_split_dense(const float *feats, int feat_rows, const uint32_t *bitmap, const uint32_t *prefix, int batch, int c,
                                 int d, int h, int w, int layout, int pad, float *bev, void *stream);
int dz_conv2d_forward_split(const dz_conv2d_desc *h_desc, int math, int out_f32, void *stream);
const char *dz_conv2d_variant_split(const dz_conv2d_desc *h_desc, int out_f32);
int dz_linear_forward_split(const float *x, long rows, int cin, int x_stride, const float *w, int cout, int cout_pad, const float *scale,
                            const float *shift, const float *group_shift, int group_rows, int relu, float *y, int y_stride, int math,
                            int out_f32, int group_max, void *stream);
const char *dz_spconv_variant_split(int cin, int cout);
const char *dz_spconv_variant_split_arm(int cin, int cout, int kvol, int has_tile_masks, size_t nbr_bytes);
const char *dz_spconv_variant_split_packed(int cin, int cout);
int dz_xattn_folded_supported(int lq, int e, int heads);
size_t dz_xattn_folded_workspace_bytes(int b, int lk);
int dz_xattn_folded(const float *q, const float *mem, const uint8_t *key_padding_mask, const float *wk_oi, const float *wv_io, const float *bv,
                    int b, int lq, int lk, int e, int heads, float scale, float *workspace, size_t workspace_bytes, float *out, void *stream);
int dz_mlp_chain_forward(const float *x, long rows, const float *wa, const float *sa, const float *ba, const float *group_shift, int ldg, int group_rows,
                         const float *wb, const float *sb, const float *bb, const float *wk, const float *bk, const float *wv, const float *bv,
                         float *mem, float *k, float *v, int math, void *stream);
int dz_pointnet3_forward(const float *x, long rows, const float *w1, const float *s1, const float *b1, const float *w2, const float *s2,
                         const float *b2, const float *w3, const float *s3, const float *b3, int c3, int group_rows, float *tap, float *out,
                         int x_cols_f32, int math, void *stream);

size_t dz_centerhead_decode_workspace_bytes(int batch, int hw, int ncls, int k);
int dz_centerhead_decode(const float *head, int batch, int h, int w, int ncls, int k, float score_thresh,
                         const float *h_limit6, const float *h_range6, const float *h_vsize3, int stride,
                         int use_iou, float *boxes, float *scores, int *labels, int *d_counts, void *ws,
                         size_t ws_bytes, void *stream);
#define DZ_CENTERHEAD_CAND_STRIDE 1024
size_t dz_centerhead_candidates_offset(int batch, int hw, int ncls, int k, int which);
int dz_centerhead_select(const float *head, int batch, int h, int w, int ncls, int k, int use_iou, void *ws, size_t ws_bytes, void *stream);
int dz_centerhead_decode_selected(const float *head, int batch, int h, int w, int ncls, int k, float score_thresh,
                                  const float *h_limit6, const float *h_range6, const float *h_vsize3, int stride,
                                  float *boxes, float *scores, int *labels, int *d_counts, void *ws, size_t ws_bytes, void *stream);

int dz_head_at_candidates_supported(int math, int channels);
int dz_head_at_candidates(const float *shared, int batch, int h, int w, const unsigned long long *cand, const int *d_ncand, int cand_stride,
                          int k, const float *w1, int w1_cout, const float *s1, const float *b1, const float *w2, const float *s2,
                          const float *b2, int nbranch, const int *h_g_cout, const int *h_g_ooff, float *head, int math, void *stream);

int dz_roi_bev_features(const float *boxes, int n, const float *bev, long row_stride, long pix_stride, int h, int w, int c, float x_lo, float y_lo,
                        float voxel_x, float voxel_y, int stride, float *out, void *stream);

size_t dz_nms_workspace_bytes(int n_cap);
int dz_nms_rotated(const float *boxes, const int *d_n, int n_cap, float thresh, int post_max, int *keep,
                   int *d_num_keep, void *ws, size_t ws_bytes, void *stream);
int dz_nms_rotated_batched(const float *boxes, const int *d_n, int batch, int n_cap, float thresh, int post_max,
                           int *keep, int *d_num_keep, void *ws, size_t ws_bytes, void *stream);
int dz_pack_detections(const float *boxes, const float *scores, const int *labels, const int *keep,
                       const int *d_num_keep, int batch, int k, int post_max, float *out, void *stream);

int dz_boxes_overlap_bev(const float *a, int na, const float *b, int nb, float *out, void *stream);
int dz_boxes_iou_bev(const float *a, int na, const float *b, int nb, float *out, void *stream);

#define DZ_BOXM_UNION_BEV 0
#define DZ_BOXM_IOU3D 1
#define DZ_BOXM_GIOU3D 2
#define DZ_BOXM_GIOU3D_EXACT 3
int dz_boxes_pairwise_metric(const float *a, int na, const float *b, int nb, int metric, float *out, void *stream);

int dz_nms_normal(const float *boxes, const int *d_n, int n_cap, float thresh, int post_max, int *keep, int *d_num_keep,
// ... 122 lines not shown
```

Measured before the change: 1156.

## Enable packed neighbor tables for wide channels, batch fills, rework line-flag scan

Packed 3-tap neighbor tables become the default and now feed the 64- and 128-channel ring-arm sparse conv kernels, which decode each tap from a packed entry instead of reading a full 27-entry table. This cuts neighbor-table memory traffic. Several separate fill launches are merged into one multi-segment fill kernel to reduce launch count. The line-flag-driven bitmap scan moves into a dedicated level_scan_lines path bounded by the number of points. The changes touch unrelated parts and add decode arithmetic per tap in the conv inner loop.

```diff
diff --git a/detzero_amd/csrc/common.h b/detzero_amd/csrc/common.h
--- a/detzero_amd/csrc/common.h
+++ b/detzero_amd/csrc/common.h
@@ -139,10 +139,13 @@
               int *d_num_keep, hipStream_t stream);
 size_t bitmap_scan_workspace_bytes(size_t nwords);
 int bitmap_scan(const uint32_t *bitmap, size_t nwords, uint32_t *prefix, int *d_total, int mode,
-                ScanDims dims, int *coords_out, int cap_out, void *ws, size_t ws_bytes,
-                hipStream_t stream, bool nonzero_only = false,
-                const unsigned char *line_flags = nullptr);
+                ScanDims dims, int *coords_out, int cap_out, void *ws, size_t ws_bytes, hipStream_t stream);
 int level_scan(const uint32_t *bitmap, const LevelGeom &lg, uint32_t *prefix, int *d_total, int *coords_out, int cap_out, void *ws,
-               size_t ws_bytes, hipStream_t stream, bool nonzero_only, const unsigned char *line_flags = nullptr);
+               size_t ws_bytes, hipStream_t stream);
+size_t level_scan_lines_workspace_bytes(size_t nwords);
+int level_scan_lines(const uint32_t *bitmap, const LevelGeom &lg, const unsigned char *line_flags, size_t max_lines, uint32_t *prefix,
+                     int *d_total, int *coords_out, int cap_out, void *ws, size_t ws_bytes, hipStream_t stream);
+struct FillSeg { void *ptr; uint32_t value; size_t nwords; };
+int fill_u32_multi(const FillSeg *segs, int nsegs, hipStream_t stream);
 
 }
diff --git a/detzero_amd/csrc/sparse_conv_h.hip b/detzero_amd/csrc/sparse_conv_h.hip
--- a/detzero_amd/csrc/sparse_conv_h.hip
+++ b/detzero_amd/csrc/sparse_conv_h.hip
@@ -5,7 +5,7 @@
 
 constexpr int KVOL_MAX_H = 27;
 
-template <class T, class M, int NS, bool GN, int OCC>
+template <class T, class M, int NS, bool GN, int OCC, bool PK = false>
 __global__ __launch_bounds__(T::THREADS) __attribute__((amdgpu_waves_per_eu(OCC))) void k_spconv_h(SpConvHArgs a) {
     extern __shared__ __attribute__((aligned(16))) unsigned char smem_raw[];
     v4u *const smem = reinterpret_cast<v4u *>(smem_raw);
@@ -101,7 +101,7 @@
                 unsigned int rem_a = taps;
                 int tap_a = __ffs((int)rem_a) - 1;
                 auto fetch_nbr = [&](int (&dst)[P]) {
-                    const unsigned int toff = (unsigned int)tap_a * nbr_tap_bytes;
+                    const unsigned int toff = (unsigned int)(PK ? tap_a / 3 : tap_a) * nbr_tap_bytes;
 #pragma unroll
                     for (int i = 0; i < P; ++i)
                         asm volatile("buffer_load_dword %0, %1, %2, 0 offen" : "=v"(dst[i]) : "v"(nvoff[i] == OOB_OFFSET ? OOB_OFFSET : nvoff[i] + toff), "s"(nrsrc));
@@ -120,11 +120,20 @@
                     constexpr int S = decltype(s_t)::value;
                     asm volatile("s_waitcnt vmcnt(%0)" ::"n"((NS - 1) * (NST + P)));
                     unsigned int pvoff[P];
+                    const unsigned int tx = (unsigned int)tap % 3u;
+                    const unsigned int sh = 29u + tx, cm = tx >> 1;
+                    const int dl = (int)((tx + 2u) / 3u) - 1;
 #pragma unroll
                     for (int i = 0; i < P; ++i) {
                         asm volatile("" : "+v"(nb[S][i]));
                         const int q = (tid + i * T::THREADS) % (T::KC / 4);
-                        const int rb = nb[S][i];
+                        int rb = nb[S][i];
+                        if constexpr (PK) {
+                            const unsigned int e = (unsigned int)rb;
+                            const int keep = __builtin_amdgcn_sbfe((int)e, sh, 1u);
+                            const int v = (int)(e & 0x1FFFFFFFu) + dl + (int)((e >> 30) & cm);
+                            rb = (v & keep) | ~keep;
+                        }
                         pvoff[i] = (nvoff[i] != OOB_OFFSET && rb >= 0) ? (unsigned int)rb * (unsigned int)(a.cin * 4) + (unsigned int)(q * 16) : OOB_OFFSET;
                     }
                     load_hstage<T>(st, prsrc, pvoff, (unsigned int)(kc * T::KC * 4), crsrc, cvoff,
@@ -162,22 +171,23 @@
 }
 
 
-template <class M, class T, int NS, bool GN, int OCC>
+template <class M, class T, int NS, bool GN, int OCC, bool PK = false>
 static int launch_spconv_h(const SpConvHArgs &a, hipStream_t stream) {
+    static_assert(GN || !PK, "the packed table is read through the ring arm only");
     constexpr int LDS = T::LDS_BYTES + (GN ? 0 : KVOL_MAX_H * T::BP * 4);
     static PerDeviceFlags lds_done;
-    if (int rc_ = reserve_lds(reinterpret_cast<const void *>(&k_spconv_h<T, M, NS, GN, OCC>), LDS, lds_done, "dz_spconv_forward_split")) return rc_;
+    if (int rc_ = reserve_lds(reinterpret_cast<const void *>(&k_spconv_h<T, M, NS, GN, OCC, PK>), LDS, lds_done, "dz_spconv_forward_split")) return rc_;
     int grid = ceil_div(a.cap, T::BP);
     if (grid > 2048) grid = 2048;
     grid = (grid + 7) & ~7;
     if (grid < 8) grid = 8;
-    hipLaunchKernelGGL((k_spconv_h<T, M, NS, GN, OCC>), dim3(grid, a.cout_pad / T::BC), dim3(T::THREADS), LDS, stream, a);
+    hipLaunchKernelGGL((k_spconv_h<T, M, NS, GN, OCC, PK>), dim3(grid, a.cout_pad / T::BC), dim3(T::THREADS), LDS, stream, a);
     DZ_LAUNCH_CHECK();
     return DZ_OK;
 }
 
 enum SpHVariant { SH_NONE = 0, SH_W_16_16, SH_W_16_32, SH_W_32_32, SH_WP_16_16, SH_WP_16_32, SH_WP_32_32, SH_128_32_16_LDS, SH_128_32_32_LDS,
-                  SH_256_64_RING, SH_256_64_LDS, SH_256_128_RING, SH_256_128_LDS };
+                  SH_256_64_RING, SH_256_64_LDS, SH_256_128_RING, SH_256_128_LDS, SH_256_64_RINGP, SH_256_128_RINGP };
 
 using SpHLaunch = int (*)(const SpConvHArgs &, hipStream_t);
 struct SpHEntry { const char *name, *arm; SpHLaunch launch[3]; };
@@ -196,16 +206,22 @@
     {"k_spconv_h<256x64x32>", "k_spconv_h<256x64x32> lds", DZ_BY_MATH(launch_spconv_h, HTile<256, 64, 32, 4, 2>, 3, false, 2)},
     {"k_spconv_h<256x128x32>", "k_spconv_h<256x128x32> ring", DZ_BY_MATH(launch_spconv_h, HTile<256, 128, 32, 4, 2>, 2, true, 2)},
     {"k_spconv_h<256x128x32>", "k_spconv_h<256x128x32> lds", DZ_BY_MATH(launch_spconv_h, HTile<256, 128, 32, 4, 2>, 2, false, 2)},
+    {"k_spconv_h<256x64x32>", "k_spconv_h<256x64x32> ring", DZ_BY_MATH(launch_spconv_h, HTile<256, 64, 32, 4, 2>, 3, true, 2, true)},
+    {"k_spconv_h<256x128x32>", "k_spconv_h<256x128x32> ring", DZ_BY_MATH(launch_spconv_h, HTile<256, 128, 32, 4, 2>, 2, true, 2, true)},
 };
 #undef DZ_BY_MATH
-static_assert(sizeof(kSpH) / sizeof(kSpH[0]) == SH_256_128_LDS + 1, "one entry per variant");
+static_assert(sizeof(kSpH) / sizeof(kSpH[0]) == SH_256_128_RINGP + 1, "one entry per variant");
 
 static SpHVariant spconv_h_select(int cin, int cout, bool packed, bool masks) {
     if (packed || (masks && cout <= 32)) {
         if (cin == 16 && cout == 16) return packed ? SH_WP_16_16 : SH_W_16_16;
         if (cin == 16 && cout == 32) return packed ? SH_WP_16_32 : SH_W_16_32;
         if (cin == 32 && cout == 32) return packed ? SH_WP_32_32 : SH_W_32_32;
-        if (packed) return SH_NONE;
+        if (packed) {
+            if ((cin == 32 || cin == 64) && cout == 64) return SH_256_64_RINGP;
+            if ((cin == 64 || cin == 128) && cout == 128) return SH_256_128_RINGP;
+            return SH_NONE;
+        }
     }
     if (cin == 16 && cout <= 32) return SH_128_32_16_LDS;
     if (cin == 32 && cout <= 32) return SH_128_32_32_LDS;
@@ -255,7 +271,8 @@
     DZ_CHECK_ARG(in && nbr_packed && tile_masks && d_m_out && w && out, "dz_spconv_forward_split_packed: null pointer");
     DZ_CHECK_ARG(math == DZ_MATH_F16X2 || math == DZ_MATH_BF16X2 || math == DZ_MATH_F16, "dz_spconv_forward_split_packed: math %d is not a split mode", math);
     if (cap_out == 0) return DZ_OK;
-    const int kvol = 27, cout_pad = 32;
+    DZ_CHECK_ARG(cout % 8 == 0 && cin % 8 == 0, "dz_spconv_forward_split_packed: channels must be multiples of the 8-channel pair16 group");
+    const int kvol = 27, cout_pad = cout < 32 ? 32 : cout;
     const size_t in_bytes = (size_t)in_rows * cin * sizeof(float);
     const size_t w_bytes = (size_t)kvol * cout_pad * cin * sizeof(float);
     const size_t nbr_bytes = (size_t)9 * cap_out * sizeof(int);
@@ -267,7 +284,7 @@
                   (unsigned int)in_bytes, (unsigned int)w_bytes, (unsigned int)nbr_bytes, (unsigned int)tile_masks_words(cap_out) * 4u};
     const SpHVariant v = spconv_h_select(cin, cout, true, true);
     if (v == SH_NONE) {
-        set_error("dz_spconv_forward_split_packed: %d -> %d channels (the packed table feeds the 16 -> 16, 16 -> 32 and 32 -> 32 kernels)", cin, cout);
+        set_error("dz_spconv_forward_split_packed: %d -> %d channels (the packed table feeds the 16 -> 16, 16 -> 32, 32 -> 32 kernels and the ring arm of the 64 / 128-channel tiles)", cin, cout);
         return DZ_ERR_UNSUPPORTED;
     }
     return kSpH[v].launch[math - 1](a, stream);
diff --git a/detzero_amd/csrc/sparse_index.hip b/detzero_amd/csrc/sparse_index.hip
--- a/detzero_amd/csrc/sparse_index.hip
+++ b/detzero_amd/csrc/sparse_index.hip
@@ -32,24 +32,57 @@
     return DZ_OK;
 }
 
+constexpr int FILL_MAX_SEGS = 8;
+struct FillSegs { uint32_t *p[FILL_MAX_SEGS]; size_t n[FILL_MAX_SEGS]; uint32_t v[FILL_MAX_SEGS]; };
+__global__ void k_fill_u32_multi(FillSegs s) {
+    uint32_t *const p = s.p[blockIdx.y];
+    const size_t n = s.n[blockIdx.y], n4 = n / 4;
+    const uint32_t v = s.v[blockIdx.y];
+    uint4 *p4 = reinterpret_cast<uint4 *>(p);
+    const uint4 v4 = make_uint4(v, v, v, v);
+    for (size_t i = (size_t)blockIdx.x * blockDim.x + threadIdx.x; i < n4; i += (size_t)gridDim.x * blockDim.x) p4[i] = v4;
+    for (size_t i = n4 * 4 + (size_t)blockIdx.x * blockDim.x + threadIdx.x; i < n; i += (size_t)gridDim.x * blockDim.x) p[i] = v;
+}
+
+int fill_u32_multi(const FillSeg *segs, int nsegs, hipStream_t stream) {
+    if (nsegs < 0 || nsegs > FILL_MAX_SEGS) { set_error("fill_u32_multi: %d segments (at most %d)", nsegs, FILL_MAX_SEGS); return DZ_ERR_INVALID; }
+    FillSegs a;
+    int k = 0;
+    size_t longest = 0;
+    for (int i = 0; i < nsegs; ++i) {
+        if (segs[i].nwords == 0) continue;
+        if (!segs[i].ptr || ((uintptr_t)segs[i].ptr & 15u) != 0) { set_error("fill_u32_multi: pointer null or not 16-byte aligned"); return DZ_ERR_INVALID; }
+        a.p[k] = reinterpret_cast<uint32_t *>(segs[i].ptr);
+        a.n[k] = segs[i].nwords;
+        a.v[k] = segs[i].value;
+        longest = std::max(longest, segs[i].nwords);
+        ++k;
+    }
+    if (k == 0) return DZ_OK;
+    for (int i = k; i < FILL_MAX_SEGS; ++i) { a.p[i] = nullptr; a.n[i] = 0; a.v[i] = 0u; }
+    hipLaunchKernelGGL(k_fill_u32_multi, dim3(stream_grid((long)(longest / 4 + 1), 256), k), dim3(256), 0, stream, a);
+    DZ_LAUNCH_CHECK();
+    return DZ_OK;
+}
+
 template <int WPT>
 __global__ __launch_bounds__(256) void k_scan_reduce(const uint32_t *__restrict__ bitmap, size_t nwords,
-                                                     uint32_t *__restrict__ partial, const unsigned char *__restrict__ line_flags) {
+                                                     uint32_t *__restrict__ partial) {
     __shared__ uint32_t lds[4];
     const size_t base = (size_t)blockIdx.x * (256 * WPT) + (size_t)threadIdx.x * WPT;
     uint32_t s = 0;
-    if (!line_flags || (base < nwords && line_flags[base >> 5])) {
-#pragma unroll
-        for (int j = 0; j < WPT; ++j)
-            if (base + j < nwords) s += __popc(bitmap[base + j]);
-    }
+#pragma unroll
+    for (int j = 0; j < WPT; ++j)
+        if (base + j < nwords) s += __popc(bitmap[base + j]);
     uint32_t total;
     block_excl_scan_256(s, lds, total);
     if (threadIdx.x == 0) partial[blockIdx.x] = total;
 }
 
-__global__ __launch_bounds__(1024) void k_scan_partials(uint32_t *__restrict__ partial, int nblocks, int *__restrict__ d_total) {
+__global__ __launch_bounds__(1024) void k_scan_partials(uint32_t *__restrict__ partial, int nblocks, int *__restrict__ d_total,
+                                                        const int *__restrict__ d_items = nullptr, int per = 1) {
     constexpr int PPT = 8, TRIP = 1024 * PPT;
+    if (d_items) nblocks = min(nblocks, (*d_items + per - 1) / per);
     __shared__ uint32_t buf[TRIP + TRIP / 32];
     __shared__ uint32_t wsum[16];
     const int t = threadIdx.x, lane = t & 63, wid = t >> 6;
@@ -102,25 +135,60 @@
 }
 struct ScanDecode { FastDiv d0, d1, d2; };
 
-template <int MODE, int WPT, bool NZ = false>
+template <int MODE>
+__device__ __forceinline__ void emit_word_coords(uint32_t word, uint32_t r, const uint32_t key0, const ScanDecode &dec,
+                                                 int *__restrict__ coords_out, int cap_out) {
+    if (MODE == 2) {
+        uint32_t z, by, bx;
+        const uint32_t brick = fast_divmod(key0 >> 6, dec.d0, z);
+        const uint32_t t = fast_divmod(brick, dec.d2, bx);
+        const uint32_t bb = fast_divmod(t, dec.d1, by);
+        const int y0 = (int)(by * 8u + ((key0 >> 3) & 7u)), x0 = (int)(bx * 8u);
+        while (word) {
+            const int bit = __ffs((int)word) - 1;
+            word &= word - 1;
+            if ((int)r < cap_out) reinterpret_cast<int4 *>(coords_out)[r] = make_int4((int)bb, (int)z, y0 + (bit >> 3), x0 + (bit & 7));
+            ++r;
+        }
+        return;
+    }
+    uint32_t c2, c1, c0;
+    const uint32_t t1 = fast_divmod(key0, dec.d2, c2);
+    const uint32_t t0 = fast_divmod(t1, dec.d1, c1);
+    uint32_t bb = fast_divmod(t0, dec.d0, c0);
+    int last = 0;
+    while (word) {
+        const int bit = __ffs((int)word) - 1;
+        word &= word - 1;
+        c2 += (uint32_t)(bit - last);
+        last = bit;
+        while (c2 >= dec.d2.d) {
+            c2 -= dec.d2.d;
+            if (++c1 == dec.d1.d) { c1 = 0; if (++c0 == dec.d0.d) { c0 = 0; ++bb; } }
+        }
+        if ((int)r < cap_out) {
+            int4 o;
+            if (MODE == 0) o = make_int4((int)bb, (int)c0, (int)c1, (int)c2);
+            else o = make_int4((int)bb, (int)c2, (int)c1, (int)c0);
+            reinterpret_cast<int4 *>(coords_out)[r] = o;
+        }
+        ++r;
+    }
+}
+
+template <int MODE, int WPT>
 __global__ __launch_bounds__(256) void k_scan_down(const uint32_t *__restrict__ bitmap, size_t nwords,
                                                    const uint32_t *__restrict__ partial,
                                                    uint32_t *__restrict__ prefix, ScanDecode dec,
-                                                   int *__restrict__ coords_out, int cap_out,
-                                                   const unsigned char *__restrict__ line_flags, const int *__restrict__ d_total) {
+                                                   int *__restrict__ coords_out, int cap_out) {
     constexpr int CHUNK = 256 * WPT;
-    if (NZ) {
-        const uint32_t p0 = partial[blockIdx.x], p1 = blockIdx.x + 1 < gridDim.x ? partial[blockIdx.x + 1] : (uint32_t)*d_total;
-        if (p0 == p1) return;
-    }
     __shared__ uint32_t lds[4];
     __shared__ __attribute__((aligned(16))) uint32_t w_s[CHUNK];
     __shared__ __attribute__((aligned(16))) uint32_t p_s[CHUNK];
     const size_t base = (size_t)blockIdx.x * CHUNK + (size_t)threadIdx.x * WPT;
     uint32_t wv[WPT];
-    const bool live = !line_flags || (base < nwords && line_flags[base >> 5]);
-#pragma unroll
-    for (int j = 0; j < WPT; ++j) wv[j] = (live && base + j < nwords) ? bitmap[base + j] : 0u;
+#pragma unroll
+    for (int j = 0; j < WPT; ++j) wv[j] = (base + j < nwords) ? bitmap[base + j] : 0u;
     uint32_t s = 0;
 #pragma unroll
     for (int j = 0; j < WPT; ++j) s += __popc(wv[j]);
@@ -131,7 +199,7 @@
     for (int j = 0; j < WPT; ++j) { pv[j] = run; run += __popc(wv[j]); }
 #pragma unroll
     for (int j = 0; j < WPT; ++j)
-        if (base + j < nwords && (!NZ || wv[j])) prefix[base + j] = pv[j];
+        if (base + j < nwords) prefix[base + j] = pv[j];
     if (MODE < 0 || total == 0) return;
 #pragma unroll
     for (int j = 0; j < WPT; ++j) { w_s[threadIdx.x * WPT + j] = wv[j]; p_s[threadIdx.x * WPT + j] = pv[j]; }
@@ -141,44 +209,7 @@
         const int idx = threadIdx.x + 256 * j;
         uint32_t word = w_s[idx];
         if (!word) continue;
-        uint32_t r = p_s[idx];
-        const uint32_t key0 = (uint32_t)(((size_t)blockIdx.x * CHUNK + idx) << 5);
-        if (MODE == 2) {
-            uint32_t z, by, bx;
-            const uint32_t brick = fast_divmod(key0 >> 6, dec.d0, z);
-            const uint32_t t = fast_divmod(brick, dec.d2, bx);
-            const uint32_t bb = fast_divmod(t, dec.d1, by);
-            const int y0 = (int)(by * 8u + ((key0 >> 3) & 7u)), x0 = (int)(bx * 8u);
-            while (word) {
-                const int bit = __ffs((int)word) - 1;
-                word &= word - 1;
-                if ((int)r < cap_out) reinterpret_cast<int4 *>(coords_out)[r] = make_int4((int)bb, (int)z, y0 + (bit >> 3), x0 + (bit & 7));
-                ++r;
-            }
-            continue;
-        }
-        uint32_t c2, c1, c0;
-        const uint32_t t1 = fast_divmod(key0, dec.d2, c2);
-        const uint32_t t0 = fast_divmod(t1, dec.d1, c1);
-        uint32_t bb = fast_divmod(t0, dec.d0, c0);
-        int last = 0;
-        while (word) {
-            const int bit = __ffs((int)word) - 1;
-            word &= word - 1;
-            c2 += (uint32_t)(bit - last);
-            last = bit;
-            while (c2 >= dec.d2.d) {
-                c2 -= dec.d2.d;
-                if (++c1 == dec.d1.d) { c1 = 0; if (++c0 == dec.d0.d) { c0 = 0; ++bb; } }
-            }
-            if ((int)r < cap_out) {
-                int4 o;
-                if (MODE == 0) o = make_int4((int)bb, (int)c0, (int)c1, (int)c2);
-                else o = make_int4((int)bb, (int)c2, (int)c1, (int)c0);
-                reinterpret_cast<int4 *>(coords_out)[r] = o;
-            }
-            ++r;
-        }
+        emit_word_coords<MODE>(word, p_s[idx], (uint32_t)(((size_t)blockIdx.x * CHUNK + idx) << 5), dec, coords_out, cap_out);
     }
 }
 
@@ -189,47 +220,210 @@
 
 template <int WPT>
 static void launch_scan(const uint32_t *bitmap, size_t nwords, uint32_t *prefix, int *d_total, int mode, const ScanDecode &dec,
-                        int *coords_out, int cap_out, uint32_t *partial, hipStream_t stream, bool nonzero_only,
-                        const unsigned char *lf) {
+                        int *coords_out, int cap_out, uint32_t *partial, hipStream_t stream) {
     const int nblocks = (int)((nwords + 256 * WPT - 1) / (256 * WPT));
-    hipLaunchKernelGGL(k_scan_reduce<WPT>, dim3(nblocks), dim3(256), 0, stream, bitmap, nwords, partial, lf);
-    hipLaunchKernelGGL(k_scan_partials, dim3(1), dim3(1024), 0, stream, partial, nblocks, d_total);
-    if (mode == 0 && nonzero_only)
-        hipLaunchKernelGGL((k_scan_down<0, WPT, true>), dim3(nblocks), dim3(256), 0, stream, bitmap, nwords, partial, prefix, dec,
-                           coords_out, cap_out, lf, d_total);
-    else if (mode == 0)
-        hipLaunchKernelGGL((k_scan_down<0, WPT>), dim3(nblocks), dim3(256), 0, stream, bitmap, nwords, partial, prefix, dec,
-                           coords_out, cap_out, lf, d_total);
+    hipLaunchKernelGGL(k_scan_reduce<WPT>, dim3(nblocks), dim3(256), 0, stream, bitmap, nwords, partial);
+    hipLaunchKernelGGL(k_scan_partials, dim3(1), dim3(1024), 0, stream, partial, nblocks, d_total, nullptr, 1);
+    if (mode == 0)
+        hipLaunchKernelGGL((k_scan_down<0, WPT>), dim3(nblocks), dim3(256), 0, stream, bitmap, nwords, partial, prefix, dec, coords_out, cap_out);
     else if (mode == 1)
-        hipLaunchKernelGGL((k_scan_down<1, WPT>), dim3(nblocks), dim3(256), 0, stream, bitmap, nwords, partial, prefix, dec,
-                           coords_out, cap_out, lf, d_total);
-    else if (mode == 2 && nonzero_only)
-        hipLaunchKernelGGL((k_scan_down<2, WPT, true>), dim3(nblocks), dim3(256), 0, stream, bitmap, nwords, partial, prefix, dec,
-                           coords_out, cap_out, lf, d_total);
+        hipLaunchKernelGGL((k_scan_down<1, WPT>), dim3(nblocks), dim3(256), 0, stream, bitmap, nwords, partial, prefix, dec, coords_out, cap_out);
     else if (mode == 2)
-        hipLaunchKernelGGL((k_scan_down<2, WPT>), dim3(nblocks), dim3(256), 0, stream, bitmap, nwords, partial, prefix, dec,
-                           coords_out, cap_out, lf, d_total);
+        hipLaunchKernelGGL((k_scan_down<2, WPT>), dim3(nblocks), dim3(256), 0, stream, bitmap, nwords, partial, prefix, dec, coords_out, cap_out);
     else
-        hipLaunchKernelGGL((k_scan_down<-1, WPT>), dim3(nblocks), dim3(256), 0, stream, bitmap, nwords, partial, prefix, dec,
-                           coords_out, cap_out, lf, d_total);
-}
-
-int bitmap_scan(const uint32_t *bitmap, size_t nwords, uint32_t *prefix, int *d_total, int mode,
-                ScanDims dims, int *coords_out, int cap_out, void *ws, size_t ws_bytes,
-                hipStream_t stream, bool nonzero_only, const unsigned char *line_flags) {
-    if (ws_bytes < bitmap_scan_workspace_bytes(nwords)) {
-        set_error("bitmap_scan: workspace %zu < %zu", ws_bytes, bitmap_scan_workspace_bytes(nwords));
-        return DZ_ERR_WORKSPACE;
-    }
-    uint32_t *partial = reinterpret_cast<uint32_t *>(ws);
+        hipLaunchKernelGGL((k_scan_down<-1, WPT>), dim3(nblocks), dim3(256), 0, stream, bitmap, nwords, partial, prefix, dec, coords_out, cap_out);
+}
+
+static ScanDecode make_decode(const ScanDims &dims) {
     ScanDecode dec;
     dec.d0 = FastDiv{(uint32_t)(dims.d0 > 0 ? dims.d0 : 1), 1.0 / (double)(dims.d0 > 0 ? dims.d0 : 1)};
     dec.d1 = FastDiv{(uint32_t)(dims.d1 > 0 ? dims.d1 : 1), 1.0 / (double)(dims.d1 > 0 ? dims.d1 : 1)};
     dec.d2 = FastDiv{(uint32_t)(dims.d2 > 0 ? dims.d2 : 1), 1.0 / (double)(dims.d2 > 0 ? dims.d2 : 1)};
-    if (nwords <= ((size_t)1 << 21))
-        launch_scan<1>(bitmap, nwords, prefix, d_total, mode, dec, coords_out, cap_out, partial, stream, nonzero_only, line_flags);
+    return dec;
+}
+
+constexpr size_t SCAN_WPT4_WORDS = (size_t)1 << 21;
+
+int bitmap_scan(const uint32_t *bitmap, size_t nwords, uint32_t *prefix, int *d_total, int mode,
+                ScanDims dims, int *coords_out, int cap_out, void *ws, size_t ws_bytes, hipStream_t stream) {
+    if (ws_bytes < bitmap_scan_workspace_bytes(nwords)) {
+        set_error("bitmap_scan: workspace %zu < %zu", ws_bytes, bitmap_scan_workspace_bytes(nwords));
+        return DZ_ERR_WORKSPACE;
+    }
+    uint32_t *partial = reinterpret_cast<uint32_t *>(ws);
+    const ScanDecode dec = make_decode(dims);
+    if (nwords <= SCAN_WPT4_WORDS)
+        launch_scan<1>(bitmap, nwords, prefix, d_total, mode, dec, coords_out, cap_out, partial, stream);
     else
-        launch_scan<4>(bitmap, nwords, prefix, d_total, mode, dec, coords_out, cap_out, partial, stream, nonzero_only, line_flags);
+        launch_scan<4>(bitmap, nwords, prefix, d_total, mode, dec, coords_out, cap_out, partial, stream);
+    DZ_LAUNCH_CHECK();
+    return DZ_OK;
+}
+
+__device__ __forceinline__ uint32_t nonzero_bytes(uint32_t x) {
+    return (uint32_t)((x & 0xFFu) != 0u) + (uint32_t)((x & 0xFF00u) != 0u) + (uint32_t)((x & 0xFF0000u) != 0u) + (uint32_t)((x & 0xFF000000u) != 0u);
+}
+
+__global__ __launch_bounds__(256) void k_lines_count(const uint4 *__restrict__ flags16, int nunits, uint32_t *__restrict__ lpartial) {
+    __shared__ uint32_t lds[4];
+    const int u = blockIdx.x * 256 + threadIdx.x;
+    uint32_t s = 0;
+    if (u < nunits) {
+        const uint4 v = flags16[u];
+        s = nonzero_bytes(v.x) + nonzero_bytes(v.y) + nonzero_bytes(v.z) + nonzero_bytes(v.w);
+    }
+    uint32_t total;
+    block_excl_scan_256(s, lds, total);
+    if (threadIdx.x == 0) lpartial[blockIdx.x] = total;
+}
+
+__global__ __launch_bounds__(256) void k_lines_emit(const uint4 *__restrict__ flags16, int nunits, const uint32_t *__restrict__ lpartial,
+                                                    int *__restrict__ list) {
+    __shared__ uint32_t lds[4];
+    const int u = blockIdx.x * 256 + threadIdx.x;
+    uint4 v = make_uint4(0u, 0u, 0u, 0u);
+    if (u < nunits) v = flags16[u];
+    const uint32_t s = nonzero_bytes(v.x) + nonzero_bytes(v.y) + nonzero_bytes(v.z) + nonzero_bytes(v.w);
+    uint32_t total;
+    uint32_t run = block_excl_scan_256(s, lds, total) + lpartial[blockIdx.x];
+    if (s == 0) return;
+    const uint32_t w[4] = {v.x, v.y, v.z, v.w};
+#pragma unroll
+    for (int i = 0; i < 16; ++i)
+        if ((w[i >> 2] >> (8 * (i & 3))) & 0xFFu) list[run++] = u * 16 + i;
+}
+
+template <int WPT>
+__device__ __forceinline__ size_t load_line_words(const uint32_t *__restrict__ bitmap, size_t nwords, const int *__restrict__ list, int nl,
+                                                  int c, uint32_t (&wv)[WPT]) {
+    const int pos = threadIdx.x * WPT, li = c * (8 * WPT) + (pos >> 5);
+#pragma unroll
+    for (int j = 0; j < WPT; ++j) wv[j] = 0u;
+    if (li >= nl) return nwords;
+    const size_t base = (size_t)list[li] * 32 + (size_t)(pos & 31);
+    if constexpr (WPT == 4) {
+        if (base + 4 <= nwords) {
+            const uint4 v = *reinterpret_cast<const uint4 *>(bitmap + base);
+            wv[0] = v.x; wv[1] = v.y; wv[2] = v.z; wv[3] = v.w;
+            return base;
+        }
+    }
+#pragma unroll
+    for (int j = 0; j < WPT; ++j)
+        if (base + j < nwords) wv[j] = bitmap[base + j];
+    return base;
+}
+
+template <int WPT>
+__global__ __launch_bounds__(256) void k_lines_reduce(const uint32_t *__restrict__ bitmap, size_t nwords, const int *__restrict__ list,
+                                                      const int *__restrict__ d_nlines, uint32_t *__restrict__ partial) {
+    __shared__ uint32_t lds[4];
+    const int nl = *d_nlines, nchunks = (nl + 8 * WPT - 1) / (8 * WPT);
+    for (int c = blockIdx.x; c < nchunks; c += gridDim.x) {
+        uint32_t wv[WPT], s = 0;
+        load_line_words<WPT>(bitmap, nwords, list, nl, c, wv);
+#pragma unroll
+        for (int j = 0; j < WPT; ++j) s += __popc(wv[j]);
+        uint32_t total;
+        block_excl_scan_256(s, lds, total);
+        if (threadIdx.x == 0) partial[c] = total;
+    }
+}
+
+template <int MODE, int WPT>
+__global__ __launch_bounds__(256) void k_lines_down(const uint32_t *__restrict__ bitmap, size_t nwords, const int *__restrict__ list,
+                                                    const int *__restrict__ d_nlines, const uint32_t *__restrict__ partial,
+                                                    uint32_t *__restrict__ prefix, ScanDecode dec, int *__restrict__ coords_out, int cap_out) {
+    constexpr int CHUNK = 256 * WPT, LPC = 8 * WPT;
+    __shared__ uint32_t lds[4];
+    __shared__ __attribute__((aligned(16))) uint32_t w_s[CHUNK];
+    __shared__ __attribute__((aligned(16))) uint32_t p_s[CHUNK];
+    __shared__ int l_s[LPC];
+    const int nl = *d_nlines, nchunks = (nl + LPC - 1) / LPC;
+    for (int c = blockIdx.x; c < nchunks; c += gridDim.x) {
+        if (threadIdx.x < LPC) l_s[threadIdx.x] = c * LPC + (int)threadIdx.x < nl ? list[c * LPC + threadIdx.x] : 0;
+        uint32_t wv[WPT], s = 0;
+        const size_t base = load_line_words<WPT>(bitmap, nwords, list, nl, c, wv);
+#pragma unroll
+        for (int j = 0; j < WPT; ++j) s += __popc(wv[j]);
+        uint32_t total;
+        uint32_t run = block_excl_scan_256(s, lds, total) + partial[c];
+        uint32_t pv[WPT];
+#pragma unroll
+        for (int j = 0; j < WPT; ++j) { pv[j] = run; run += __popc(wv[j]); }
+#pragma unroll
+        for (int j = 0; j < WPT; ++j)
+            if (wv[j]) prefix[base + j] = pv[j];
+#pragma unroll
+        for (int j = 0; j < WPT; ++j) { w_s[threadIdx.x * WPT + j] = wv[j]; p_s[threadIdx.x * WPT + j] = pv[j]; }
+        __syncthreads();
+#pragma unroll 1
+        for (int j = 0; j < WPT; ++j) {
+            const int idx = threadIdx.x + 256 * j;
+            const uint32_t word = w_s[idx];
+            if (!word) continue;
+            emit_word_coords<MODE>(word, p_s[idx], (uint32_t)(((size_t)l_s[idx >> 5] * 32 + (size_t)(idx & 31)) << 5), dec, coords_out, cap_out);
+        }
+        __syncthreads();
+    }
+}
+
+static size_t lines_layout(size_t nwords, size_t *o_list, size_t *o_lpart, size_t *o_count) {
+    const size_t nlines = (nwords + 31) / 32, nunits = (nlines + 15) / 16;
+    size_t off = bitmap_scan_workspace_bytes(nwords);
+    *o_list = off;
+    off += align_up(nunits * 16 * sizeof(int), 256);
+    *o_lpart = off;
+    off += align_up((nunits + 255) / 256 * sizeof(uint32_t), 256);
+    *o_count = off;
+    return off + 256;
+}
+
+size_t level_scan_lines_workspace_bytes(size_t nwords) {
+    size_t a, b, c;
+    return lines_layout(nwords, &a, &b, &c);
+}
+
+template <int WPT>
+static void launch_lines(const uint32_t *bitmap, size_t nwords, const int *list, const int *d_nlines, size_t max_lines, uint32_t *partial,
+                         uint32_t *prefix, int *d_total, int mode, const ScanDecode &dec, int *coords_out, int cap_out, hipStream_t stream) {
+    const int max_chunks = (int)((max_lines + 8 * WPT - 1) / (8 * WPT));
+    const int grid = std::max(1, std::min(max_chunks, 2048));
+    hipLaunchKernelGGL(k_lines_reduce<WPT>, dim3(grid), dim3(256), 0, stream, bitmap, nwords, list, d_nlines, partial);
+    hipLaunchKernelGGL(k_scan_partials, dim3(1), dim3(1024), 0, stream, partial, max_chunks, d_total, d_nlines, 8 * WPT);
+    if (mode == 0)
+        hipLaunchKernelGGL((k_lines_down<0, WPT>), dim3(grid), dim3(256), 0, stream, bitmap, nwords, list, d_nlines, partial, prefix, dec,
+                           coords_out, cap_out);
+    else
+        hipLaunchKernelGGL((k_lines_down<2, WPT>), dim3(grid), dim3(256), 0, stream, bitmap, nwords, list, d_nlines, partial, prefix, dec,
+                           coords_out, cap_out);
+}
+
+int level_scan_lines(const uint32_t *bitmap, const LevelGeom &lg, const unsigned char *line_flags, size_t max_lines, uint32_t *prefix,
+                     int *d_total, int *coords_out, int cap_out, void *ws, size_t ws_bytes, hipStream_t stream) {
+    const size_t nwords = align_up((lg.cells() + 31) / 32, 8);
+    const size_t nlines = (nwords + 31) / 32, nunits = (nlines + 15) / 16;
+    size_t o_list, o_lpart, o_count;
+    const size_t need = lines_layout(nwords, &o_list, &o_lpart, &o_count);
+    if (ws_bytes < need) { set_error("level_scan_lines: workspace %zu < %zu", ws_bytes, need); return DZ_ERR_WORKSPACE; }
+    if (nunits >= 0x7FFFFFFFull / 16) { set_error("level_scan_lines: %zu bitmap lines do not fit 32-bit line ids", nlines); return DZ_ERR_UNSUPPORTED; }
+    if (((uintptr_t)line_flags & 15u) != 0 || ((uintptr_t)bitmap & 15u) != 0) { set_error("level_scan_lines: pointer not 16-byte aligned"); return DZ_ERR_INVALID; }
+    uint32_t *partial = reinterpret_cast<uint32_t *>(ws);
+    int *list = reinterpret_cast<int *>((char *)ws + o_list);
+    uint32_t *lpartial = reinterpret_cast<uint32_t *>((char *)ws + o_lpart);
+    int *d_nlines = reinterpret_cast<int *>((char *)ws + o_count);
+    const uint4 *flags16 = reinterpret_cast<const uint4 *>(line_flags);
+    const int nblk = (int)((nunits + 255) / 256);
+    hipLaunchKernelGGL(k_lines_count, dim3(nblk), dim3(256), 0, stream, flags16, (int)nunits, lpartial);
+    hipLaunchKernelGGL(k_scan_partials, dim3(1), dim3(1024), 0, stream, lpartial, nblk, d_nlines, nullptr, 1);
+    hipLaunchKernelGGL(k_lines_emit, dim3(nblk), dim3(256), 0, stream, flags16, (int)nunits, lpartial, list);
+    if (max_lines > nlines) max_lines = nlines;
+    const ScanDecode dec = lg.layout == 0 ? make_decode(ScanDims{lg.d, lg.h, lg.w}) : make_decode(ScanDims{lg.d, lg.nby, lg.nbx});
+    const int mode = lg.layout == 0 ? 0 : 2;
+    if (nwords <= SCAN_WPT4_WORDS)
+        launch_lines<1>(bitmap, nwords, list, d_nlines, max_lines, partial, prefix, d_total, mode, dec, coords_out, cap_out, stream);
+    else
+        launch_lines<4>(bitmap, nwords, list, d_nlines, max_lines, partial, prefix, d_total, mode, dec, coords_out, cap_out, stream);
     DZ_LAUNCH_CHECK();
     return DZ_OK;
 }
@@ -685,13 +879,11 @@
 }
 
 int level_scan(const uint32_t *bitmap, const LevelGeom &lg, uint32_t *prefix, int *d_total, int *coords_out, int cap_out, void *ws,
-               size_t ws_bytes, hipStream_t stream, bool nonzero_only, const unsigned char *line_flags) {
+               size_t ws_bytes, hipStream_t stream) {
     const size_t nwords = align_up((lg.cells() + 31) / 32, 8);
     if (lg.layout == 0)
-        return bitmap_scan(bitmap, nwords, prefix, d_total, 0, ScanDims{lg.d, lg.h, lg.w}, coords_out, cap_out, ws, ws_bytes, stream,
-                           nonzero_only, line_flags);
-    return bitmap_scan(bitmap, nwords, prefix, d_total, 2, ScanDims{lg.d, lg.nby, lg.nbx}, coords_out, cap_out, ws, ws_bytes, stream,
-                       nonzero_only, line_flags);
+        return bitmap_scan(bitmap, nwords, prefix, d_total, 0, ScanDims{lg.d, lg.h, lg.w}, coords_out, cap_out, ws, ws_bytes, stream);
+    return bitmap_scan(bitmap, nwords, prefix, d_total, 2, ScanDims{lg.d, lg.nby, lg.nbx}, coords_out, cap_out, ws, ws_bytes, stream);
 }
 
 }
@@ -744,7 +936,7 @@
     if (n_cap > 0)
         hipLaunchKernelGGL(k_set_bits_from_coords, dim3(stream_grid(n_cap, 256)), dim3(256), 0, stream, coords,
                            d_n, n_cap, lg, bitmap);
-    rc = level_scan(bitmap, lg, prefix, d_m, coords_out, cap_out, ws, ws_bytes, stream, false);
+    rc = level_scan(bitmap, lg, prefix, d_m, coords_out, cap_out, ws, ws_bytes, stream);
     if (rc) return rc;
     if (rank_of_input && n_cap > 0)
         hipLaunchKernelGGL(k_rank_of_coords, dim3(stream_grid(n_cap, 256)), dim3(256), 0, stream, coords, d_n,
@@ -776,10 +968,17 @@
     else if (cap_in > 0)
         hipLaunchKernelGGL(k_mark_outputs, dim3(stream_grid(cap_in, 256)), dim3(256), 0, stream, coords_in, d_m_in,
                            cap_in, g, lo, bitmap_out);
-    rc = level_scan(bitmap_out, lo, prefix_out, d_m_out, coords_out, cap_out, ws, ws_bytes, stream, false);
+    rc = level_scan(bitmap_out, lo, prefix_out, d_m_out, coords_out, cap_out, ws, ws_bytes, stream);
     if (rc) return rc;
     DZ_LAUNCH_CHECK();
     return DZ_OK;
+}
+
+int dz_fill_segments(void *const *ptrs, const uint32_t *values, const size_t *nwords, int nsegs, void *stream_) {
+    DZ_CHECK_ARG(nsegs >= 0 && nsegs <= FILL_MAX_SEGS && (nsegs == 0 || (ptrs && values && nwords)), "dz_fill_segments: 0..%d segments", FILL_MAX_SEGS);
+    FillSeg segs[FILL_MAX_SEGS];
+    for (int i = 0; i < nsegs; ++i) segs[i] = FillSeg{ptrs[i], values[i], nwords[i]};
+    return fill_u32_multi(segs, nsegs, (hipStream_t)stream_);
 }
 
 int dz_tile_masks_words(int cap_out) { return cap_out < 0 ? 0 : tile_masks_words(cap_out); }
diff --git a/detzero_amd/csrc/voxelize.hip b/detzero_amd/csrc/voxelize.hip
--- a/detzero_amd/csrc/voxelize.hip
+++ b/detzero_amd/csrc/voxelize.hip
@@ -356,9 +356,8 @@
     const size_t pt_words = align_up(((size_t)n + 31) / 32, 8);
     const int cap = n;
 
-    int rc = fill_u32(w.bitmap, 0u, nwords, stream);
-    if (!rc) rc = fill_u32(w.pt_bitmap, 0u, pt_words, stream);
-    if (!rc) rc = fill_u32(w.mins, 0x7f7f7f7fu, (size_t)max_points * cap, stream);
+    const FillSeg fills[3] = {{w.bitmap, 0u, nwords}, {w.pt_bitmap, 0u, pt_words}, {w.mins, 0x7f7f7f7fu, (size_t)max_points * cap}};
+    int rc = fill_u32_multi(fills, 3, stream);
     if (rc) return rc;
     const int grid_n = stream_grid(n, 256);
     hipLaunchKernelGGL(k_hard_keys, dim3(grid_n), dim3(256), 0, stream, points, n, c, g, n_per, (uint32_t)cells, w.keys, w.bitmap);
@@ -425,7 +424,7 @@
     size_t off = align_up((size_t)(n < 1 ? 1 : n) * 4, 256);
     *o_min = off;
     off += align_up((size_t)max_points * (cap < 1 ? 1 : cap) * 4, 256);
-    *sw_bytes = bitmap_scan_workspace_bytes(nwords);
+    *sw_bytes = level_scan_lines_workspace_bytes(nwords);
     *o_sw = off;
     off += align_up(*sw_bytes, 256);
     *lf_words = align_up((nwords + 31) / 32, 16) / 4;
@@ -467,18 +466,16 @@
     if (ws_bytes < need) { set_error("dz_voxelize_to_level: workspace %zu < %zu", ws_bytes, need); return DZ_ERR_WORKSPACE; }
     uint32_t *keys = (uint32_t *)ws;
     int *mins = (int *)((char *)ws + o_min);
-    static const int use_flags = getenv("DZ_TUNE_LINE_FLAGS") ? atoi(getenv("DZ_TUNE_LINE_FLAGS")) : 1;
-    unsigned char *line_flags = use_flags ? (unsigned char *)ws + o_lf : nullptr;
-    int rc = fill_u32(bitmap, 0u, nwords, stream);
-    if (!rc) rc = fill_u32(mins, 0x7f7f7f7fu, (size_t)max_points * cap, stream);
-    if (!rc && line_flags) rc = fill_u32(line_flags, 0u, lf_words, stream);
-    if (rc) return rc;
-    if (n == 0) return level_scan(bitmap, lg, prefix, d_m, coords_out, cap, (char *)ws + o_sw, sw_bytes, stream, true, line_flags);
+    unsigned char *line_flags = (unsigned char *)ws + o_lf;
+    const FillSeg fills[3] = {{bitmap, 0u, nwords}, {mins, 0x7f7f7f7fu, (size_t)max_points * cap}, {line_flags, 0u, lf_words}};
+    int rc = fill_u32_multi(fills, 3, stream);
+    if (rc) return rc;
+    if (n == 0) return level_scan_lines(bitmap, lg, line_flags, 0, prefix, d_m, coords_out, cap, (char *)ws + o_sw, sw_bytes, stream);
     DZ_CHECK_ARG(points, "dz_voxelize_to_level: null points");
     const int grid_n = stream_grid(n, 256);
     hipLaunchKernelGGL(k_level_keys, dim3(grid_n), dim3(256), 0, stream, points, (int)n, c, g, n_per_frame, lg, keys, bitmap,
                        line_flags);
-    rc = level_scan(bitmap, lg, prefix, d_m, coords_out, cap, (char *)ws + o_sw, sw_bytes, stream, true, line_flags);
+    rc = level_scan_lines(bitmap, lg, line_flags, (size_t)n, prefix, d_m, coords_out, cap, (char *)ws + o_sw, sw_bytes, stream);
     if (rc) return rc;
     hipLaunchKernelGGL(k_hard_insert, dim3(grid_n), dim3(256), 0, stream, keys, (int)n, bitmap, prefix, mins, cap, max_points);
     const dim3 ge(stream_grid((long)cap * (c_dst / 8), 256));
@@ -542,10 +539,9 @@
     int *counts = (int *)(base + o_cnt);
     unsigned long long *acc = (unsigned long long *)(base + o_acc);
 
-    int rc = fill_u32(bitmap, 0u, nwords, stream);
-    if (!rc && cap > 0) rc = fill_u32(feats, 0u, (size_t)cap * c, stream);
-    if (!rc && cap > 0) rc = fill_u32(acc, 0u, (size_t)cap * c * 2, stream);
-    if (!rc && cap > 0) rc = fill_u32(counts, 0u, (size_t)cap, stream);
+    const size_t rows = cap > 0 ? (size_t)cap : 0;
+    const FillSeg fills[4] = {{bitmap, 0u, nwords}, {feats, 0u, rows * c}, {acc, 0u, rows * c * 2}, {counts, 0u, rows}};
+    int rc = fill_u32_multi(fills, 4, stream);
     if (rc) return rc;
     if (n > 0) {
         DZ_CHECK_ARG(points_b, "dz_voxelize_dynamic_mean: null points");
diff --git a/detzero_amd/det_modules.py b/detzero_amd/det_modules.py
--- a/detzero_amd/det_modules.py
+++ b/detzero_amd/det_modules.py
@@ -10,7 +10,6 @@
 from .lib import DetZeroHipError
 from .range_audit import RangeAudit
 
-PACKED_TABLES = bool(os.environ.get('DZ_TUNE_PACKED_TABLES'))
 
 K3, S1, P1 = (3, 3, 3), (1, 1, 1), (1, 1, 1)
 
@@ -359,7 +358,7 @@
         steps = []
         tiled = self.engine == 'tiles' and self.math != 0
 
-        pack = PACKED_TABLES and self.math != 0 and not tiled and self.layout == 0
+        pack = self.math != 0 and not tiled and self.layout == 0
 
         xrun = (self.engine if self.math != 0 else self.f32_engine) == 'xrun' and self.layout == 0
         xrun_couts = tuple(int(c) for c in os.environ.get('DZ_TUNE_XRUN_COUTS', '32,64,128').split(',') if c)
@@ -371,7 +370,7 @@
                 nbr = ops.neighbors_xrun(dst, cout)
                 if getattr(nbr, 'xwin', None) is not None:
                     return nbr
-            nbr = src.neighbors_to(dst, k, s, p, packed=pack and cout <= 32)
+            nbr = src.neighbors_to(dst, k, s, p, packed=pack and tuple(k) == (3, 3, 3) and 36 * max(dst.cap, 1) < (1 << 31))
             return ops.build_tiles(nbr, dst) if tiled and cout in self.tile_couts and k[0] * k[1] * k[2] >= 3 else nbr
 
         def hand_over(step):
diff --git a/detzero_amd/lib.py b/detzero_amd/lib.py
--- a/detzero_amd/lib.py
+++ b/detzero_amd/lib.py
@@ -81,6 +81,7 @@
     'dz_linear_forward_split': (c_int, [c_void_p, ctypes.c_long, c_int, c_int, c_void_p, c_int, c_int, c_void_p, c_void_p, c_void_p, c_int,
                                         c_int, c_void_p, c_int, c_int, c_int, c_int, c_void_p]),
     'dz_tile_masks_words': (c_int, [c_int]),
+    'dz_fill_segments': (c_int, [c_void_p, c_void_p, c_void_p, c_int, c_void_p]),
     'dz_build_neighbors': (c_int, [c_void_p, c_void_p, c_int, c_void_p, c_void_p, c_int, c_int, c_int, c_int, c_int,
                                    c_void_p, c_void_p, c_void_p, c_void_p, c_void_p, c_void_p]),
     'dz_build_neighbors_packed': (c_int, [c_void_p, c_void_p, c_int, c_void_p, c_void_p, c_int, c_int, c_int, c_int, c_int,
diff --git a/include/detzero_hip.h b/include/detzero_hip.h
--- a/include/detzero_hip.h
+++ b/include/detzero_hip.h
@@ -66,6 +66,7 @@
                        const uint32_t *prefix_in, int b, int d, int h, int w, int layout, const int *h_k3,
                        const int *h_s3, const int *h_p3, int *nbr, uint32_t *tile_masks, void *stream);
 int dz_tile_masks_words(int cap_out);
+int dz_fill_segments(void *const *ptrs, const uint32_t *values, const size_t *nwords, int nsegs, void *stream);
 int dz_build_neighbors_packed(const int *coords_out, const int *d_m_out, int cap_out, const uint32_t *bitmap_in,
                               const uint32_t *prefix_in, int b, int d, int h, int w, int layout, const int *h_k3,
                               const int *h_s3, const int *h_p3, int *nbr, uint32_t *tile_masks, void *stream);
```

Result: slower. 1140 (-1.4%).
